# ppwwyyxx/OpenPano

Hardware: NVIDIA H100
Metric: Mpixels/sec SIFT+match+blend (higher is better)
Workload: dtype f32

## Files before the change

openpano_b200/csrc/common.cuh:

```cuda
#pragma once

#include <cuda_runtime.h>
#include <stdint.h>
#include <string>
#include <vector>
#include <map>
#include <memory>
#include <type_traits>
#include <unordered_map>

#include "../../include/pano_b200.h"


int  ctx_alloc(pano_ctx* ctx, void** p, size_t bytes);
void ctx_cache_release(pano_ctx* ctx, size_t keep_bytes);
void ctx_free(pano_ctx* ctx, void* p);
template <class T>
class DevBuf {
 public:
  DevBuf() = default;
  DevBuf(pano_ctx* ctx, T* p) : ctx_(ctx), p_(p) {}
  DevBuf(const DevBuf&) = delete;
  DevBuf& operator=(const DevBuf&) = delete;
  DevBuf(DevBuf&& o) noexcept : ctx_(o.ctx_), p_(o.release()) {}
  DevBuf& operator=(DevBuf&& o) noexcept {
    if (this != &o) { reset(); ctx_ = o.ctx_; p_ = o.release(); }
    return *this;
  }
  ~DevBuf() { reset(); }
  int alloc(pano_ctx* ctx, size_t count) {
    reset();
    ctx_ = ctx;
    void* q = nullptr;
    const int rc = ctx_alloc(ctx, &q, count * sizeof(T));
    p_ = (T*)q;
    return rc;
  }
  void reset() {
    if (p_) ctx_free(ctx_, p_);
    p_ = nullptr;
  }
  T* release() { T* q = p_; p_ = nullptr; return q; }
  T* get() const { return p_; }
  operator T*() const { return p_; }

 private:
  pano_ctx* ctx_ = nullptr;
  T* p_ = nullptr;
};

struct CudaDestroy {
  void operator()(void* host) const { cudaFreeHost(host); }
  void operator()(cudaEvent_t e) const { cudaEventDestroy(e); }
  void operator()(cudaStream_t s) const { cudaStreamDestroy(s); }
  void operator()(cudaMemPool_t p) const { cudaMemPoolDestroy(p); }
};
class PinnedBuf {
 public:
  cudaError_t grow(size_t bytes, size_t alloc, unsigned flags) {
    if (bytes <= cap()) return cudaSuccess;
    p_.reset();
    void* p = nullptr;
    const cudaError_t e = cudaHostAlloc(&p, alloc, flags);
    if (e == cudaSuccess) { p_.reset(p); cap_ = alloc; }
    return e;
  }
  void* get() const { return p_.get(); }
  size_t cap() const { return p_ ? cap_ : 0; }

 private:
  std::unique_ptr<void, CudaDestroy> p_;
  size_t cap_ = 0;
};
using EventPtr = std::unique_ptr<std::remove_pointer_t<cudaEvent_t>, CudaDestroy>;
using StreamPtr = std::unique_ptr<std::remove_pointer_t<cudaStream_t>, CudaDestroy>;
using PoolPtr = std::unique_ptr<std::remove_pointer_t<cudaMemPool_t>, CudaDestroy>;
static inline cudaError_t make_event(EventPtr* ev, unsigned flags) {
  cudaEvent_t e = nullptr;
  const cudaError_t err = cudaEventCreateWithFlags(&e, flags);
  ev->reset(err == cudaSuccess ? e : nullptr);
  return err;
}
static inline cudaError_t make_stream(StreamPtr* s) {
  cudaStream_t h = nullptr;
  const cudaError_t err = cudaStreamCreateWithFlags(&h, cudaStreamNonBlocking);
  s->reset(err == cudaSuccess ? h : nullptr);
  return err;
}


struct ProfEvent {
  const char* name;
  EventPtr start, stop;
};

struct SiftPlan;

struct pano_ctx {
  ~pano_ctx();
  StreamPtr own_stream;
  cudaStream_t stream = nullptr;
  PoolPtr pool;
  int device = 0;
  struct CachedBlock { void* p; unsigned long long stamp; };
  std::multimap<size_t, CachedBlock> cache;
  std::unordered_map<void*, size_t> live;
  size_t cached_bytes = 0, cache_limit = (size_t)16 << 30;
  unsigned long long cache_stamp = 0;
  std::string err;
  bool profiling = false;
  std::vector<ProfEvent> prof_pending;
  std::vector<EventPtr> event_pool;
  std::map<std::string, std::pair<int, double>> prof_acc;
  long long launches = 0;
  int last_match_exact_rows = 0;
  int last_match_nominated_rows = 0;
  int last_match_full_rescans = 0;
  int num_sms = 132;
  bool attr_tc = false, attr_match = false;
  int sift_cap = 0;
  std::unique_ptr<SiftPlan> sift_plan;
  void* tma_encode = nullptr;
  PinnedBuf pinned, pinned2;
  PinnedBuf ring;
  size_t ring_off = 0;
  std::vector<PinnedBuf> small_pinned;
  PinnedBuf flag;
  unsigned flag_seq = 0;
  DevBuf<double2> planet_tab;
};

static inline void ctx_enter(const pano_ctx* ctx) { if (ctx) cudaSetDevice(ctx->device); }

int  ctx_fail(pano_ctx* ctx, int code, const char* fmt, ...);
int  ctx_cuda(pano_ctx* ctx, cudaError_t e, const char* what);
void* ctx_pinned(pano_ctx* ctx, size_t bytes);
void* ctx_pinned2(pano_ctx* ctx, size_t bytes);
extern "C" bool host_is_pinned(const void* p);
cudaError_t ctx_spin_event(cudaEvent_t ev);
cudaError_t ctx_spin_stream(pano_ctx* ctx);
cudaError_t ctx_signal(pano_ctx* ctx, unsigned* token);
cudaError_t ctx_wait_signal(pano_ctx* ctx, unsigned token);
void* ctx_ring(pano_ctx* ctx, size_t bytes);
PinnedBuf ctx_small_pinned_get(pano_ctx* ctx, size_t bytes);
void ctx_small_pinned_put(pano_ctx* ctx, PinnedBuf&& b);
int  ctx_fetch(pano_ctx* ctx, void* d_dst, const void* h_pinned_src, size_t bytes);
int  ctx_store(pano_ctx* ctx, void* h_pinned_dst, const void* d_src, size_t bytes);
int  ctx_put(pano_ctx* ctx, void* d_dst, const void* h_src, size_t bytes);
int  ctx_zero(pano_ctx* ctx, void* d_dst, size_t bytes);
#define CTX_MAX_SEGS 8
int  ctx_put_many(pano_ctx* ctx, int n, void* const* d_dst, const void* const* h_src, const size_t* bytes);
int  ctx_store_many(pano_ctx* ctx, int n, void* const* h_pinned_dst, const void* const* d_src, const size_t* bytes);
int  ctx_copy_blocks(pano_ctx* ctx, int n, void* const* dst, const void* const* src, const size_t* bytes);
void ctx_prof_begin(pano_ctx* ctx, const char* name);
void ctx_prof_end(pano_ctx* ctx);

struct UploadRing {
  ~UploadRing() { if (copy) cudaStreamSynchronize(copy.get()); }
  cudaError_t init();
  int upload(pano_ctx* ctx, int count, const void* const* srcs, const size_t* bytes, const void** d_src, int* slot_out);
  cudaError_t release(pano_ctx* ctx, int slot);

  StreamPtr copy;
  EventPtr ev_copied[2];
  EventPtr ev_done[2];
  DevBuf<unsigned char> slot[2];
  size_t slot_cap[2] = {0, 0};
  PinnedBuf stage[2];
  int windows = 0;
};

double pano_now_ms();
extern double g_trace_slow_ms;
void pano_trace_slow(const char* what, double ms);
struct SlowCall {
  const char* what; double t0;
  explicit SlowCall(const char* w) : what(w), t0(g_trace_slow_ms > 0 ? pano_now_ms() : 0.0) {}
  ~SlowCall() { if (g_trace_slow_ms > 0) { const double d = pano_now_ms() - t0; if (d > g_trace_slow_ms) pano_trace_slow(what, d); } }
};

#define PANO_CUDA(ctx, call)                                          \
  do {                                                                \
    cudaError_t _e;                                                   \
    { SlowCall _sc(#call); _e = (call); }                             \
    if (_e != cudaSuccess) return ctx_cuda((ctx), _e, #call);         \
  } while (0)

#define PANO_LAUNCH(ctx, name, kernel, grid, block, smem, ...)                      \
  do {                                                                              \
    (ctx)->launches++;                                                              \
    if ((ctx)->profiling) ctx_prof_begin((ctx), (name));                            \
    { SlowCall _sc(name); kernel<<<(grid), (block), (smem), (ctx)->stream>>>(__VA_ARGS__); } \
    if ((ctx)->profiling) ctx_prof_end((ctx));                                      \
    cudaError_t _e = cudaGetLastError();                                            \
    if (_e != cudaSuccess) return ctx_cuda((ctx), _e, name);                        \
  } while (0)

struct __align__(64) TmaDesc { unsigned long long opaque[16]; };
int ctx_tma_encode(pano_ctx* ctx, TmaDesc* out, void* base, int rank, const unsigned long long* dims,
                   const unsigned long long* strides_bytes, const unsigned* box);

static inline int pix8_bytes(int fmt) {
  switch (fmt) {
    case PANO_PIX_GREY: return 1;
    case PANO_PIX_RGB: return 3;
    case PANO_PIX_RGBA: return 4;
    case PANO_PIX_RGB_PLANAR: return 3;
    default: return 0;
  }
}
static inline bool pix8_layout(int fmt) { return fmt == PANO_PIX_RGBA || fmt == PANO_PIX_RGB_PLANAR; }
int pix8_check(pano_ctx* ctx, const char* what, int i, int fmt, const void* d_pix);

static inline int ceil_div(int a, int b) { return (a + b - 1) / b; }
static inline unsigned grid_y(long long count) { return (unsigned)(count < 1 ? 1 : count < 65535 ? count : 65535); }
static inline size_t align_up(size_t a, size_t b) { return (a + b - 1) / b * b; }

int host_gauss_kernel(float sigma, int window_factor, float* taps, int cap);

#ifdef __CUDACC__

#define PANO_PI 3.14159265358979323846
#define PANO_PI_2 1.57079632679489661923
#define PANO_SQRT1_2 0.70710678118654752440

#define DBETWEEN(a, b, c) (((a) >= (b)) && ((a) <= (c) - 1))

__constant__ uint64_t c_exp2f_tab[32] = {
    0x3ff0000000000000ull, 0x3fefd9b0d3158574ull, 0x3fefb5586cf9890full, 0x3fef9301d0125b51ull,
    0x3fef72b83c7d517bull, 0x3fef54873168b9aaull, 0x3fef387a6e756238ull, 0x3fef1e9df51fdee1ull,
    0x3fef06fe0a31b715ull, 0x3feef1a7373aa9cbull, 0x3feedea64c123422ull, 0x3feece086061892dull,
    0x3feebfdad5362a27ull, 0x3feeb42b569d4f82ull, 0x3feeab07dd485429ull, 0x3feea47eb03a5585ull,
    0x3feea09e667f3bcdull, 0x3fee9f75e8ec5f74ull, 0x3feea11473eb0187ull, 0x3feea589994cce13ull,
    0x3feeace5422aa0dbull, 0x3feeb737b0cdc5e5ull, 0x3feec49182a3f090ull, 0x3feed503b23e255dull,
    0x3feee89f995ad3adull, 0x3feeff76f2fb5e47ull, 0x3fef199bdd85529cull, 0x3fef3720dcef9069ull,
    0x3fef5818dcfba487ull, 0x3fef7c97337b9b5full, 0x3fefa4afa2a490daull, 0x3fefd0765b6e4540ull};

__device__ __forceinline__ void load_exp2f_tab(uint64_t* s_tab, int tid) {
  if (tid < 32) s_tab[tid] = c_exp2f_tab[tid];
}

__device__ __forceinline__ float glibc_expf(float x, const uint64_t* __restrict__ tab) {
  if (x < -0x1.9fe368p6f) return 0.0f;
  const double InvLn2N = 0x1.71547652b82fep+0 * 32, SHIFT = 0x1.8p+52;
  const double C0 = 0x1.c6af84b912394p-5 / 32 / 32 / 32, C1 = 0x1.ebfce50fac4f3p-3 / 32 / 32,
               C2 = 0x1.62e42ff0c52d6p-1 / 32;
  double xd = (double)x;
  double z = InvLn2N * xd;
  double kd = z + SHIFT;
  uint64_t ki = (uint64_t)__double_as_longlong(kd);
  kd -= SHIFT;
  double r = z - kd;
  uint64_t t = tab[ki & 31];
  t += ki << 47;
  double s = __longlong_as_double((long long)t);
  z = C0 * r + C1;
  double r2 = r * r;
  double y = C2 * r + 1;
  y = z * r2 + y;
  y = y * s;
  return (float)y;
}

__device__ __forceinline__ float glibc_sincos_poly(double x, double x2, bool neg_table, int n) {
  const double sgn = neg_table ? -1.0 : 1.0;
  if ((n & 1) == 0) {
    const double s1c = -0x1.555545995a603p-3, s2c = 0x1.1107605230bc4p-7, s3c = -0x1.994eb3774cf24p-13;
    double x3 = x * x2;
    double s1 = s2c + x2 * s3c;
    double x7 = x3 * x2;
    double s = x + x3 * s1c;
    return (float)(s + x7 * s1);
  } else {
    const double c0 = sgn * 0x1p0, c1c = sgn * -0x1.ffffffd0c621cp-2, c2c = sgn * 0x1.55553e1068f19p-5,
                 c3c = sgn * -0x1.6c087e89a359dp-10, c4c = sgn * 0x1.99343027bf8c3p-16;
    double x4 = x2 * x2;
    double c2 = c3c + x2 * c4c;
    double c1 = c1c + x2 * c2c;
    double x6 = x4 * x2;
    double c = c0 + x2 * c1;
    return (float)(c + x6 * c2);
  }
}

__device__ __forceinline__ uint32_t glibc_abstop12(float x) { return (__float_as_uint(x) >> 20) & 0x7ff; }

__device__ __forceinline__ void glibc_sincosf(float y, float* sn, float* cs) {
  const double hpi_inv = 0x1.45F306DC9C883p+23, hpi = 0x1.921FB54442D18p0;
  double x = (double)y;
  if (glibc_abstop12(y) < glibc_abstop12(0x1.921FB6p-1f)) {
    double x2 = x * x;
    if (glibc_abstop12(y) < glibc_abstop12(0x1p-12f)) { *sn = y; *cs = 1.0f; return; }
    *sn = glibc_sincos_poly(x, x2, false, 0);
    *cs = glibc_sincos_poly(x, x2, false, 1);
    return;
  }
  double r = x * hpi_inv;
  int n = ((int32_t)r + 0x800000) >> 24;
  x = x - n * hpi;
  const double sign = ((n & 3) == 1 || (n & 3) == 2) ? -1.0 : 1.0;
  bool neg = (n & 2) != 0;
  *sn = glibc_sincos_poly(x * sign, x * x, neg, n);
  *cs = glibc_sincos_poly(x * sign, x * x, neg, n ^ 1);
}

__device__ __forceinline__ float glibc_hypotf(float x, float y) {
  double dx = (double)x, dy = (double)y;
  return (float)sqrt(dx * dx + dy * dy);
}

__device__ __forceinline__ float fast_atan(float y, float x) {
  float absx = fabsf(x), absy = fabsf(y);
  float m = absx > absy ? absx : absy;
  if ((double)m < 1e-6) return (float)(-PANO_PI);
  float a = (absy < absx ? absy : absx) / m;
  float s = a * a;
  double sd = (double)s, ad = (double)a;
  float r = (float)(((-0.0464964749 * sd + 0.15931422) * sd - 0.327622764) * sd * ad + ad);
  if (absy > absx) r = (float)(PANO_PI_2 - (double)r);
  if (x < 0) r = (float)(PANO_PI - (double)r);
  if (y < 0) r = -r;
  return r;
}

__device__ __forceinline__ void mag_ort_at(const float* __restrict__ img, int w, int x, int y,
                                           float* mag, float* ort) {
  const float* row = img + (size_t)y * w;
  float dy = row[x + w] - row[x - w];
  float dx = row[x + 1] - row[x - 1];
  *mag = glibc_hypotf(dx, dy);
  *ort = (float)((double)fast_atan(dy, dx) + PANO_PI);
}

struct SrcF32 {
  const float* img;
  static constexpr bool kMayBeNo = true, kLut = false;
  __device__ __forceinline__ void fetch(int w, int fr, int fc, float* q) const {
    const float* p00 = img + ((size_t)fr * w + fc) * 3;
    const float* p10 = p00 + (size_t)w * 3;
#pragma unroll
    for (int k = 0; k < 6; ++k) { q[k] = __ldg(p00 + k); q[6 + k] = __ldg(p10 + k); }
  }
};
struct SrcRgb8 {
  const unsigned char* pix;
  const float* lut;
  int channels;
  static constexpr bool kMayBeNo = false, kLut = true;
  __device__ __forceinline__ void fetch(int w, int fr, int fc, float* q) const {
    if (channels == 1) {
      const unsigned char* p00 = pix + (size_t)fr * w + fc;
      const float a = (float)__ldg(p00), b = (float)__ldg(p00 + 1);
      const float c = (float)__ldg(p00 + w), d = (float)__ldg(p00 + w + 1);
      q[0] = q[1] = q[2] = a; q[3] = q[4] = q[5] = b;
      q[6] = q[7] = q[8] = c; q[9] = q[10] = q[11] = d;
    } else {
      const unsigned char* p00 = pix + ((size_t)fr * w + fc) * 3;
      const unsigned char* p10 = p00 + (size_t)w * 3;
#pragma unroll
      for (int k = 0; k < 6; ++k) { q[k] = lut[__ldg(p00 + k)]; q[6 + k] = lut[__ldg(p10 + k)]; }
    }
  }
};
struct SrcPix8 {
  const unsigned char* pix;
  const float* lut;
  int fmt;
  size_t plane;
  static constexpr bool kMayBeNo = false, kLut = true;
  __device__ __forceinline__ void fetch(int w, int fr, int fc, float* q) const {
    if (fmt == PANO_PIX_RGBA) {
      const unsigned* p00 = reinterpret_cast<const unsigned*>(pix) + (size_t)fr * w + fc;
      const unsigned t[4] = {__ldg(p00), __ldg(p00 + 1), __ldg(p00 + w), __ldg(p00 + w + 1)};
#pragma unroll
      for (int k = 0; k < 4; ++k) {
        q[3 * k] = lut[t[k] & 0xff]; q[3 * k + 1] = lut[(t[k] >> 8) & 0xff]; q[3 * k + 2] = lut[(t[k] >> 16) & 0xff];
      }
    } else if (fmt == PANO_PIX_RGB_PLANAR) {
      const unsigned char* p00 = pix + (size_t)fr * w + fc;
#pragma unroll
      for (int ch = 0; ch < 3; ++ch) {
        const unsigned char* p = p00 + ch * plane;
        q[ch] = lut[__ldg(p)]; q[3 + ch] = lut[__ldg(p + 1)];
        q[6 + ch] = lut[__ldg(p + w)]; q[9 + ch] = lut[__ldg(p + w + 1)];
      }
    } else {
      SrcRgb8{pix, lut, fmt}.fetch(w, fr, fc, q);
    }
  }
};
__device__ __forceinline__ void build_rgb8_lut(float* lut, int tid) {
  if (tid < 256) lut[tid] = (float)((double)tid / 255.0);
}

__device__ __forceinline__ int f2i_x86(float v) {
  return (v >= -2147483648.0f && v < 2147483648.0f) ? (int)v : (int)0x80000000u;
}

template <class Src>
__device__ __forceinline__ bool interpolate_rgb(const Src& src, int w, int h, float r, float c, float* o0, float* o1,
                                                float* o2) {
  int fr = f2i_x86(floorf(r)), fc = f2i_x86(floorf(c));
  if (fr < 0 || fc < 0 || fc + 1 >= w || fr + 1 >= h) return false;
  r -= (float)fr;
  c -= (float)fc;
  float q[12];
  src.fetch(w, fr, fc, q);
  const float q00 = q[0], q01 = q[1], q02 = q[2], q03 = q[3], q04 = q[4], q05 = q[5];
  const float q10 = q[6], q11 = q[7], q12 = q[8], q13 = q[9], q14 = q[10], q15 = q[11];
  if (Src::kMayBeNo && (q00 < 0 || q10 < 0 || q13 < 0 || q03 < 0)) return false;
  float w00 = (1 - r) * (1 - c), w10 = r * (1 - c), w11 = r * c, w01 = (1 - r) * c;
  float a0 = 0.f + q00 * w00, a1 = 0.f + q01 * w00, a2 = 0.f + q02 * w00;
  a0 += q10 * w10; a1 += q11 * w10; a2 += q12 * w10;
  a0 += q13 * w11; a1 += q14 * w11; a2 += q15 * w11;
  a0 += q03 * w01; a1 += q04 * w01; a2 += q05 * w01;
  *o0 = a0; *o1 = a1; *o2 = a2;
  return true;
}
__device__ __forceinline__ bool interpolate_rgb(const float* __restrict__ img, int w, int h, float r, float c,
                                                float* o0, float* o1, float* o2) {
  return interpolate_rgb(SrcF32{img}, w, h, r, c, o0, o1, o2);
}

#endif
```

openpano_b200/csrc/match.cu:

```cuda
#include "sift.cuh"
#include "match_tc.cuh"
#include <float.h>
#include <stdlib.h>
#include <string.h>
#include <algorithm>

__device__ __forceinline__ float exact_dist(const float* __restrict__ a, const float* __restrict__ b) {
  float l0 = 0.f, l1 = 0.f, l2 = 0.f, l3 = 0.f;
  const float4* pa = (const float4*)a;
  const float4* pb = (const float4*)b;
#pragma unroll 8
  for (int k = 0; k < 32; ++k) {
    float4 x = __ldg(pa + k), y = __ldg(pb + k);
    float d0 = x.x - y.x, d1 = x.y - y.y, d2 = x.z - y.z, d3 = x.w - y.w;
    l0 += d0 * d0; l1 += d1 * d1; l2 += d2 * d2; l3 += d3 * d3;
  }
  return (l0 + l1) + (l2 + l3);
}

__device__ __forceinline__ void top2_merge(float& mn, int& idx, float& sec, float m2, int i2, float s2) {
  if (m2 < mn || (m2 == mn && i2 < idx)) { sec = fminf(mn, s2); mn = m2; idx = i2; }
  else sec = fminf(sec, m2);
}

#define MT 64
#define MT_STRIDE 132
#define MT_THREADS 256

struct MatchTask {
  long long q_base, t_base;
  int q_n, t_n;
  int q_row0;
  long long res_off;
};

struct RowInfo { float mn, mn_hi; int idx; float sec_lo, sec_hi; int state; int requested; int pad; };

__global__ void __launch_bounds__(MT_THREADS)
k_match_top2(const float* __restrict__ desc, const MatchTask* __restrict__ tasks, RowInfo* __restrict__ res) {
  extern __shared__ float sm[];
  float* sq = sm;
  float* st = sm + MT * MT_STRIDE;
  const MatchTask tk = tasks[blockIdx.x];
  const int tid = threadIdx.x, tx = tid & 15, ty = tid >> 4;
  const float* Q = desc + tk.q_base * 128;
  const float* T = desc + tk.t_base * 128;

  for (int i = tid; i < MT * 32; i += MT_THREADS) {
    int r = i >> 5, c4 = i & 31;
    int gr = tk.q_row0 + r;
    float4 v = make_float4(0.f, 0.f, 0.f, 0.f);
    if (gr < tk.q_n) v = __ldg((const float4*)(Q + (size_t)gr * 128) + c4);
    *(float4*)(sq + r * MT_STRIDE + c4 * 4) = v;
  }

  float bmn[4], bsec[4];
  int bidx[4];
#pragma unroll
  for (int i = 0; i < 4; ++i) { bmn[i] = FLT_MAX; bsec[i] = FLT_MAX; bidx[i] = 0x7fffffff; }

  for (int t0 = 0; t0 < tk.t_n; t0 += MT) {
    __syncthreads();
    for (int i = tid; i < MT * 32; i += MT_THREADS) {
      int r = i >> 5, c4 = i & 31;
      int gr = t0 + r;
      float4 v = make_float4(0.f, 0.f, 0.f, 0.f);
      if (gr < tk.t_n) v = __ldg((const float4*)(T + (size_t)gr * 128) + c4);
      *(float4*)(st + r * MT_STRIDE + c4 * 4) = v;
    }
    __syncthreads();
    float acc[4][4][4];
#pragma unroll
    for (int i = 0; i < 4; ++i)
#pragma unroll
      for (int j = 0; j < 4; ++j)
#pragma unroll
        for (int l = 0; l < 4; ++l) acc[i][j][l] = 0.f;
#pragma unroll 4
    for (int k = 0; k < 32; ++k) {
      float4 a[4], b[4];
#pragma unroll
      for (int i = 0; i < 4; ++i) a[i] = *(const float4*)(sq + (ty + 16 * i) * MT_STRIDE + k * 4);
#pragma unroll
      for (int j = 0; j < 4; ++j) b[j] = *(const float4*)(st + (tx + 16 * j) * MT_STRIDE + k * 4);
#pragma unroll
      for (int i = 0; i < 4; ++i)
#pragma unroll
        for (int j = 0; j < 4; ++j) {
          float d0 = a[i].x - b[j].x, d1 = a[i].y - b[j].y, d2 = a[i].z - b[j].z, d3 = a[i].w - b[j].w;
          acc[i][j][0] += d0 * d0; acc[i][j][1] += d1 * d1;
          acc[i][j][2] += d2 * d2; acc[i][j][3] += d3 * d3;
        }
    }
#pragma unroll
    for (int i = 0; i < 4; ++i)
#pragma unroll
      for (int j = 0; j < 4; ++j) {
        int col = t0 + tx + 16 * j;
        if (col < tk.t_n) {
          float d = (acc[i][j][0] + acc[i][j][1]) + (acc[i][j][2] + acc[i][j][3]);
          if (d < bmn[i]) { bsec[i] = bmn[i]; bmn[i] = d; bidx[i] = col; }
          else if (d < bsec[i]) bsec[i] = d;
        }
      }
  }
#pragma unroll
  for (int i = 0; i < 4; ++i) {
    float mn = bmn[i], sec = bsec[i];
    int idx = bidx[i];
#pragma unroll
    for (int off = 8; off >= 1; off >>= 1) {
      float m2 = __shfl_xor_sync(0xffffffffu, mn, off);
      float s2 = __shfl_xor_sync(0xffffffffu, sec, off);
      int i2 = __shfl_xor_sync(0xffffffffu, idx, off);
      top2_merge(mn, idx, sec, m2, i2, s2);
    }
    int row = tk.q_row0 + ty + 16 * i;
    if (tx == 0 && row < tk.q_n) {
      RowInfo o; o.mn = mn; o.mn_hi = mn; o.idx = idx; o.sec_lo = sec; o.sec_hi = sec; o.state = 3; o.requested = 0; o.pad = 0;
      res[tk.res_off + row] = o;
    }
  }
}


struct SideMeta {
  long long q_base, t_base;
  int q_n, t_n;
  long long res_off;
  int r0, r1;
  int parts, pad;
};

__device__ __forceinline__ float tc_eps(float nq, float nmax) {
  return 0.00215f * sqrtf(nq * nmax) + 0.0005f * nmax + 1.0f;
}

__device__ __forceinline__ RowInfo refine_row(const float* __restrict__ desc, const SideMeta& sm, int r, const TcTop2 ap,
                                              float eps, float ratio_sqr) {
  RowInfo o;
  o.requested = 0; o.pad = 0;
  const bool idx_ok = ap.idx >= 0 && ap.idx < sm.t_n;
  o.idx = idx_ok ? ap.idx : 0;
  const bool single = ap.m2 == FLT_MAX;
  const bool certain = idx_ok && (single || (ap.m2 - ap.m1 > 2.f * eps));
  if (sm.t_n <= 0) { o.mn = FLT_MAX; o.mn_hi = FLT_MAX; o.sec_lo = FLT_MAX; o.sec_hi = FLT_MAX; o.state = 3; }
  else if (certain && !single && (ap.m1 - eps) > ratio_sqr * (ap.m2 + eps)) {
    o.mn = ap.m1 - eps; o.mn_hi = ap.m1 + eps;
    o.sec_lo = fmaxf(ap.m2 - eps, o.mn); o.sec_hi = ap.m2 + eps;
    o.state = 2;
  }
  else if (certain) {
    o.mn = exact_dist(desc + (size_t)(sm.q_base + r) * 128, desc + (size_t)(sm.t_base + o.idx) * 128);
    o.mn_hi = o.mn;
    if (single) { o.sec_lo = FLT_MAX; o.sec_hi = FLT_MAX; o.state = 3; }
    else { o.sec_lo = fmaxf(ap.m2 - eps, o.mn); o.sec_hi = fmaxf(ap.m2 + eps, o.mn); o.state = 2; }
  } else {
    o.mn = fmaxf(ap.m1 - eps, 0.f); o.mn_hi = ap.m1 + eps;
    o.sec_lo = fmaxf(ap.m2 - eps, 0.f); o.sec_hi = ap.m2 + eps;
    o.state = 0;
  }
  return o;
}

__device__ __forceinline__ void refine_side_row(const float* __restrict__ desc, const float* __restrict__ norms,
                                                const unsigned* __restrict__ maxnorm_bits, const SideMeta* __restrict__ sides,
                                                TcTop2* __restrict__ approx, long long res_total, float ratio_sqr, int lazy,
                                                RowInfo* __restrict__ info, int side, int r) {
  const SideMeta sm = sides[side];
  if (r >= sm.q_n) return;
  if (r < sm.r0 || r >= sm.r1) return;
  if (lazy && (side & 1) && sm.t_n > 0) {
    RowInfo o; o.mn = 0.f; o.mn_hi = FLT_MAX; o.idx = 0; o.sec_lo = 0.f; o.sec_hi = FLT_MAX; o.state = 4; o.requested = 0; o.pad = 0;
    info[sm.res_off + r] = o;
    return;
  }
  const float nmax = __uint_as_float(*maxnorm_bits);
  TcTop2 ap = approx[sm.res_off + r];
  if (sm.parts > 1) {
    for (int p = 1; p < sm.parts; ++p) {
      const TcTop2 q = approx[(long long)p * res_total + sm.res_off + r];
      if (q.m1 < ap.m1) { ap.m2 = fminf(ap.m1, q.m2); ap.m1 = q.m1; ap.idx = q.idx; }
      else ap.m2 = fminf(ap.m2, q.m1);
    }
    approx[sm.res_off + r] = ap;
  }
  info[sm.res_off + r] = refine_row(desc, sm, r, ap, tc_eps(norms[sm.q_base + r], nmax), ratio_sqr);
}

__global__ void k_refine(const float* __restrict__ desc, const float* __restrict__ norms,
                         const unsigned* __restrict__ maxnorm_bits, const SideMeta* __restrict__ sides, int n_sides,
                         TcTop2* __restrict__ approx, long long res_total, float ratio_sqr, int lazy,
                         RowInfo* __restrict__ info) {
  const int r = blockIdx.x * blockDim.x + threadIdx.x;
  for (int side = blockIdx.y; side < n_sides; side += gridDim.y)
    refine_side_row(desc, norms, maxnorm_bits, sides, approx, res_total, ratio_sqr, lazy, info, side, r);
}

__global__ void k_refine_gathered(const float* __restrict__ desc, const float* __restrict__ norms,
                                  const unsigned* __restrict__ maxnorm_bits, const SideMeta* __restrict__ sides,
                                  const int2* __restrict__ g_meta, const TcTop2* __restrict__ g_approx,
                                  const int* __restrict__ n_blocks, float ratio_sqr, TcTop2* __restrict__ approx,
                                  RowInfo* __restrict__ info) {
  const int g = blockIdx.x * blockDim.x + threadIdx.x;
  if (g >= *n_blocks * 128) return;
  const int2 me = g_meta[g];
  if (me.x < 0) return;
  const SideMeta sm = sides[me.x];
  const TcTop2 ap = g_approx[g];
  const float nmax = __uint_as_float(*maxnorm_bits);
  approx[sm.res_off + me.y] = ap;
  info[sm.res_off + me.y] = refine_row(desc, sm, me.y, ap, tc_eps(norms[sm.q_base + me.y], nmax), ratio_sqr);
}

__global__ void __launch_bounds__(256)
k_exact_rows(const float* __restrict__ desc, const SideMeta* __restrict__ sides, const int2* __restrict__ list,
             const int* __restrict__ list_count, RowInfo* __restrict__ info) {
  __shared__ __align__(16) float sq[128];
  __shared__ float s_mn[8], s_sec[8];
  __shared__ int s_idx[8];
  const int tid = threadIdx.x, lane = tid & 31, wid = tid >> 5;
  const int n = *list_count;
  for (int e = blockIdx.x; e < n; e += gridDim.x) {
    const int2 it = list[e];
    const SideMeta sm = sides[it.x];
    const float* q = desc + (size_t)(sm.q_base + it.y) * 128;
    __syncthreads();
    if (tid < 32) *(float4*)(&sq[tid * 4]) = __ldg((const float4*)q + tid);
    __syncthreads();
    float mn = FLT_MAX, sec = FLT_MAX;
    int idx = 0x7fffffff;
    for (int c = tid; c < sm.t_n; c += 256) {
      const float4* pb = (const float4*)(desc + (size_t)(sm.t_base + c) * 128);
      float4 yv[32];
#pragma unroll
      for (int k = 0; k < 32; ++k) yv[k] = __ldg(pb + k);
      float l0 = 0.f, l1 = 0.f, l2 = 0.f, l3 = 0.f;
#pragma unroll
      for (int k = 0; k < 32; ++k) {
        const float4 x = *(const float4*)(&sq[k * 4]), y = yv[k];
        float d0 = x.x - y.x, d1 = x.y - y.y, d2 = x.z - y.z, d3 = x.w - y.w;
        l0 += d0 * d0; l1 += d1 * d1; l2 += d2 * d2; l3 += d3 * d3;
      }
      float d = (l0 + l1) + (l2 + l3);
      if (d < mn) { sec = mn; mn = d; idx = c; }
      else if (d < sec) sec = d;
    }
#pragma unroll
    for (int off = 16; off >= 1; off >>= 1) {
      float m2 = __shfl_xor_sync(0xffffffffu, mn, off);
      float s2 = __shfl_xor_sync(0xffffffffu, sec, off);
      int i2 = __shfl_xor_sync(0xffffffffu, idx, off);
      top2_merge(mn, idx, sec, m2, i2, s2);
    }
    if (lane == 0) { s_mn[wid] = mn; s_sec[wid] = sec; s_idx[wid] = idx; }
    __syncthreads();
    if (tid == 0) {
      for (int wdx = 1; wdx < 8; ++wdx) top2_merge(mn, idx, sec, s_mn[wdx], s_idx[wdx], s_sec[wdx]);
      RowInfo o; o.mn = mn; o.mn_hi = mn; o.idx = idx; o.sec_lo = sec; o.sec_hi = sec; o.state = 3; o.requested = 1; o.pad = 0;
      info[sm.res_off + it.y] = o;
    }
  }
}

struct PairMeta {
  int side_small, side_large;
  int n_small, n_large;
  long long out_off;
  int rev, pad;
  int k0, k1;
};

#define OUT_PENDING (-2)

__device__ __forceinline__ void request_row(const SideMeta* __restrict__ sides, RowInfo* __restrict__ info, int side,
                                            int row, int* list_rows, int* list_unknown,
                                            int* __restrict__ side_cnt, int n_sides) {
  const long long off = sides[side].res_off;
  RowInfo* ri = &info[off + row];
  if (atomicExch(&ri->requested, 1) == 0) {
    if (ri->state & 4) list_unknown[off + atomicAdd(&side_cnt[n_sides + side], 1)] = row;
    else list_rows[off + atomicAdd(&side_cnt[side], 1)] = row;
  }
}

__device__ __forceinline__ void match_decide_row(const PairMeta* __restrict__ pairs, const SideMeta* __restrict__ sides,
                                                 RowInfo* __restrict__ info, float ratio_sqr, int first_round,
                                                 int* __restrict__ out, int* __restrict__ total,
                                                 int* list_rows, int* list_unknown, int* __restrict__ side_cnt,
                                                 int n_sides, int pair, int row) {
  const PairMeta pm = pairs[pair];
  const int k = pm.k0 + row;
  if (k >= pm.k1) return;
  const size_t oslot = pm.out_off + k;
  if (!first_round && out[oslot] != OUT_PENDING) return;
  int result = -1;
  if (pm.n_large > 0) {
    const SideMeta ss = sides[pm.side_small], sl = sides[pm.side_large];
    const RowInfo r = info[ss.res_off + k];
    if (!(r.state & 2)) {
      if (r.mn > ratio_sqr * r.sec_hi) result = -1;
      else {
        result = OUT_PENDING;
        request_row(sides, info, pm.side_small, k, list_rows, list_unknown, side_cnt, n_sides);
        if (info[sl.res_off + r.idx].state & 4)
          request_row(sides, info, pm.side_large, r.idx, list_rows, list_unknown, side_cnt, n_sides);
      }
    } else {
      const RowInfo c = info[sl.res_off + r.idx];
      if (c.state & 4) {
        if (r.mn > ratio_sqr * r.sec_hi) result = -1;
        else if (!(r.mn > 0.f)) result = r.idx;
        else {
          result = OUT_PENDING;
          request_row(sides, info, pm.side_large, r.idx, list_rows, list_unknown, side_cnt, n_sides);
        }
      } else {
        float c_lo, c_hi;
        bool need_c = false;
        if (c.state & 2) {
          const bool mine = c.idx == k;
          c_lo = mine ? c.sec_lo : c.mn; c_hi = mine ? c.sec_hi : c.mn_hi;
          need_c = mine && !(c.state & 1);
        } else {
          c_lo = c.mn; c_hi = c.sec_hi;
          need_c = true;
        }
        const float nlo = fminf(r.sec_lo, c_lo), nhi = fminf(r.sec_hi, c_hi);
        if (r.mn > ratio_sqr * nhi) result = -1;
        else if (!(r.mn > ratio_sqr * nlo)) result = r.idx;
        else {
          result = OUT_PENDING;
          if (!(r.state & 1)) request_row(sides, info, pm.side_small, k, list_rows, list_unknown, side_cnt, n_sides);
          if (need_c) request_row(sides, info, pm.side_large, r.idx, list_rows, list_unknown, side_cnt, n_sides);
        }
      }
    }
  }
  out[oslot] = result;
  if (result >= 0) atomicAdd(total, 1);
}

__global__ void k_match_decide(const PairMeta* __restrict__ pairs, int n_pairs, const SideMeta* __restrict__ sides,
                               RowInfo* __restrict__ info, float ratio_sqr, int first_round,
                               int* __restrict__ out, int* __restrict__ total,
                               int* list_rows, int* list_unknown, int* __restrict__ side_cnt,
                               int n_sides) {
  const int row = blockIdx.x * blockDim.x + threadIdx.x;
  for (int pair = blockIdx.y; pair < n_pairs; pair += gridDim.y)
    match_decide_row(pairs, sides, info, ratio_sqr, first_round, out, total, list_rows, list_unknown, side_cnt, n_sides,
                     pair, row);
}

__global__ void k_gather_plan(const TcGatherSide* __restrict__ gsides, int n_sides, const int* __restrict__ side_cnt,
                              const int* __restrict__ list_rows, int block_cap, TcTask* __restrict__ tasks,
                              int* __restrict__ n_blocks, int2* __restrict__ fb_list, int* __restrict__ fb_cnt) {
  const int side = blockIdx.x * blockDim.x + threadIdx.x;
  if (side >= n_sides) return;
  const int cnt = side_cnt[side];
  if (cnt == 0) return;
  const TcGatherSide gs = gsides[side];
  const int nb = (cnt + 127) / 128;
  const int b0 = atomicAdd(n_blocks, nb);
  if (b0 + nb > block_cap) {
    atomicSub(n_blocks, nb);
    const int f0 = atomicAdd(fb_cnt, cnt);
    for (int i = 0; i < cnt; ++i) fb_list[f0 + i] = make_int2(side, list_rows[gs.list_off + i]);
    return;
  }
  for (int i = 0; i < nb; ++i) {
    TcTask t;
    t.q_blk = b0 + i; t.q_row0 = (b0 + i) * 128; t.q_n = min(128, cnt - i * 128);
    t.t_blk0 = gs.t_blk0; t.t_blocks = gs.t_blocks; t.t_n = gs.t_n; t.t_pad = i * 128;
    t.res_off = side;
    tasks[b0 + i] = t;
  }
}

__global__ void __launch_bounds__(256)
k_exact_cands(const float* __restrict__ desc, const SideMeta* __restrict__ sides, const int* __restrict__ n_blocks,
              const int2* __restrict__ g_meta, const int* __restrict__ cand_cnt, const int* __restrict__ cand,
              RowInfo* __restrict__ info, int2* __restrict__ fb_list, int* __restrict__ fb_cnt) {
  const int lane = threadIdx.x & 31;
  const int nrow = *n_blocks * 128;
  for (int g = blockIdx.x * 8 + (threadIdx.x >> 5); g < nrow; g += gridDim.x * 8) {
    const int2 me = g_meta[g];
    if (me.x < 0) continue;
    const SideMeta sm = sides[me.x];
    const int cnt = cand_cnt[g];
    if (cnt > TC_CAND_CAP || cnt < 1 || (cnt < 2 && sm.t_n >= 2)) {
      if (lane == 0) fb_list[atomicAdd(fb_cnt, 1)] = me;
      continue;
    }
    float mn = FLT_MAX, sec = FLT_MAX;
    int idx = 0x7fffffff;
    if (lane < cnt) {
      idx = cand[(size_t)g * TC_CAND_CAP + lane];
      mn = exact_dist(desc + (size_t)(sm.q_base + me.y) * 128, desc + (size_t)(sm.t_base + idx) * 128);
    }
#pragma unroll
    for (int off = 16; off >= 1; off >>= 1) {
      float m2 = __shfl_xor_sync(0xffffffffu, mn, off);
      float s2 = __shfl_xor_sync(0xffffffffu, sec, off);
      int i2 = __shfl_xor_sync(0xffffffffu, idx, off);
      top2_merge(mn, idx, sec, m2, i2, s2);
    }
    if (lane == 0) {
      RowInfo o; o.mn = mn; o.mn_hi = mn; o.idx = idx; o.sec_lo = sec; o.sec_hi = sec; o.state = 3; o.requested = 1; o.pad = 0;
      info[sm.res_off + me.y] = o;
    }
  }
}

__global__ void __launch_bounds__(256)
k_match_count(const PairMeta* __restrict__ pairs, const int* __restrict__ out, int n_pairs, int* __restrict__ hdr) {
  __shared__ int s_c[8], s_p[8];
  const PairMeta pm = pairs[blockIdx.x];
  int c = 0, pend = 0;
  for (int r = pm.k0 + threadIdx.x; r < pm.k1; r += 256) {
    const int v = out[pm.out_off + r];
    c += v >= 0; pend += v == OUT_PENDING;
  }
  for (int off = 16; off; off >>= 1) { c += __shfl_xor_sync(0xffffffffu, c, off); pend += __shfl_xor_sync(0xffffffffu, pend, off); }
  if ((threadIdx.x & 31) == 0) { s_c[threadIdx.x >> 5] = c; s_p[threadIdx.x >> 5] = pend; }
  __syncthreads();
  if (threadIdx.x == 0) {
    for (int q = 1; q < 8; ++q) { c += s_c[q]; pend += s_p[q]; }
    hdr[2 + blockIdx.x] = c;
    if (pend) atomicAdd(&hdr[1], pend);
  }
}

__global__ void __launch_bounds__(1024)
k_match_offsets(int n_pairs, int* __restrict__ hdr) {
  __shared__ int s_w[32];
  __shared__ int s_carry;
  const int* cnt = hdr + 2;
  int* off = hdr + 2 + n_pairs;
  const int tid = threadIdx.x, lane = tid & 31, wid = tid >> 5;
  if (tid == 0) s_carry = 0;
  __syncthreads();
  for (int base = 0; base < n_pairs; base += 1024) {
    const int k = base + tid;
    const int v = k < n_pairs ? cnt[k] : 0;
    int incl = v;
    for (int d = 1; d < 32; d <<= 1) { const int t = __shfl_up_sync(0xffffffffu, incl, d); if (lane >= d) incl += t; }
    if (lane == 31) s_w[wid] = incl;
    __syncthreads();
    if (wid == 0) {
      int w = s_w[lane], a = w;
      for (int d = 1; d < 32; d <<= 1) { const int t = __shfl_up_sync(0xffffffffu, a, d); if (lane >= d) a += t; }
      s_w[lane] = a - w;
    }
    __syncthreads();
    const int carry = s_carry;
    if (k < n_pairs) off[k] = carry + s_w[wid] + incl - v;
    __syncthreads();
    if (tid == 1023) s_carry = carry + s_w[31] + incl;
    __syncthreads();
  }
  if (tid == 0) { off[n_pairs] = s_carry; hdr[0] = s_carry; }
}

__global__ void __launch_bounds__(256)
k_match_write(const PairMeta* __restrict__ pairs, const int* __restrict__ out, int n_pairs, const int* __restrict__ hdr,
              int* __restrict__ dense) {
  __shared__ int s_w[8];
  __shared__ int s_base;
  const PairMeta pm = pairs[blockIdx.x];
  int* dst = dense + 2 * (size_t)hdr[2 + n_pairs + blockIdx.x];
  const int tid = threadIdx.x, lane = tid & 31, wid = tid >> 5;
  if (tid == 0) s_base = 0;
  __syncthreads();
  for (int r0 = pm.k0; r0 < pm.k1; r0 += 256) {
    const int r = r0 + tid;
    const int j = r < pm.k1 ? out[pm.out_off + r] : -1;
    const unsigned bal = __ballot_sync(0xffffffffu, j >= 0);
    if (lane == 0) s_w[wid] = __popc(bal);
    __syncthreads();
    int before = s_base;
    for (int q = 0; q < wid; ++q) before += s_w[q];
    if (j >= 0) {
      int* d = dst + 2 * (before + __popc(bal & ((1u << lane) - 1)));
      if (pm.rev) { d[0] = j; d[1] = r; } else { d[0] = r; d[1] = j; }
    }
    __syncthreads();
    if (tid == 0) { int t = 0; for (int q = 0; q < 8; ++q) t += s_w[q]; s_base += t; }
    __syncthreads();
  }
}

__global__ void k_match_download(int* __restrict__ h_dst, const int* __restrict__ dense, const int* __restrict__ hdr) {
  const size_t n = (size_t)hdr[0] * 2;
  for (size_t i = (size_t)blockIdx.x * blockDim.x + threadIdx.x; i < n; i += (size_t)gridDim.x * blockDim.x) h_dst[i] = dense[i];
}


struct MatchPlan {
  std::vector<SideMeta> sides;
  std::vector<PairMeta> pairs;
  std::vector<MatchTask> exact_tasks;
  std::vector<TcTask> tc_tasks;
  std::vector<int> task_part;
  std::vector<TcGatherSide> gsides;
  std::vector<char> rev;
  long long res_total = 0, out_total = 0;
  int max_side_n = 0, max_small = 0;
  int parts = 1;
  int shard = 0, n_shards = 1;
  bool lazy = false;
  long long large_blocks = 0;
  long long block_pairs = 0;
};

#define MC_FB(r) (1 + (r))
#define MC_BLK_FILTER(r) (5 + (r))
#define MC_BLK_NOMINATE(r) (9 + (r))
#define MC_HEAD 16
#define MC_ROUNDS 4

static bool use_exact_path() {
  const char* e = getenv("PANO_MATCH_PATH");
  return e && strcmp(e, "exact") == 0;
}

static int build_plan(pano_ctx* ctx, pano_featureset* fs, int n_pairs, const int* ij, MatchPlan& pl,
                      const std::vector<TcImage>* tcimgs) {
  for (int k = 0; k < n_pairs; ++k) {
    int i = ij[2 * k], j = ij[2 * k + 1];
    if (i < 0 || j < 0 || i >= fs->n_images || j >= fs->n_images)
      return ctx_fail(ctx, PANO_ERR_INVALID, "pair %d: image index out of range", k);
    if (fs->h_count[i] > 0 && fs->h_count[j] > 0) {
      const long long bl = (std::max(fs->h_count[i], fs->h_count[j]) + 127) / 128, bs = (std::min(fs->h_count[i], fs->h_count[j]) + 127) / 128;
      pl.large_blocks += bl;
      pl.block_pairs += bl * bs;
    }
  }
  if (tcimgs) {
    pl.lazy = pl.block_pairs >= 32768;
    if (const char* e = getenv("PANO_MATCH_LAZY")) pl.lazy = atoi(e) != 0;
    if (pl.n_shards > 1) pl.lazy = true;
    long long n1 = 0, tile_sum = 0;
    for (int k = 0; k < n_pairs; ++k) {
      const int ci = fs->h_count[ij[2 * k]], cj = fs->h_count[ij[2 * k + 1]];
      if (ci <= 0 || cj <= 0) continue;
      const long long bs = (std::min(ci, cj) + 127) / 128, bl = (std::max(ci, cj) + 127) / 128;
      const long long ts = (std::min(ci, cj) + 255) / 256, tl = (std::max(ci, cj) + 255) / 256;
      const long long mine = pl.lazy ? (bs + pl.n_shards - 1) / pl.n_shards : bs;
      n1 += mine; tile_sum += mine * tl;
      if (!pl.lazy) { n1 += bl; tile_sum += bl * ts; }
    }
    const long long W = std::max(1, ctx->num_sms);
    if (n1 > 0 && n1 < 12 * W) {
      const double T = (double)tile_sum / (double)n1;
      auto cost = [&](int P) { return (double)((n1 * P + W - 1) / W) * (T / P + 0.7); };
      double best = cost(1) * 0.96;
      for (int P = 2; P <= 8; ++P)
        if (T / P >= 4.0 && cost(P) < best * 0.99) { best = cost(P); pl.parts = P; }
    }
    if (const char* e = getenv("PANO_MATCH_PARTS")) pl.parts = std::max(1, std::min(8, atoi(e)));
  }
  for (int k = 0; k < n_pairs; ++k) {
    int i = ij[2 * k], j = ij[2 * k + 1];
    const bool rev = fs->h_count[i] > fs->h_count[j];
    const int is = rev ? j : i, il = rev ? i : j;
    const int ns = fs->h_count[is], nl = fs->h_count[il];
    const int k0 = (int)((long long)ns * pl.shard / pl.n_shards), k1 = (int)((long long)ns * (pl.shard + 1) / pl.n_shards);
    const int tiles_l = tcimgs ? (*tcimgs)[il].n_pad / 256 : 0, tiles_s = tcimgs ? (*tcimgs)[is].n_pad / 256 : 0;
    const int parts_a = std::max(1, std::min(pl.parts, tiles_l / 4)), parts_b = pl.lazy ? 1 : std::max(1, std::min(pl.parts, tiles_s / 4));
    SideMeta a{fs->base[is], fs->base[il], ns, nl, pl.res_total, k0, k1, parts_a, 0}; pl.res_total += ns;
    SideMeta b{fs->base[il], fs->base[is], nl, ns, pl.res_total, 0, nl, parts_b, 0}; pl.res_total += nl;
    PairMeta pm{(int)pl.sides.size(), (int)pl.sides.size() + 1, ns, nl, pl.out_total, rev ? 1 : 0, 0, k0, k1};
    pl.out_total += ns;
    pl.sides.push_back(a); pl.sides.push_back(b);
    pl.pairs.push_back(pm);
    pl.rev.push_back(rev ? 1 : 0);
    pl.max_side_n = std::max(pl.max_side_n, std::max(ns, nl));
    pl.max_small = std::max(pl.max_small, k1 - k0);
    if (tcimgs) {
      const TcImage &ts = (*tcimgs)[is], &tl = (*tcimgs)[il];
      auto add_tasks = [&](const TcImage& tq, const TcImage& tt, int row_lo, int row_hi, int q_n, int t_n, long long res_off, int parts) {
        const int tiles = tt.n_pad / 256;
        for (int r0 = row_lo / 128 * 128; r0 < row_hi; r0 += 128)
          for (int pp = 0; pp < parts; ++pp) {
            const int t0 = (int)((long long)tiles * pp / parts), t1 = (int)((long long)tiles * (pp + 1) / parts);
            pl.tc_tasks.push_back(TcTask{tq.blk0 + r0 / 128, r0, q_n, tt.blk0 + 2 * t0, 2 * (t1 - t0), t_n, t0 * 256, res_off});
            pl.task_part.push_back(pp);
          }
      };
      if (nl > 0) add_tasks(ts, tl, k0, k1, ns, nl, a.res_off, parts_a);
      if (ns > 0 && !pl.lazy) add_tasks(tl, ts, 0, nl, nl, ns, b.res_off, parts_b);
      pl.gsides.push_back(TcGatherSide{a.q_base, a.res_off, a.res_off, ts.blk0, tl.blk0, tl.n_pad / 128, nl});
      pl.gsides.push_back(TcGatherSide{b.q_base, b.res_off, b.res_off, tl.blk0, ts.blk0, ts.n_pad / 128, ns});
    } else {
      for (int r0 = k0 / MT * MT; r0 < k1; r0 += MT) pl.exact_tasks.push_back(MatchTask{a.q_base, a.t_base, ns, nl, r0, a.res_off});
      for (int r0 = 0; r0 < nl; r0 += MT) pl.exact_tasks.push_back(MatchTask{b.q_base, b.t_base, nl, ns, r0, b.res_off});
    }
  }
  for (size_t t = 0; t < pl.tc_tasks.size(); ++t) pl.tc_tasks[t].res_off += (long long)pl.task_part[t] * pl.res_total;
  return PANO_OK;
}

struct MatchBuffers {
  DevBuf<unsigned char> tasks; DevBuf<PairMeta> pairs; DevBuf<SideMeta> sides;
  DevBuf<RowInfo> info; DevBuf<TcTop2> approx;
  DevBuf<int2> list;
  DevBuf<int> counters;
  int n_counters = 0;
  DevBuf<int> out;
  DevBuf<TcGatherSide> gsides; DevBuf<int> list_rows; DevBuf<TcTask> gtasks; DevBuf<unsigned char> gq;
  DevBuf<int2> g_meta; DevBuf<int> g_thr; DevBuf<int> cand_cnt; DevBuf<int> cand;
  DevBuf<int> list_unknown; DevBuf<TcTask> ntasks; DevBuf<unsigned char> nq; DevBuf<int2> n_meta;
  DevBuf<TcTop2> n_approx;
  int rounds = 2;
};

static int run_plan(pano_ctx* ctx, pano_featureset* fs, const MatchPlan& pl, float ratio, bool tensor,
                    const TcOperands* ops, MatchBuffers& b) {
  int rc = 0;
  const size_t bt = tensor ? pl.tc_tasks.size() * sizeof(TcTask) : pl.exact_tasks.size() * sizeof(MatchTask);
  const size_t bp = pl.pairs.size() * sizeof(PairMeta), bs = pl.sides.size() * sizeof(SideMeta);
  const long long nres = std::max<long long>(pl.res_total, 1);
  if ((rc = b.tasks.alloc(ctx, bt)) || (rc = b.pairs.alloc(ctx, pl.pairs.size())) ||
      (rc = b.sides.alloc(ctx, pl.sides.size())) || (rc = b.info.alloc(ctx, nres)) ||
      (rc = b.approx.alloc(ctx, nres * std::max(pl.parts, 1))) || (rc = b.list.alloc(ctx, nres)) ||
      (rc = b.out.alloc(ctx, std::max<long long>(pl.out_total, 1))))
    return rc;
  const int n_sides = (int)pl.sides.size();
  b.n_counters = MC_HEAD + MC_ROUNDS * 2 * n_sides;
  if ((rc = b.counters.alloc(ctx, b.n_counters))) return rc;
  const void* tsrc = tensor ? (const void*)pl.tc_tasks.data() : (const void*)pl.exact_tasks.data();
  const size_t bg = tensor ? pl.gsides.size() * sizeof(TcGatherSide) : 0;
  if (bg && (rc = b.gsides.alloc(ctx, pl.gsides.size()))) return rc;
  {
    void* dsts[5] = {b.tasks, b.pairs, b.sides, b.counters, b.gsides};
    const void* srcs[5] = {tsrc, pl.pairs.data(), pl.sides.data(), nullptr, pl.gsides.data()};
    size_t sizes[5] = {bt, bp, bs, b.n_counters * sizeof(int), bg};
    if ((rc = ctx_put_many(ctx, 5, dsts, srcs, sizes))) return rc;
  }
  if (pl.pairs.empty()) return PANO_OK;
  const float rs = ratio * ratio;
  const int n_pairs = (int)pl.pairs.size();
  dim3 gd(std::max(1, ceil_div(pl.max_small, 256)), grid_y(n_pairs));
  if (!tensor) {
    const size_t smem = (size_t)2 * MT * MT_STRIDE * sizeof(float);
    if (!ctx->attr_match) {
      PANO_CUDA(ctx, cudaFuncSetAttribute(k_match_top2, cudaFuncAttributeMaxDynamicSharedMemorySize, (int)smem));
      ctx->attr_match = true;
    }
    if (!pl.exact_tasks.empty())
      PANO_LAUNCH(ctx, "k_match_top2", k_match_top2, (unsigned)pl.exact_tasks.size(), MT_THREADS, smem, fs->d_desc,
                  (const MatchTask*)b.tasks.get(), b.info);
    if (pl.max_small > 0) {
      if ((rc = b.list_rows.alloc(ctx, nres))) return rc;
      PANO_LAUNCH(ctx, "k_match_decide", k_match_decide, gd, 256, 0, b.pairs, n_pairs, b.sides, b.info, rs, 1, b.out,
                  b.counters, b.list_rows, b.list_rows, b.counters + MC_HEAD, n_sides);
    }
    return PANO_OK;
  }
  rc = tc_run_top2(ctx, ops, (const TcTask*)b.tasks.get(), (int)pl.tc_tasks.size(), b.approx);
  if (rc) return rc;
  if (pl.max_side_n > 0) {
    dim3 gr(ceil_div(pl.max_side_n, 128), grid_y(n_sides));
    PANO_LAUNCH(ctx, "k_refine", k_refine, gr, 128, 0, fs->d_desc, ops->d_norms, ops->d_maxnorm, b.sides, n_sides, b.approx,
                (long long)pl.res_total, rs, pl.lazy ? 1 : 0, b.info);
  }
  if (pl.max_small > 0) {
    int block_cap = (int)std::min<size_t>(std::max<size_t>(pl.tc_tasks.size(), 1), 4096);
    if (const char* e = getenv("PANO_MATCH_BLOCK_CAP")) block_cap = std::max(1, std::min(block_cap, atoi(e)));
    const size_t grow = (size_t)block_cap * 128;
    TcFilter f;
    if ((rc = b.list_rows.alloc(ctx, nres)) || (rc = b.gtasks.alloc(ctx, block_cap)) ||
        (rc = b.gq.alloc(ctx, (size_t)block_cap * tc_block_bytes())) || (rc = b.g_meta.alloc(ctx, grow)) ||
        (rc = b.g_thr.alloc(ctx, grow)) || (rc = b.cand_cnt.alloc(ctx, grow)) ||
        (rc = b.cand.alloc(ctx, grow * TC_CAND_CAP)))
      return rc;
    f.gq = b.gq; f.tasks = b.gtasks; f.gsides = b.gsides; f.list_rows = b.list_rows; f.approx = b.approx;
    f.g_meta = b.g_meta; f.g_thr = b.g_thr; f.cand_cnt = b.cand_cnt; f.cand = b.cand;
    TcFilter nf;
    int nom_cap = 0;
    if (pl.lazy) {
      nom_cap = (int)std::min<long long>(std::max<long long>(pl.large_blocks, 1), 8192);
      const size_t nrow = (size_t)nom_cap * 128;
      if ((rc = b.list_unknown.alloc(ctx, nres)) || (rc = b.ntasks.alloc(ctx, nom_cap)) ||
          (rc = b.nq.alloc(ctx, (size_t)nom_cap * tc_block_bytes())) || (rc = b.n_meta.alloc(ctx, nrow)) ||
          (rc = b.n_approx.alloc(ctx, nrow)))
        return rc;
      nf.gq = b.nq; nf.tasks = b.ntasks; nf.gsides = b.gsides; nf.list_rows = b.list_unknown; nf.approx = nullptr;
      nf.g_meta = b.n_meta; nf.g_thr = nullptr; nf.cand_cnt = nullptr; nf.cand = nullptr;
    }
    int* list_unknown = pl.lazy ? b.list_unknown : b.list_rows;
    const int eg = ctx->num_sms * 4;
    b.rounds = pl.lazy ? 3 : 2;
    for (int round = 0; round <= b.rounds; ++round) {
      int* side_cnt = b.counters + MC_HEAD + round * 2 * n_sides;
      int* fb_cnt = b.counters + MC_FB(round);
      int* n_blocks = b.counters + MC_BLK_FILTER(round);
      PANO_LAUNCH(ctx, "k_match_decide", k_match_decide, gd, 256, 0, b.pairs, n_pairs, b.sides, b.info, rs, round == 0 ? 1 : 0,
                  b.out, b.counters, b.list_rows, list_unknown, side_cnt, n_sides);
      if (round == b.rounds) break;
      if (pl.lazy) {
        int* nom_blocks = b.counters + MC_BLK_NOMINATE(round);
        PANO_LAUNCH(ctx, "k_gather_plan", k_gather_plan, ceil_div(n_sides, 128), 128, 0, b.gsides, n_sides,
                    side_cnt + n_sides, b.list_unknown, nom_cap, b.ntasks, nom_blocks, b.list, fb_cnt);
        nf.n_tasks = nom_blocks;
        if ((rc = tc_run_nominate(ctx, ops, &nf, nom_cap, b.n_approx))) return rc;
        PANO_LAUNCH(ctx, "k_refine_gathered", k_refine_gathered, nom_cap, 128, 0, fs->d_desc, ops->d_norms, ops->d_maxnorm,
                    b.sides, b.n_meta, b.n_approx, nom_blocks, rs, b.approx, b.info);
      }
      PANO_LAUNCH(ctx, "k_gather_plan", k_gather_plan, ceil_div(n_sides, 128), 128, 0, b.gsides, n_sides, side_cnt,
                  b.list_rows, block_cap, b.gtasks, n_blocks, b.list, fb_cnt);
      f.n_tasks = n_blocks;
      if ((rc = tc_run_filter(ctx, ops, &f, block_cap))) return rc;
      PANO_LAUNCH(ctx, "k_exact_cands", k_exact_cands, eg, 256, 0, fs->d_desc, b.sides, n_blocks, b.g_meta, b.cand_cnt,
                  b.cand, b.info, b.list, fb_cnt);
      PANO_LAUNCH(ctx, "k_exact_rows", k_exact_rows, eg, 256, 0, fs->d_desc, b.sides, b.list, fb_cnt, b.info);
    }
  }
  return PANO_OK;
}

static int ensure_tc_operands(pano_ctx* ctx, pano_featureset* fs, std::vector<TcImage>& imgs) {
  imgs.resize(fs->n_images);
  int blk = 0;
  for (int i = 0; i < fs->n_images; ++i) {
    TcImage& im = imgs[i];
    im.row0 = fs->base[i]; im.n = fs->h_count[i];
    im.n_pad = (im.n + 255) / 256 * 256;
    im.blk0 = blk;
    blk += im.n_pad / 128;
  }
  if (fs->tc_ready) return PANO_OK;
  int rc = tc_prepare(ctx, fs->d_desc, imgs, &fs->tc);
  if (rc) return rc;
  fs->tc_ready = true;
  return PANO_OK;
}

static int match_common(pano_ctx* ctx, pano_featureset* fs, int n_pairs, const int* ij, const pano_params* p,
                        int shard, int n_shards, MatchPlan& pl, MatchBuffers& b) {
  if (n_shards < 1 || shard < 0 || shard >= n_shards) return ctx_fail(ctx, PANO_ERR_INVALID, "shard %d of %d", shard, n_shards);
  pl.shard = shard; pl.n_shards = n_shards;
  int rc = featureset_sync_counts(fs);
  if (rc) return rc;
  const bool tensor = !use_exact_path();
  std::vector<TcImage> tcimgs;
  if (tensor && (rc = ensure_tc_operands(ctx, fs, tcimgs))) return rc;
  rc = build_plan(ctx, fs, n_pairs, ij, pl, tensor ? &tcimgs : nullptr);
  if (rc) return rc;
  return run_plan(ctx, fs, pl, p->match_reject_next_ratio, tensor, &fs->tc, b);
}

extern "C" {

int pano_match_pairs(pano_ctx* ctx, pano_featureset* fs, int n_pairs, const int* ij, const pano_params* p,
                     pano_matches* out) {
  return pano_match_pairs_shard(ctx, fs, n_pairs, ij, p, 0, 1, out);
}

int pano_match_pairs_shard(pano_ctx* ctx, pano_featureset* fs, int n_pairs, const int* ij, const pano_params* p,
                           int shard, int n_shards, pano_matches* out) {
  ctx_enter(ctx);
  if (!ctx || !fs || !out || n_pairs < 0 || (n_pairs && !ij) || !p) return PANO_ERR_INVALID;
  memset(out, 0, sizeof(*out));
  MatchPlan pl;
  MatchBuffers b;
  int rc = match_common(ctx, fs, n_pairs, ij, p, shard, n_shards, pl, b);
  if (rc) return rc;
  const size_t n_hdr = 3 + 2 * (size_t)n_pairs;
  const size_t cap = (size_t)std::max<long long>(pl.out_total, 1) * 2;
  DevBuf<int> d_hdr, d_dense;
  if ((rc = d_hdr.alloc(ctx, n_hdr)) || (rc = d_dense.alloc(ctx, cap))) return rc;
  int* h_stage = (int*)ctx_ring(ctx, (n_hdr + cap) * sizeof(int));
  if (!h_stage) return ctx_fail(ctx, PANO_ERR_CUDA, "pinned ring allocation failed");
  if ((rc = ctx_zero(ctx, d_hdr, 2 * sizeof(int)))) return rc;
  if (n_pairs > 0) {
    PANO_LAUNCH(ctx, "k_match_count", k_match_count, n_pairs, 256, 0, b.pairs, b.out, n_pairs, d_hdr);
    PANO_LAUNCH(ctx, "k_match_offsets", k_match_offsets, 1, 1024, 0, n_pairs, d_hdr);
    PANO_LAUNCH(ctx, "k_match_write", k_match_write, n_pairs, 256, 0, b.pairs, b.out, n_pairs, d_hdr, d_dense);
    PANO_LAUNCH(ctx, "k_match_download", k_match_download, std::max(1, std::min(ctx->num_sms, (int)(cap / 4096) + 1)), 256, 0,
                h_stage + n_hdr, d_dense, d_hdr);
  }
  rc = ctx_store(ctx, h_stage, d_hdr, n_hdr * sizeof(int));
  cudaError_t e = ctx_spin_stream(ctx);
  if (rc) return rc;
  if (e != cudaSuccess) return ctx_cuda(ctx, e, "match download");
  if (n_pairs > 0 && h_stage[1] != 0) return ctx_fail(ctx, PANO_ERR_CUDA, "match: %d undecided rows (internal error)", h_stage[1]);
  const int total = n_pairs > 0 ? h_stage[0] : 0;
  out->n_pairs = n_pairs;
  out->count = (int*)calloc(std::max(n_pairs, 1), sizeof(int));
  out->offset = (int*)calloc(n_pairs + 1, sizeof(int));
  out->idx = (int*)calloc((size_t)std::max(total, 1) * 2, sizeof(int));
  if (n_pairs > 0) {
    memcpy(out->count, h_stage + 2, (size_t)n_pairs * sizeof(int));
    memcpy(out->offset, h_stage + 2 + n_pairs, (size_t)(n_pairs + 1) * sizeof(int));
    memcpy(out->idx, h_stage + n_hdr, (size_t)total * 2 * sizeof(int));
  }
  return PANO_OK;
}

void pano_matches_free(pano_matches* m) {
  if (!m) return;
  free(m->count); free(m->offset); free(m->idx);
  memset(m, 0, sizeof(*m));
}

int pano_match_pairs_dev(pano_ctx* ctx, pano_featureset* fs, int n_pairs, const int* ij, const pano_params* p,
                         int* total_matches) {
  return pano_match_pairs_dev_shard(ctx, fs, n_pairs, ij, p, 0, 1, total_matches);
}

int pano_match_pairs_dev_shard(pano_ctx* ctx, pano_featureset* fs, int n_pairs, const int* ij, const pano_params* p,
                               int shard, int n_shards, int* total_matches) {
  ctx_enter(ctx);
  if (!ctx || !fs || n_pairs < 0 || (n_pairs && !ij) || !p || !total_matches) return PANO_ERR_INVALID;
  MatchPlan pl;
  MatchBuffers b;
  int rc = match_common(ctx, fs, n_pairs, ij, p, shard, n_shards, pl, b);
  if (rc) return rc;
  int* h = (int*)ctx_ring(ctx, (size_t)std::max(b.n_counters, MC_HEAD) * sizeof(int));
  if (!h) return ctx_fail(ctx, PANO_ERR_CUDA, "pinned ring allocation failed");
  const int n_counters = b.n_counters, n_sides = (int)pl.sides.size(), rounds = b.rounds;
  rc = b.counters ? ctx_store(ctx, h, b.counters, (size_t)n_counters * sizeof(int)) : 0;
  cudaError_t e = ctx_spin_stream(ctx);
  if (rc) return rc;
  if (e != cudaSuccess) return ctx_cuda(ctx, e, "match total download");
  if (n_counters < MC_HEAD) { *total_matches = 0; return PANO_OK; }
  long long requested = 0, nominated = 0, undecided = 0, rescans = 0;
  for (int round = 0; round <= rounds; ++round)
    for (int q = 0; q < 2 * n_sides; ++q) {
      const int v = h[MC_HEAD + round * 2 * n_sides + q];
      if (round == rounds) undecided += v;
      else if (q < n_sides) requested += v;
      else nominated += v;
    }
  for (int round = 0; round < rounds; ++round) rescans += h[MC_FB(round)];
  ctx->last_match_nominated_rows = (int)nominated;
  ctx->last_match_exact_rows = (int)requested;
  ctx->last_match_full_rescans = (int)rescans;
  if (undecided != 0) return ctx_fail(ctx, PANO_ERR_CUDA, "match: %lld rows undecided after the exact passes", undecided);
  *total_matches = h[0];
  return PANO_OK;
}

int pano_match_bruteforce(pano_ctx* ctx, const float* a, int n, const float* b, int m, const pano_params* p,
                          int* pairs_out, int* n_pairs_out) {
  ctx_enter(ctx);
  if (!ctx || n < 0 || m < 0 || !p || !pairs_out || !n_pairs_out) return PANO_ERR_INVALID;
  *n_pairs_out = 0;
  if (n == 0 || m == 0) return PANO_OK;
  int cnt[2] = {n, m};
  const float* ds[2] = {a, b};
  pano_featureset* fs = nullptr;
  int rc = pano_featureset_upload(ctx, 2, cnt, ds, nullptr, &fs);
  if (rc) return rc;
  int ij[2] = {0, 1};
  pano_matches mt;
  rc = pano_match_pairs(ctx, fs, 1, ij, p, &mt);
  pano_featureset_free(fs);
  if (rc) return rc;
  *n_pairs_out = mt.count[0];
  memcpy(pairs_out, mt.idx, sizeof(int) * 2 * mt.count[0]);
  pano_matches_free(&mt);
  return PANO_OK;
}

}
```

openpano_b200/csrc/match_tc.cu:

```cuda
#include "sift.cuh"
#include "match_tc.cuh"
#include <cuda_fp16.h>
#include <float.h>
#include <algorithm>

#define TC_KC 18
#define TC_BLOCK_BYTES (TC_KC * 2048)
#define TC_LBO 2048u
#define TC_TLBO 4096u
#define TC_SBO 128u
#define TC_TILE_BLOCKS 2
#define TC_STAGES 2
#define TC_THREADS 384
#define TC_CONSUMER_WARPS 8


__global__ void k_tc_maxnorm(const float* __restrict__ desc, const TcImage* __restrict__ imgs, int n_img,
                             float* __restrict__ norms, unsigned* __restrict__ maxnorm_bits) {
  const int img = blockIdx.y;
  const TcImage im = imgs[img];
  const int r = blockIdx.x * blockDim.x + threadIdx.x;
  float n = 0.f;
  if (r < im.n) {
    const float4* p = (const float4*)(desc + (size_t)(im.row0 + r) * 128);
    float acc = 0.f;
#pragma unroll 8
    for (int k = 0; k < 32; ++k) { float4 v = __ldg(p + k); acc += v.x * v.x; acc += v.y * v.y; acc += v.z * v.z; acc += v.w * v.w; }
    n = acc;
    norms[im.row0 + r] = n;
  }
  for (int off = 16; off; off >>= 1) n = fmaxf(n, __shfl_xor_sync(0xffffffffu, n, off));
  if ((threadIdx.x & 31) == 0 && n > 0.f) atomicMax(maxnorm_bits, __float_as_uint(n));
}

__device__ __forceinline__ float tc_scale_from_maxnorm(float maxn2) {
  if (!(maxn2 > 0.f)) return 1.f;
  int e = (int)ceilf(0.5f * log2f(maxn2 / 1024.f));
  return exp2f((float)-e);
}

__global__ void k_tc_prep(const float* __restrict__ desc, const float* __restrict__ norms,
                          const unsigned* __restrict__ maxnorm_bits, const TcImage* __restrict__ imgs,
                          unsigned char* __restrict__ qbuf, unsigned char* __restrict__ tbuf) {
  const TcImage im = imgs[blockIdx.y];
  const int r = blockIdx.x * blockDim.x + threadIdx.x;
  if (r >= im.n_pad) return;
  const float s = tc_scale_from_maxnorm(__uint_as_float(*maxnorm_bits));
  const size_t blk = (size_t)(im.blk0 + r / 128);
  const int rr = r % 128;
  unsigned char* qd = qbuf + blk * TC_BLOCK_BYTES + (rr / 8) * TC_SBO + (rr % 8) * 16;
  const int tr = r % 256;
  unsigned char* td = tbuf + (size_t)(im.blk0 + (r / 256) * 2) * TC_BLOCK_BYTES + (tr / 8) * TC_SBO + (tr % 8) * 16;
  const bool real = r < im.n;
  const float4* p = (const float4*)(desc + (size_t)(im.row0 + (real ? r : 0)) * 128);
#pragma unroll 4
  for (int kc = 0; kc < 16; ++kc) {
    float4 a = real ? __ldg(p + 2 * kc) : make_float4(0.f, 0.f, 0.f, 0.f);
    float4 b = real ? __ldg(p + 2 * kc + 1) : make_float4(0.f, 0.f, 0.f, 0.f);
    __half2 q0 = __floats2half2_rn(a.x * s, a.y * s), q1 = __floats2half2_rn(a.z * s, a.w * s);
    __half2 q2 = __floats2half2_rn(b.x * s, b.y * s), q3 = __floats2half2_rn(b.z * s, b.w * s);
    const float m = -2.f * s;
    __half2 t0 = __floats2half2_rn(a.x * m, a.y * m), t1 = __floats2half2_rn(a.z * m, a.w * m);
    __half2 t2 = __floats2half2_rn(b.x * m, b.y * m), t3 = __floats2half2_rn(b.z * m, b.w * m);
    uint4 qv, tv;
    qv.x = *(unsigned*)&q0; qv.y = *(unsigned*)&q1; qv.z = *(unsigned*)&q2; qv.w = *(unsigned*)&q3;
    tv.x = *(unsigned*)&t0; tv.y = *(unsigned*)&t1; tv.z = *(unsigned*)&t2; tv.w = *(unsigned*)&t3;
    *(uint4*)(qd + (size_t)kc * TC_LBO) = qv;
    *(uint4*)(td + (size_t)kc * TC_TLBO) = tv;
  }
  float n = real ? norms[im.row0 + r] * s * s : 0.f;
  __half nh = __float2half_rn(n);
  __half nl = __float2half_rn(n - __half2float(nh));
  const __half one = __float2half_rn(1.f), zero = __float2half_rn(0.f);
  __half qx[8] = {one, one, nh, nl, one, zero, zero, zero};
  __half tx[8] = {nh, nl, one, one, one, zero, zero, zero};
  if (!real) {
    tx[0] = __float2half_rn(30000.f); tx[1] = zero; tx[2] = zero; tx[3] = zero; tx[4] = zero;
    qx[2] = zero; qx[3] = zero;
  }
  *(uint4*)(qd + (size_t)16 * TC_LBO) = *(uint4*)qx;
  *(uint4*)(td + (size_t)16 * TC_TLBO) = *(uint4*)tx;
  *(uint4*)(qd + (size_t)17 * TC_LBO) = make_uint4(0, 0, 0, 0);
  *(uint4*)(td + (size_t)17 * TC_TLBO) = make_uint4(0, 0, 0, 0);
}


__device__ __forceinline__ uint32_t smem_u32(const void* p) { return (uint32_t)__cvta_generic_to_shared(p); }

__device__ __forceinline__ void mbar_init(uint32_t bar, uint32_t count) {
  asm volatile("mbarrier.init.shared::cta.b64 [%0], %1;" ::"r"(bar), "r"(count));
}
__device__ __forceinline__ void mbar_arrive(uint32_t bar) {
  asm volatile("mbarrier.arrive.shared::cta.b64 _, [%0];" ::"r"(bar) : "memory");
}
__device__ __forceinline__ void mbar_expect_tx(uint32_t bar, uint32_t bytes) {
  asm volatile("mbarrier.arrive.expect_tx.shared::cta.b64 _, [%0], %1;" ::"r"(bar), "r"(bytes) : "memory");
}
__device__ __forceinline__ void mbar_wait(uint32_t bar, uint32_t parity) {
  uint32_t done = 0;
  for (uint32_t spin = 0; spin < (1u << 28); ++spin) {
    asm volatile(
        "{\n\t.reg .pred P1;\n\t"
        "mbarrier.try_wait.parity.shared::cta.b64 P1, [%1], %2;\n\t"
        "selp.b32 %0, 1, 0, P1;\n\t}"
        : "=r"(done)
        : "r"(bar), "r"(parity)
        : "memory");
    if (done) return;
  }
  __trap();
}
__device__ __forceinline__ void bulk_g2s(uint32_t dst, const void* src, uint32_t bytes, uint32_t bar) {
  asm volatile("cp.async.bulk.shared::cluster.global.mbarrier::complete_tx::bytes [%0], [%1], %2, [%3];"
               ::"r"(dst), "l"(src), "r"(bytes), "r"(bar) : "memory");
}
__device__ __forceinline__ uint64_t make_smem_desc(uint32_t saddr, uint32_t lbo) {
  return (uint64_t)((saddr & 0x3FFFFu) >> 4) | ((uint64_t)(lbo >> 4) << 16) | ((uint64_t)(TC_SBO >> 4) << 32);
}
__device__ __forceinline__ void wgmma_m64n128k16(float (&d)[64], uint64_t adesc, uint64_t bdesc, int accum) {
  asm volatile(
      "{\n\t.reg .pred p;\n\t"
      "setp.ne.b32 p, %66, 0;\n\t"
      "wgmma.mma_async.sync.aligned.m64n128k16.f32.f16.f16 "
      "{%0, %1, %2, %3, %4, %5, %6, %7, %8, %9, %10, %11, %12, %13, %14, %15, %16, %17, %18, %19, %20, %21, %22, %23, %24, %25, %26, %27, %28, %29, %30, %31, %32, %33, %34, %35, %36, %37, %38, %39, %40, %41, %42, %43, %44, %45, %46, %47, %48, %49, %50, %51, %52, %53, %54, %55, %56, %57, %58, %59, %60, %61, %62, %63}, "
      "%64, %65, p, 1, 1, 0, 0;\n\t}"
      : "+f"(d[0]), "+f"(d[1]), "+f"(d[2]), "+f"(d[3]), "+f"(d[4]), "+f"(d[5]), "+f"(d[6]), "+f"(d[7]),
        "+f"(d[8]), "+f"(d[9]), "+f"(d[10]), "+f"(d[11]), "+f"(d[12]), "+f"(d[13]), "+f"(d[14]), "+f"(d[15]),
        "+f"(d[16]), "+f"(d[17]), "+f"(d[18]), "+f"(d[19]), "+f"(d[20]), "+f"(d[21]), "+f"(d[22]), "+f"(d[23]),
        "+f"(d[24]), "+f"(d[25]), "+f"(d[26]), "+f"(d[27]), "+f"(d[28]), "+f"(d[29]), "+f"(d[30]), "+f"(d[31]),
        "+f"(d[32]), "+f"(d[33]), "+f"(d[34]), "+f"(d[35]), "+f"(d[36]), "+f"(d[37]), "+f"(d[38]), "+f"(d[39]),
        "+f"(d[40]), "+f"(d[41]), "+f"(d[42]), "+f"(d[43]), "+f"(d[44]), "+f"(d[45]), "+f"(d[46]), "+f"(d[47]),
        "+f"(d[48]), "+f"(d[49]), "+f"(d[50]), "+f"(d[51]), "+f"(d[52]), "+f"(d[53]), "+f"(d[54]), "+f"(d[55]),
        "+f"(d[56]), "+f"(d[57]), "+f"(d[58]), "+f"(d[59]), "+f"(d[60]), "+f"(d[61]), "+f"(d[62]), "+f"(d[63])
      : "l"(adesc), "l"(bdesc), "r"(accum));
}
__device__ __forceinline__ void wgmma_fence() { asm volatile("wgmma.fence.sync.aligned;" ::: "memory"); }
__device__ __forceinline__ void wgmma_commit() { asm volatile("wgmma.commit_group.sync.aligned;" ::: "memory"); }
template <int N>
__device__ __forceinline__ void wgmma_wait() { asm volatile("wgmma.wait_group.sync.aligned %0;" ::"n"(N) : "memory"); }
__device__ __forceinline__ void acc_fence(float (&d)[64]) {
#pragma unroll
  for (int i = 0; i < 64; ++i) asm volatile("" : "+f"(d[i])::"memory");
}


struct __align__(8) TcBarriers {
  uint64_t full[TC_STAGES], empty[TC_STAGES], a_full[2], a_empty[2];
};

template <bool FILTER, int H>
__device__ __forceinline__ void tc_reduce_half(const float (&d)[64], uint32_t keymask, bool prefilter, const int* g2,
                                               int* k1, int* k2, const int* thr, int col_base, int t_n, const int* grow,
                                               int* __restrict__ cand_cnt, int* __restrict__ cand) {
  if (FILTER) {
#pragma unroll
    for (int r = 0; r < 2; ++r) {
      unsigned hit = 0;
#pragma unroll
      for (int j = 0; j < 32; ++j)
        hit |= ((int)(__float_as_uint(d[4 * (j >> 1) + 2 * r + (j & 1)]) & 0xffffff00u) <= thr[r]) ? (1u << j) : 0u;
      while (hit) {
        const int j = __ffs(hit) - 1;
        hit &= hit - 1;
        const int col = col_base + H * 128 + 8 * (j >> 1) + (j & 1);
        if (col < t_n) {
          const int slot = atomicAdd(&cand_cnt[grow[r]], 1);
          if (slot < TC_CAND_CAP) cand[(size_t)grow[r] * TC_CAND_CAP + slot] = col;
        }
      }
    }
  } else {
    if (prefilter) {
      int m0 = (int)__float_as_uint(d[0]), m1 = (int)__float_as_uint(d[2]);
#pragma unroll
      for (int i = 0; i < 16; ++i) {
        m0 = min(m0, min((int)__float_as_uint(d[4 * i]), (int)__float_as_uint(d[4 * i + 1])));
        m1 = min(m1, min((int)__float_as_uint(d[4 * i + 2]), (int)__float_as_uint(d[4 * i + 3])));
      }
      if (!__any_sync(0xffffffffu, m0 < g2[0] || m1 < g2[1])) return;
    }
#pragma unroll
    for (int i = 0; i < 16; ++i)
#pragma unroll
      for (int e = 0; e < 4; ++e) {
        uint32_t ukey;
        asm("lop3.b32 %0, %1, %2, %3, 0xEA;" : "=r"(ukey) : "r"(__float_as_uint(d[4 * i + e])), "r"(keymask), "r"((uint32_t)(H * 128 + 8 * i + (e & 1))));
        const int key = (int)ukey, r = e >> 1;
        k2[r] = min(k2[r], max(k1[r], key));
        k1[r] = min(k1[r], key);
      }
  }
}

template <bool FILTER>
__global__ void __launch_bounds__(TC_THREADS, 1)
k_tc_pass(const unsigned char* __restrict__ qbuf, const unsigned char* __restrict__ tbuf,
          const TcTask* __restrict__ tasks, const int* __restrict__ n_tasks_dev, int n_tasks_host,
          const unsigned* __restrict__ maxnorm_bits, TcTop2* __restrict__ res,
          const int* __restrict__ g_thr, int* __restrict__ cand_cnt, int* __restrict__ cand) {
  extern __shared__ __align__(1024) unsigned char tc_smem[];
  const int task_end = n_tasks_dev ? *n_tasks_dev : n_tasks_host;
  if ((int)blockIdx.x >= task_end) return;
  unsigned char* sA = tc_smem;
  unsigned char* sB = tc_smem + 2 * TC_BLOCK_BYTES;
  TcBarriers* bars = (TcBarriers*)(sB + (size_t)TC_STAGES * TC_TILE_BLOCKS * TC_BLOCK_BYTES);
  const int warp = threadIdx.x >> 5, lane = threadIdx.x & 31;
  if (threadIdx.x == 0) {
    for (int s = 0; s < TC_STAGES; ++s) { mbar_init(smem_u32(&bars->full[s]), 1); mbar_init(smem_u32(&bars->empty[s]), TC_CONSUMER_WARPS); }
    for (int s = 0; s < 2; ++s) { mbar_init(smem_u32(&bars->a_full[s]), 1); mbar_init(smem_u32(&bars->a_empty[s]), TC_CONSUMER_WARPS); }
    asm volatile("fence.mbarrier_init.release.cluster;" ::: "memory");
  }
  __syncthreads();

  if (warp == 0) {
    if (lane == 0) {
      uint32_t gt = 0;
      uint32_t ti = 0;
      for (int task = blockIdx.x; task < task_end; task += gridDim.x, ++ti) {
        const TcTask tk = tasks[task];
        const int ntile = tk.t_blocks / TC_TILE_BLOCKS;
        const uint32_t as = ti & 1u;
        mbar_wait(smem_u32(&bars->a_empty[as]), ((ti >> 1) & 1u) ^ 1u);
        mbar_expect_tx(smem_u32(&bars->a_full[as]), TC_BLOCK_BYTES);
        bulk_g2s(smem_u32(sA + (size_t)as * TC_BLOCK_BYTES), qbuf + (size_t)tk.q_blk * TC_BLOCK_BYTES, TC_BLOCK_BYTES,
                 smem_u32(&bars->a_full[as]));
        for (int t = 0; t < ntile; ++t, ++gt) {
          const uint32_t s = gt % TC_STAGES, ph = (gt / TC_STAGES) & 1u;
          mbar_wait(smem_u32(&bars->empty[s]), ph ^ 1u);
          const uint32_t bytes = TC_TILE_BLOCKS * TC_BLOCK_BYTES;
          mbar_expect_tx(smem_u32(&bars->full[s]), bytes);
          bulk_g2s(smem_u32(sB + (size_t)s * bytes), tbuf + (size_t)(tk.t_blk0 + t * TC_TILE_BLOCKS) * TC_BLOCK_BYTES, bytes,
                   smem_u32(&bars->full[s]));
        }
      }
    }
  } else if (warp >= 4) {
    const int wg = (warp - 4) >> 2, quad = lane & 3;
    const int r0 = wg * 64 + (warp & 3) * 16 + (lane >> 2);
    const int rows[2] = {r0, r0 + 8};
    uint32_t keymask;
    asm volatile("mov.b32 %0, 0xffffff00;" : "=r"(keymask));
    float acc0[64], acc1[64];
    uint32_t gt = 0, ti = 0;
    for (int task = blockIdx.x; task < task_end; task += gridDim.x, ++ti) {
      const TcTask tk = tasks[task];
      const int ntile = tk.t_blocks / TC_TILE_BLOCKS;
      int g1[2] = {0x7f7fff00, 0x7f7fff00}, g2[2] = {0x7f7fff00, 0x7f7fff00};
      int gi[2] = {0x7fffffff, 0x7fffffff};
      const int col0 = (FILTER || n_tasks_dev) ? 0 : tk.t_pad;
      int grow[2], thr[2];
#pragma unroll
      for (int r = 0; r < 2; ++r) { grow[r] = tk.q_row0 + rows[r]; thr[r] = FILTER ? g_thr[grow[r]] : 0; }
      const bool prefilter = !FILTER && tk.t_blocks >= 128;
      const uint32_t asl = ti & 1u;
      mbar_wait(smem_u32(&bars->a_full[asl]), (ti >> 1) & 1u);
      const uint32_t a0 = smem_u32(sA + (size_t)asl * TC_BLOCK_BYTES) + (uint32_t)(wg * 8) * TC_SBO;
      for (int t = 0; t < ntile; ++t, ++gt) {
        const uint32_t s = gt % TC_STAGES;
        mbar_wait(smem_u32(&bars->full[s]), (gt / TC_STAGES) & 1u);
        const uint32_t b0 = smem_u32(sB + (size_t)s * TC_TILE_BLOCKS * TC_BLOCK_BYTES);
        acc_fence(acc0); acc_fence(acc1);
        wgmma_fence();
#pragma unroll
        for (int k = 0; k < TC_KC / 2; ++k)
          wgmma_m64n128k16(acc0, make_smem_desc(a0 + k * 2 * TC_LBO, TC_LBO), make_smem_desc(b0 + k * 2 * TC_TLBO, TC_TLBO), k);
        wgmma_commit();
#pragma unroll
        for (int k = 0; k < TC_KC / 2; ++k)
          wgmma_m64n128k16(acc1, make_smem_desc(a0 + k * 2 * TC_LBO, TC_LBO),
                           make_smem_desc(b0 + 16 * TC_SBO + k * 2 * TC_TLBO, TC_TLBO), k);
        wgmma_commit();
        int k1[2] = {0x7fffffff, 0x7fffffff}, k2[2] = {0x7fffffff, 0x7fffffff};
        const int col_base = t * 256 + 2 * quad;
        wgmma_wait<1>();
        acc_fence(acc0);
        tc_reduce_half<FILTER, 0>(acc0, keymask, prefilter, g2, k1, k2, thr, col_base, tk.t_n, grow, cand_cnt, cand);
        wgmma_wait<0>();
        acc_fence(acc1);
        __syncwarp();
        if (lane == 0) mbar_arrive(smem_u32(&bars->empty[s]));
        tc_reduce_half<FILTER, 1>(acc1, keymask, prefilter, g2, k1, k2, thr, col_base, tk.t_n, grow, cand_cnt, cand);
        if (!FILTER) {
#pragma unroll
          for (int r = 0; r < 2; ++r) {
            const int v1 = k1[r] & (int)0xffffff00, v2 = k2[r] & (int)0xffffff00;
            if (v1 < g1[r]) { g2[r] = min(g1[r], v2); g1[r] = v1; gi[r] = col0 + col_base + (k1[r] & 0xff); }
            else g2[r] = min(g2[r], v1);
          }
        }
      }
      __syncwarp();
      if (lane == 0) mbar_arrive(smem_u32(&bars->a_empty[asl]));
#pragma unroll
      for (int r = 0; r < 2 && !FILTER; ++r) {
#pragma unroll
        for (int off = 1; off < 4; off <<= 1) {
          const int o1 = __shfl_xor_sync(0xffffffffu, g1[r], off), o2 = __shfl_xor_sync(0xffffffffu, g2[r], off);
          const int oi = __shfl_xor_sync(0xffffffffu, gi[r], off);
          if (o1 < g1[r] || (o1 == g1[r] && oi < gi[r])) { g2[r] = min(g1[r], o2); g1[r] = o1; gi[r] = oi; }
          else g2[r] = min(g2[r], o1);
        }
        const int qrow = tk.q_row0 + rows[r];
        if (quad == 0 && (n_tasks_dev ? rows[r] < tk.q_n : qrow < tk.q_n)) {
          const float s = tc_scale_from_maxnorm(__uint_as_float(*maxnorm_bits));
          const float inv = 1.f / (s * s);
          TcTop2 o;
          o.m1 = (__int_as_float(g1[r]) - 1.f) * inv;
          o.m2 = g2[r] == 0x7f7fff00 ? FLT_MAX : (__int_as_float(g2[r]) - 1.f) * inv;
          o.idx = gi[r];
          o.pad = 0;
          res[(n_tasks_dev ? 0 : tk.res_off) + qrow] = o;
        }
      }
    }
  }
}


size_t tc_block_bytes() { return TC_BLOCK_BYTES; }

size_t tc_smem_bytes() {
  return (size_t)TC_BLOCK_BYTES * (2 + TC_STAGES * TC_TILE_BLOCKS) + sizeof(TcBarriers) + 1024;
}

int tc_prepare(pano_ctx* ctx, const float* d_desc, const std::vector<TcImage>& imgs, TcOperands* ops) {
  const int n = (int)imgs.size();
  long long rows = 0, blocks = 0;
  int max_pad = 0;
  for (auto& im : imgs) { rows = std::max<long long>(rows, im.row0 + im.n); blocks = std::max<long long>(blocks, im.blk0 + im.n_pad / 128); max_pad = std::max(max_pad, im.n_pad); }
  int rc = 0;
  if ((rc = ops->d_imgs.alloc(ctx, n)) || (rc = ops->d_norms.alloc(ctx, std::max<long long>(rows, 1))) ||
      (rc = ops->d_maxnorm.alloc(ctx, 1)) ||
      (rc = ops->qbuf.alloc(ctx, (size_t)std::max<long long>(blocks, 1) * TC_BLOCK_BYTES)) ||
      (rc = ops->tbuf.alloc(ctx, (size_t)std::max<long long>(blocks, 1) * TC_BLOCK_BYTES)))
    return rc;
  if ((rc = ctx_put(ctx, ops->d_imgs, imgs.data(), n * sizeof(TcImage)))) return rc;
  if ((rc = ctx_zero(ctx, ops->d_maxnorm, sizeof(unsigned)))) return rc;
  if (max_pad == 0) return PANO_OK;
  dim3 g1(ceil_div(max_pad, 128), n);
  PANO_LAUNCH(ctx, "k_tc_maxnorm", k_tc_maxnorm, g1, 128, 0, d_desc, ops->d_imgs, n, ops->d_norms, ops->d_maxnorm);
  PANO_LAUNCH(ctx, "k_tc_prep", k_tc_prep, g1, 128, 0, d_desc, ops->d_norms, ops->d_maxnorm, ops->d_imgs, ops->qbuf, ops->tbuf);
  return PANO_OK;
}

static int tc_set_attrs(pano_ctx* ctx) {
  if (ctx->attr_tc) return PANO_OK;
  const size_t smem = tc_smem_bytes();
  PANO_CUDA(ctx, cudaFuncSetAttribute(k_tc_pass<false>, cudaFuncAttributeMaxDynamicSharedMemorySize, (int)smem));
  PANO_CUDA(ctx, cudaFuncSetAttribute(k_tc_pass<true>, cudaFuncAttributeMaxDynamicSharedMemorySize, (int)smem));
  ctx->attr_tc = true;
  return PANO_OK;
}

int tc_run_top2(pano_ctx* ctx, const TcOperands* ops, const TcTask* d_tasks, int n_tasks, TcTop2* d_res) {
  if (n_tasks == 0) return PANO_OK;
  const size_t smem = tc_smem_bytes();
  if (int rc = tc_set_attrs(ctx)) return rc;
  PANO_LAUNCH(ctx, "k_tc_top2", k_tc_pass<false>, std::min(n_tasks, ctx->num_sms), TC_THREADS, smem, ops->qbuf, ops->tbuf, d_tasks,
              (const int*)nullptr, n_tasks, ops->d_maxnorm, d_res, (const int*)nullptr, (int*)nullptr, (int*)nullptr);
  return PANO_OK;
}


__global__ void __launch_bounds__(128)
k_tc_gather_rows(const unsigned char* __restrict__ qbuf, unsigned char* __restrict__ gq,
                 const TcTask* __restrict__ tasks, const int* __restrict__ n_tasks_dev,
                 const TcGatherSide* __restrict__ gsides, const int* __restrict__ list_rows,
                 const TcTop2* __restrict__ approx, const float* __restrict__ norms,
                 const unsigned* __restrict__ maxnorm_bits, int2* __restrict__ g_meta, int* __restrict__ g_thr,
                 int* __restrict__ cand_cnt) {
  if ((int)blockIdx.x >= *n_tasks_dev) return;
  const TcTask tk = tasks[blockIdx.x];
  const int side = (int)tk.res_off;
  const TcGatherSide gs = gsides[side];
  const int r = threadIdx.x, g = tk.q_row0 + r;
  unsigned char* dst = gq + (size_t)tk.q_blk * TC_BLOCK_BYTES + (r / 8) * TC_SBO + (r % 8) * 16;
  if (r < tk.q_n) {
    const int row = list_rows[gs.list_off + tk.t_pad + r];
    const unsigned char* src = qbuf + (size_t)(gs.q_blk0 + row / 128) * TC_BLOCK_BYTES + ((row % 128) / 8) * TC_SBO + (row % 8) * 16;
#pragma unroll
    for (int kc = 0; kc < TC_KC; ++kc) *(uint4*)(dst + (size_t)kc * TC_LBO) = *(const uint4*)(src + (size_t)kc * TC_LBO);
    if (approx) {
      const float nmax = __uint_as_float(*maxnorm_bits);
      const float s = tc_scale_from_maxnorm(nmax);
      const float nq = norms[gs.q_base + row];
      const float eps = 0.00215f * sqrtf(nq * nmax) + 0.0005f * nmax + 1.0f;
      const TcTop2 ap = approx[gs.res_off + row];
      float thr_v = ap.m2 == FLT_MAX ? FLT_MAX : (ap.m2 + 2.5f * eps) * (s * s) + 1.f;
      g_thr[g] = (int)(__float_as_uint(thr_v) | 0xffu);
      cand_cnt[g] = 0;
    }
    g_meta[g] = make_int2(side, row);
  } else {
#pragma unroll
    for (int kc = 0; kc < TC_KC; ++kc) *(uint4*)(dst + (size_t)kc * TC_LBO) = make_uint4(0, 0, 0, 0);
    if (approx) { g_thr[g] = -1; cand_cnt[g] = 0; }
    g_meta[g] = make_int2(-1, -1);
  }
}

int tc_run_filter(pano_ctx* ctx, const TcOperands* ops, const TcFilter* f, int max_blocks) {
  if (max_blocks <= 0) return PANO_OK;
  const size_t smem = tc_smem_bytes();
  if (int rc = tc_set_attrs(ctx)) return rc;
  PANO_LAUNCH(ctx, "k_tc_gather_rows", k_tc_gather_rows, max_blocks, 128, 0, ops->qbuf, f->gq, f->tasks, f->n_tasks,
              f->gsides, f->list_rows, f->approx, ops->d_norms, ops->d_maxnorm, f->g_meta, f->g_thr, f->cand_cnt);
  PANO_LAUNCH(ctx, "k_tc_filter", k_tc_pass<true>, std::min(max_blocks, ctx->num_sms), TC_THREADS, smem, f->gq, ops->tbuf, f->tasks, f->n_tasks,
              0, ops->d_maxnorm, (TcTop2*)nullptr, f->g_thr, f->cand_cnt, f->cand);
  return PANO_OK;
}

int tc_run_nominate(pano_ctx* ctx, const TcOperands* ops, const TcFilter* f, int max_blocks, TcTop2* d_res) {
  if (max_blocks <= 0) return PANO_OK;
  const size_t smem = tc_smem_bytes();
  if (int rc = tc_set_attrs(ctx)) return rc;
  PANO_LAUNCH(ctx, "k_tc_gather_rows", k_tc_gather_rows, max_blocks, 128, 0, ops->qbuf, f->gq, f->tasks, f->n_tasks,
              f->gsides, f->list_rows, (const TcTop2*)nullptr, ops->d_norms, ops->d_maxnorm, f->g_meta, (int*)nullptr,
              (int*)nullptr);
  PANO_LAUNCH(ctx, "k_tc_nominate", k_tc_pass<false>, std::min(max_blocks, ctx->num_sms), TC_THREADS, smem, f->gq, ops->tbuf, f->tasks,
              f->n_tasks, 0, ops->d_maxnorm, d_res, (const int*)nullptr, (int*)nullptr, (int*)nullptr);
  return PANO_OK;
}
```

openpano_b200/csrc/match_tc.cuh:

```cuda
#pragma once
#include "common.cuh"
#include <vector>

struct TcImage {
  long long row0;
  int n;
  int n_pad;
  int blk0;
};

struct TcTop2 { float m1, m2; int idx; int pad; };

#define TC_CAND_CAP 16

struct TcTask {
  int q_blk;
  int q_row0, q_n;
  int t_blk0, t_blocks;
  int t_n, t_pad;
  long long res_off;
};

struct TcGatherSide {
  long long q_base;
  long long res_off;
  long long list_off;
  int q_blk0;
  int t_blk0, t_blocks, t_n;
};

struct TcFilter {
  unsigned char* gq;
  TcTask* tasks;
  int* n_tasks;
  const TcGatherSide* gsides;
  const int* list_rows;
  const TcTop2* approx;
  int2* g_meta;
  int* g_thr;
  int* cand_cnt;
  int* cand;
};

struct TcOperands {
  DevBuf<TcImage> d_imgs;
  DevBuf<float> d_norms;
  DevBuf<unsigned> d_maxnorm;
  DevBuf<unsigned char> qbuf;
  DevBuf<unsigned char> tbuf;
};

int  tc_prepare(pano_ctx* ctx, const float* d_desc, const std::vector<TcImage>& imgs, TcOperands* ops);
int  tc_run_top2(pano_ctx* ctx, const TcOperands* ops, const TcTask* d_tasks, int n_tasks, TcTop2* d_res);
int  tc_run_filter(pano_ctx* ctx, const TcOperands* ops, const TcFilter* f, int max_blocks);
int  tc_run_nominate(pano_ctx* ctx, const TcOperands* ops, const TcFilter* f, int max_blocks, TcTop2* d_res);
size_t tc_block_bytes();
```

openpano_b200/csrc/sift.cu:

```cuda
#include "sift.cuh"
#include "desc_interval.h"
#include <math.h>
#include <string.h>
#include <algorithm>
#include <map>
#include <mutex>
#include <cuda.h>

__device__ __forceinline__ void bilinear_coef(int d, float inv, int src_n, int* s, float* frac) {
  float r = ((float)d + 0.5f) * inv - 0.5f;
  int si = (int)floorf(r);
  r -= (float)si;
  if (si < 0) { si = 0; r = 0.f; }
  else if (si + 1 >= src_n) { si = src_n - 2; r = 1.f; }
  *s = si; *frac = r;
}

__device__ __forceinline__ int first_tap_at_least(int t, float inv, int src_n, int dst_n) {
  auto tap = [&](int d) { int s; float f; bilinear_coef(d, inv, src_n, &s, &f); return s; };
  int d = (int)fminf(fmaxf(((float)t + 0.5f) / inv - 0.5f, 0.f), (float)dst_n);
  while (d > 0 && tap(d - 1) >= t) --d;
  while (d < dst_n && tap(d) < t) ++d;
  return d;
}

#define PG_TW 64
#define PG_TH 32
#define PG_THREADS 256

template <class Src>
__global__ void __launch_bounds__(PG_THREADS) k_pyramid_grey(const ImgMeta* __restrict__ imgs,
                                                             const OctMeta* __restrict__ octs, int n_oct,
                                                             float* __restrict__ arena, float* work) {
  constexpr int SW = PG_TW + 1, SP = SW * (PG_TH + 1);
  __shared__ float tile[3 * SP];
  __shared__ float lut[Src::kLut ? 256 : 1];
  const ImgMeta im = imgs[blockIdx.z];
  const int C0 = blockIdx.x * PG_TW, R0 = blockIdx.y * PG_TH;
  if (C0 >= im.w0 || R0 >= im.h0) return;
  const int own_w = min(PG_TW, im.w0 - C0), own_h = min(PG_TH, im.h0 - R0);
  const int last_c = min(PG_TW, im.w0 - 1 - C0), last_r = min(PG_TH, im.h0 - 1 - R0);
  Src src;
  if constexpr (Src::kLut) {
    build_rgb8_lut(lut, threadIdx.x);
    __syncthreads();
    if constexpr (std::is_same<Src, SrcPix8>::value) src = Src{im.pix, lut, im.channels, (size_t)im.in_w * im.in_h};
    else src = Src{im.pix, lut, im.channels};
  } else {
    src = Src{im.src};
  }
  const OctMeta& o0 = octs[blockIdx.z * n_oct];
  float* g0 = arena + o0.gauss_off;
  auto stage = [&](int lr, int lc, int sy, float ry) {
    const int r = R0 + lr, c = C0 + lc;
    int sx; float rx;
    bilinear_coef(r, im.ifx, im.in_h, &sx, &rx);
    const float irx = 1.0f - rx, iry = 1.0f - ry;
    float q[12];
    src.fetch(im.in_w, sx, sy, q);
    float v[3];
#pragma unroll
    for (int ch = 0; ch < 3; ++ch) {
      v[ch] = rx * (q[9 + ch] * ry + q[6 + ch] * iry) + irx * (q[3 + ch] * ry + q[ch] * iry);
      tile[ch * SP + lr * SW + lc] = v[ch];
    }
    if (lr < own_h && lc < own_w) {
      g0[(size_t)r * o0.pitch + c] = (v[0] + v[1] + v[2]) / 3.f;
      if (work) {
        float* dst = work + im.work_off + ((size_t)r * im.w0 + c) * 3;
        dst[0] = v[0]; dst[1] = v[1]; dst[2] = v[2];
      }
    }
  };
  constexpr int PG_ROWS_PER_PASS = PG_THREADS / PG_TW;
  static_assert(PG_THREADS % PG_TW == 0 && PG_TW >= PG_TH + 1, "whole row groups; the last one holds the halo column");
  {
    const int lc = threadIdx.x % PG_TW;
    if (lc <= last_c) {
      int sy; float ry;
      bilinear_coef(C0 + lc, im.ify, im.in_w, &sy, &ry);
      for (int lr = threadIdx.x / PG_TW; lr <= last_r; lr += PG_ROWS_PER_PASS) stage(lr, lc, sy, ry);
    }
    const int hr = (int)threadIdx.x - (PG_THREADS - PG_TW);
    if (hr >= 0 && hr <= last_r && PG_TW <= last_c) {
      int sy; float ry;
      bilinear_coef(C0 + PG_TW, im.ify, im.in_w, &sy, &ry);
      stage(hr, PG_TW, sy, ry);
    }
  }
  if (n_oct == 1) return;
  __syncthreads();
  for (int o = 1; o < n_oct; ++o) {
    const OctMeta& om = octs[blockIdx.z * n_oct + o];
    const float ifx = om.ifx, ify = om.ify;
    const int d_r0 = first_tap_at_least(R0, ifx, im.h0, om.h), d_r1 = first_tap_at_least(R0 + PG_TH, ifx, im.h0, om.h);
    const int d_c0 = first_tap_at_least(C0, ify, im.w0, om.w), d_c1 = first_tap_at_least(C0 + PG_TW, ify, im.w0, om.w);
    const int nc = d_c1 - d_c0;
    if (nc == 0) continue;
    float* g = arena + om.gauss_off;
    const int pitch = om.pitch;
    const int step_r = PG_THREADS / nc, step_c = PG_THREADS - step_r * nc;
    int dr = d_r0 + (int)threadIdx.x / nc, dc = d_c0 + (int)threadIdx.x % nc;
    for (; dr < d_r1; dr += step_r, dc += step_c) {
      if (dc >= d_c1) { dc -= nc; ++dr; if (dr >= d_r1) break; }
      int sx, sy; float rx, ry;
      bilinear_coef(dr, ifx, im.h0, &sx, &rx);
      bilinear_coef(dc, ify, im.w0, &sy, &ry);
      const float irx = 1.0f - rx, iry = 1.0f - ry;
      const float* p0 = tile + (sx - R0) * SW + (sy - C0);
      const float* p1 = p0 + SW;
      float v[3];
#pragma unroll
      for (int ch = 0; ch < 3; ++ch)
        v[ch] = rx * (p1[ch * SP + 1] * ry + p1[ch * SP] * iry) + irx * (p0[ch * SP + 1] * ry + p0[ch * SP] * iry);
      g[(size_t)dr * pitch + dc] = (v[0] + v[1] + v[2]) / 3.f;
    }
  }
}

struct ExtremaParams {
  int nscale;
  float pre_color_thres, diff_thres;
  int cap;
  int* cand_count;
  uint32_t* cand_keys;
  int seam_cap;
  int* seam_count;
  uint32_t* seam_keys;
};

__device__ __forceinline__ uint32_t make_key(int oct, int scale, int y, int x) {
  return ((uint32_t)oct << 29) | ((uint32_t)scale << 26) | ((uint32_t)y << 13) | (uint32_t)x;
}

template <class DoG>
__device__ __forceinline__ bool is_extremum(float center, float pre_color_thres, float diff_thres, const DoG& dog) {
  if (center < pre_color_thres) return false;
  const float cmp1 = center - diff_thres, cmp2 = center + diff_thres;
  bool mx = true, mn = true;
#pragma unroll
  for (int ds = -1; ds <= 1; ++ds) {
#pragma unroll
    for (int di = -1; di <= 1; ++di)
#pragma unroll
      for (int dj = -1; dj <= 1; ++dj) {
        if (ds == 0 && di == 0 && dj == 0) continue;
        const float v = dog(ds, di, dj);
        if (v >= cmp1) mx = false;
        if (v <= cmp2) mn = false;
      }
    if (!mx && !mn) return false;
  }
  return true;
}

__device__ __forceinline__ void append_candidate(const ExtremaParams& ep, int img, uint32_t key) {
  const int slot = atomicAdd(&ep.cand_count[img], 1);
  if (slot < ep.cap) ep.cand_keys[(size_t)img * ep.cap + slot] = key;
}

#include "blur_tile.cuh"

__global__ void __launch_bounds__(BT_THREADS)
k_blur_dog(const OctMeta* __restrict__ octs, const int2* __restrict__ span, int n_om,
           float* __restrict__ arena, const __grid_constant__ GaussTable gt) {
  extern __shared__ float smem[];
  const BlurTile tl = find_blur_tile(span, n_om, blockIdx.x);
  const OctMeta om = octs[tl.om];
  const int R = gt.rmax;
  const int GW = BT_W + 2 * R;
  const int GH = BT_H + 2 * R;
  float* grey = smem;
  float* colbuf = smem + GH * GW;
  const int x0 = tl.tx * BT_W, y0 = tl.ty * BT_H;
  const float* g0 = arena + om.gauss_off;
  const int tid = threadIdx.x;

  for (int i = tid; i < GH * GW; i += BT_THREADS) {
    int yy = i / GW, xx = i - yy * GW;
    int gy = min(max(y0 + yy - R, 0), om.h - 1);
    int gx = min(max(x0 + xx - R, 0), om.w - 1);
    grey[i] = __ldg(g0 + (size_t)gy * om.pitch + gx);
  }
  __syncthreads();

  const int tx = tid & (BT_W - 1), ty = tid / BT_W;
  for (int s = 0; s < gt.nlev; ++s) {
    const int c = gt.center[s];
    const float* taps = gt.taps[s];
    const int cw = BT_W + 2 * c;
    for (int i = tid; i < BT_H * cw; i += BT_THREADS) {
      int y = i / cw, xx = i - y * cw;
      const float* col = grey + (y + R - c) * GW + (xx + R - c);
      float tmp = 0.f;
      for (int k = 0; k <= 2 * c; ++k) tmp += col[k * GW] * taps[k];
      colbuf[y * GW + xx] = tmp;
    }
    __syncthreads();
    float* lvl = arena + om.gauss_off + (size_t)(s + 1) * om.plane;
#pragma unroll
    for (int i = 0; i < BT_H / 4; ++i) {
      int y = ty + 4 * i;
      const float* row = colbuf + y * GW + tx;
      float tmp = 0.f;
      for (int k = 0; k <= 2 * c; ++k) tmp += row[k] * taps[k];
      int gx = x0 + tx, gy = y0 + y;
      if (gx < om.w && gy < om.h) lvl[(size_t)gy * om.pitch + gx] = tmp;
    }
    __syncthreads();
  }
}

#define EX_RING_FLOATS (3 * BT_H * BT_W)
__global__ void __launch_bounds__(BT_THREADS, 3)
k_blur_extrema(const OctMeta* __restrict__ octs, const int2* __restrict__ span, int n_om, int n_tiles,
               const TmaDesc* __restrict__ maps, float* __restrict__ arena, const __grid_constant__ GaussTable gt,
               const ExtremaParams ep) {
  extern __shared__ __align__(128) float smem[];
  __shared__ __align__(8) uint64_t s_bar[2];
  __shared__ BlurTile s_tile[2];
  const int R = gt.rmax;
  const int RX = (R + 3) & ~3;
  const int GW = BT_W + 2 * RX, GH = BT_H + 2 * R;
  const int GSZ = (GH * GW + 31) & ~31;
  float* grey0 = smem;
  float* colbuf = smem + 2 * GSZ;
  float* outT = colbuf + BLUR_COLBUF_FLOATS(6);
  float* ring = outT + BT_H * (BT_W + 1);
  const int tid = threadIdx.x;
  const uint32_t tile_bytes = (uint32_t)(GH * GW * sizeof(float));
  int t = blockIdx.x;
  if (tid == 0) {
    sbar_init(sm_u32(&s_bar[0]), 1);
    sbar_init(sm_u32(&s_bar[1]), 1);
    asm volatile("fence.mbarrier_init.release.cluster;" ::: "memory");
    if (t < n_tiles) {
      const BlurTile tl = find_blur_tile(span, n_om, t);
      s_tile[0] = tl;
      sbar_expect_tx(sm_u32(&s_bar[0]), tile_bytes);
      tma_load_2d(sm_u32(grey0), maps + tl.om, tl.tx * BT_W - RX, tl.ty * BT_H - R, sm_u32(&s_bar[0]));
    }
  }
  __syncthreads();
  for (int it = 0; t < n_tiles; t += gridDim.x, ++it) {
    const int b = it & 1;
    float* grey = grey0 + b * GSZ;
    const BlurTile tl = s_tile[b];
    const OctMeta om = octs[tl.om];
    const int x0 = tl.tx * BT_W, y0 = tl.ty * BT_H;
    if (tid == 0 && t + (int)gridDim.x < n_tiles) {
      const BlurTile nx = find_blur_tile(span, n_om, t + gridDim.x);
      s_tile[b ^ 1] = nx;
      asm volatile("fence.proxy.async.shared::cta;" ::: "memory");
      sbar_expect_tx(sm_u32(&s_bar[b ^ 1]), tile_bytes);
      tma_load_2d(sm_u32(grey0 + (b ^ 1) * GSZ), maps + nx.om, nx.tx * BT_W - RX, nx.ty * BT_H - R, sm_u32(&s_bar[b ^ 1]));
    }
    sbar_wait(sm_u32(&s_bar[b]), (uint32_t)(it >> 1) & 1u);
    if (x0 - RX < 0 || y0 - R < 0 || x0 + BT_W + RX > om.w || y0 + BT_H + R > om.h) {
      for (int i = tid; i < GH * GW; i += BT_THREADS) {
        const int yy = i / GW, xx = i - yy * GW;
        const int gy = y0 + yy - R, gx = x0 + xx - RX;
        const int cy = min(max(gy, 0), om.h - 1), cx = min(max(gx, 0), om.w - 1);
        if (cy != gy || cx != gx) grey[i] = grey[(cy - y0 + R) * GW + (cx - x0 + RX)];
      }
      __syncthreads();
    }
    const int tx = tid & (BT_W - 1), ty = tid / BT_W;
    const int gx = x0 + tx;
    const bool col_in = gx >= 1 && gx <= om.w - 2;
    const bool col_seam = tx == 0 || tx == BT_W - 1;
    float prev[BT_H / 4];
#pragma unroll
    for (int i = 0; i < BT_H / 4; ++i) prev[i] = grey[(ty + 4 * i + R) * GW + tx + RX];
    for (int s = 0; s < gt.nlev; ++s) {
      if (gt.center[s] == 3) blur_level<3>(grey, colbuf, outT, gt.taps[s], R, RX, GW, tid);
      else blur_level<6>(grey, colbuf, outT, gt.taps[s], R, RX, GW, tid);
      float* lvl = arena + om.gauss_off + (size_t)(s + 1) * om.plane;
      float* dog = ring + (s % 3) * (BT_H * BT_W);
#pragma unroll
      for (int i = 0; i < BT_H / 4; ++i) {
        const int y = ty + 4 * i, gy = y0 + y;
        const float v = outT[y * (BT_W + 1) + tx];
        if (gx < om.w && gy < om.h) lvl[(size_t)gy * om.pitch + gx] = v;
        dog[y * BT_W + tx] = fabsf(prev[i] - v);
        prev[i] = v;
      }
      if (s >= 2) {
        __syncthreads();
        const int j = s - 1;
        const float* d0 = ring + ((s - 2) % 3) * (BT_H * BT_W);
        const float* d1 = ring + ((s - 1) % 3) * (BT_H * BT_W);
        const float* d2 = dog;
#pragma unroll 1
        for (int i = 0; i < BT_H / 4; ++i) {
          const int y = ty + 4 * i, gy = y0 + y;
          if (!col_in || gy < 1 || gy > om.h - 2) continue;
          const int o = y * BT_W + tx;
          const float center = d1[o];
          if (center < ep.pre_color_thres) continue;
          if (col_seam || y == 0 || y == BT_H - 1) {
            const int slot = atomicAdd(&ep.seam_count[om.img], 1);
            if (slot < ep.seam_cap) ep.seam_keys[(size_t)om.img * ep.seam_cap + slot] = make_key(om.oct, j, gy, gx);
            continue;
          }
          auto at = [&](int ds, int di, int dj) {
            const float* d = ds < 0 ? d0 : ds == 0 ? d1 : d2;
            return d[o + di * BT_W + dj];
          };
          if (is_extremum(center, ep.pre_color_thres, ep.diff_thres, at))
            append_candidate(ep, om.img, make_key(om.oct, j, gy, gx));
        }
      }
    }
    __syncthreads();
  }
}

__device__ __forceinline__ void test_from_levels(const ExtremaParams& ep, const OctMeta& om, const float* arena,
                                                 int j, int gy, int gx, float center) {
  const float* c = arena + om.gauss_off + (size_t)gy * om.pitch + gx;
  auto at = [&](int ds, int di, int dj) {
    const float* q = c + (ptrdiff_t)(j + ds) * om.plane + (ptrdiff_t)di * om.pitch + dj;
    return fabsf(__ldg(q) - __ldg(q + om.plane));
  };
  if (is_extremum(center, ep.pre_color_thres, ep.diff_thres, at))
    append_candidate(ep, om.img, make_key(om.oct, j, gy, gx));
}

__global__ void __launch_bounds__(256)
k_extrema_seams(const OctMeta* __restrict__ octs, int n_oct, const float* __restrict__ arena, const ExtremaParams ep) {
  const int img = blockIdx.y;
  const int n = min(ep.seam_count[img], ep.seam_cap);
  for (int i = blockIdx.x * blockDim.x + threadIdx.x; i < n; i += gridDim.x * blockDim.x) {
    const uint32_t key = ep.seam_keys[(size_t)img * ep.seam_cap + i];
    const int oct = key >> 29, j = (key >> 26) & 7, gy = (key >> 13) & 8191, gx = key & 8191;
    const OctMeta om = octs[img * n_oct + oct];
    const float* c = arena + om.gauss_off + (size_t)gy * om.pitch + gx;
    test_from_levels(ep, om, arena, j, gy, gx, fabsf(__ldg(c + (size_t)j * om.plane) - __ldg(c + (size_t)(j + 1) * om.plane)));
  }
}

#define EXS_THREADS 192

__global__ void __launch_bounds__(EXS_THREADS, 6)
k_extrema_scan(const OctMeta* __restrict__ octs, const int2* __restrict__ span, int n_om,
               const float* __restrict__ arena, const ExtremaParams ep) {
  const BlurTile tl = find_blur_tile(span, n_om, blockIdx.x);
  const OctMeta om = octs[tl.om];
  const int x0 = tl.tx * BT_W, y0 = tl.ty * BT_H;
  for (int p = threadIdx.x; p < BT_W * BT_H; p += EXS_THREADS) {
    const int gx = x0 + (p & (BT_W - 1)), gy = y0 + p / BT_W;
    if (gx < 1 || gx > om.w - 2 || gy < 1 || gy > om.h - 2) continue;
    const float* c = arena + om.gauss_off + (size_t)gy * om.pitch + gx;
    float lv[SIFT_MAX_LEVELS];
#pragma unroll
    for (int l = 1; l < SIFT_MAX_LEVELS; ++l) lv[l] = l <= ep.nscale - 2 ? __ldg(c + (size_t)l * om.plane) : 0.f;
#pragma unroll
    for (int j = 1; j < SIFT_MAX_LEVELS - 1; ++j) {
      if (j >= ep.nscale - 2) break;
      test_from_levels(ep, om, arena, j, gy, gx, fabsf(lv[j] - lv[j + 1]));
    }
  }
}

__global__ void __launch_bounds__(256)
k_rank_sort(const int* __restrict__ cand_count, const uint32_t* __restrict__ keys,
            uint32_t* __restrict__ sorted, int cap) {
  __shared__ uint32_t sk[1024];
  const int img = blockIdx.y;
  const int n = min(cand_count[img], cap);
  const uint32_t* k = keys + (size_t)img * cap;
  for (int c0 = blockIdx.x * 256; c0 < n; c0 += gridDim.x * 256) {
    const int i = c0 + threadIdx.x;
    uint32_t mine = i < n ? k[i] : 0xffffffffu;
    int rank = 0;
    for (int base = 0; base < n; base += 1024) {
      int m = min(1024, n - base);
      __syncthreads();
      for (int t = threadIdx.x; t < m; t += blockDim.x) sk[t] = k[base + t];
      __syncthreads();
      for (int t = 0; t < m; ++t) rank += sk[t] < mine;
    }
    if (i < n) sorted[(size_t)img * cap + rank] = mine;
  }
}

__device__ bool lu3_inverse(const double* a_in, double* inv) {
  double a[9];
  int rowperm[3] = {0, 1, 2}, colperm[3] = {0, 1, 2};
  int nonzero = 3, rank = 0;
  double maxpivot = 0.0;
  for (int i = 0; i < 9; ++i) a[i] = a_in[i];
  for (int k = 0; k < 3; ++k) {
    int br = k, bc = k;
    double big = -1.0;
    for (int i = k; i < 3; ++i)
      for (int j = k; j < 3; ++j) {
        double v = fabs(a[i * 3 + j]);
        if (v > big) { big = v; br = i; bc = j; }
      }
    if (big == 0.0) { nonzero = k; break; }
    if (big > maxpivot) maxpivot = big;
    if (br != k) {
      for (int j = 0; j < 3; ++j) { double w = a[k * 3 + j]; a[k * 3 + j] = a[br * 3 + j]; a[br * 3 + j] = w; }
      int t = rowperm[k]; rowperm[k] = rowperm[br]; rowperm[br] = t;
    }
    if (bc != k) {
      for (int i = 0; i < 3; ++i) { double w = a[i * 3 + k]; a[i * 3 + k] = a[i * 3 + bc]; a[i * 3 + bc] = w; }
      int t = colperm[k]; colperm[k] = colperm[bc]; colperm[bc] = t;
    }
    for (int i = k + 1; i < 3; ++i) a[i * 3 + k] /= a[k * 3 + k];
    for (int i = k + 1; i < 3; ++i)
      for (int j = k + 1; j < 3; ++j) a[i * 3 + j] -= a[i * 3 + k] * a[k * 3 + j];
  }
  double thr = 2.2204460492503131e-16 * 3.0 * maxpivot;
  for (int k = 0; k < nonzero; ++k) if (fabs(a[k * 3 + k]) > thr) ++rank;
  if (rank < 3) return false;
  for (int col = 0; col < 3; ++col) {
    double c[3];
    for (int i = 0; i < 3; ++i) c[i] = rowperm[i] == col ? 1.0 : 0.0;
    c[1] -= a[3] * c[0];
    c[2] -= a[6] * c[0];
    c[2] -= a[7] * c[1];
    c[2] /= a[8];
    c[1] -= a[5] * c[2];
    c[0] -= a[2] * c[2];
    c[1] /= a[4];
    c[0] -= a[1] * c[1];
    c[0] /= a[0];
    for (int i = 0; i < 3; ++i) inv[colperm[i] * 3 + col] = c[i];
  }
  return true;
}

__device__ void sym3_pinv(const double* a_in, double* out) {
  double a[9], v[9] = {1, 0, 0, 0, 1, 0, 0, 0, 1};
  for (int i = 0; i < 9; ++i) a[i] = a_in[i];
  for (int sweep = 0; sweep < 32; ++sweep) {
    double off = fabs(a[1]) + fabs(a[2]) + fabs(a[5]);
    if (off < 1e-300) break;
    for (int p = 0; p < 2; ++p)
      for (int q = p + 1; q < 3; ++q) {
        double apq = a[p * 3 + q];
        if (apq == 0.0) continue;
        double theta = (a[q * 3 + q] - a[p * 3 + p]) / (2.0 * apq);
        double t = (theta >= 0 ? 1.0 : -1.0) / (fabs(theta) + sqrt(theta * theta + 1.0));
        double c = 1.0 / sqrt(t * t + 1.0);
        double s = t * c;
        for (int k = 0; k < 3; ++k) {
          double akp = a[k * 3 + p], akq = a[k * 3 + q];
          a[k * 3 + p] = c * akp - s * akq;
          a[k * 3 + q] = s * akp + c * akq;
        }
        for (int k = 0; k < 3; ++k) {
          double apk = a[p * 3 + k], aqk = a[q * 3 + k];
          a[p * 3 + k] = c * apk - s * aqk;
          a[q * 3 + k] = s * apk + c * aqk;
        }
        for (int k = 0; k < 3; ++k) {
          double vkp = v[k * 3 + p], vkq = v[k * 3 + q];
          v[k * 3 + p] = c * vkp - s * vkq;
          v[k * 3 + q] = s * vkp + c * vkq;
        }
      }
  }
  for (int i = 0; i < 3; ++i)
    for (int j = 0; j < 3; ++j) {
      double acc = 0.0;
      for (int k = 0; k < 3; ++k) {
        double l = a[k * 3 + k];
        if (fabs(l) > 1e-6) acc += v[i * 3 + k] * (1.0 / l) * v[j * 3 + k];
      }
      out[i * 3 + j] = acc;
    }
}

struct RefineParams {
  int nscale, depth;
  float offset_thres, contrast_thres, edge_ratio, gauss_sigma, scale_factor;
};

__global__ void k_refine(const OctMeta* __restrict__ octs, const float* __restrict__ arena, int n_oct,
                         const int* __restrict__ cand_count, const uint32_t* __restrict__ sorted,
                         RefineParams rp, int cap, pano_sspoint* __restrict__ out, unsigned char* __restrict__ valid) {
  const int img = blockIdx.y;
  const int n = min(cand_count[img], cap);
  for (int i = blockIdx.x * blockDim.x + threadIdx.x; i < n; i += gridDim.x * blockDim.x) {
  const size_t slot = (size_t)img * cap + i;
  uint32_t key = sorted[slot];
  int oct = key >> 29, s0 = (key >> 26) & 7, y0 = (key >> 13) & 8191, x0 = key & 8191;
  const OctMeta om = octs[img * n_oct + oct];
  const float* gauss = arena + om.gauss_off;
  const int w = om.w, h = om.h;
  auto dog_at = [&](int xx, int yy, int ss) {
    const float* q = gauss + (size_t)ss * om.plane + (size_t)yy * om.pitch + xx;
    return fabsf(__ldg(q) - __ldg(q + om.plane));
  };
#define DG(xx, yy, ss) dog_at(xx, yy, ss)
  pano_sspoint sp;
  sp.x = x0; sp.y = y0; sp.pyr_id = oct; sp.scale_id = s0;
  sp.real_x = 0; sp.real_y = 0; sp.dir = 0; sp.scale_factor = 0;
  bool ok = true;
  int nowx = x0, nowy = y0, nows = s0, niter = 0;
  double offset[3] = {0, 0, 0}, delta[3] = {0, 0, 0};
  for (; niter < rp.depth; ++niter) {
    if (!DBETWEEN(nowx, 1, w - 1) || !DBETWEEN(nowy, 1, h - 1) || !DBETWEEN(nows, 1, rp.nscale - 2)) {
      ok = false; break;
    }
    const int x = nowx, y = nowy, s = nows;
    float val = DG(x, y, s);
    delta[0] = (double)((DG(x + 1, y, s) - DG(x - 1, y, s)) / 2);
    delta[1] = (double)((DG(x, y + 1, s) - DG(x, y - 1, s)) / 2);
    delta[2] = (double)((DG(x, y, s + 1) - DG(x, y, s - 1)) / 2);
    double dxx = (double)(DG(x + 1, y, s) + DG(x - 1, y, s) - val - val);
    double dyy = (double)(DG(x, y + 1, s) + DG(x, y - 1, s) - val - val);
    double dss = (double)(DG(x, y, s + 1) + DG(x, y, s - 1) - val - val);
    double dxy = (double)((DG(x + 1, y + 1, s) - DG(x + 1, y - 1, s) - DG(x - 1, y + 1, s) + DG(x - 1, y - 1, s)) / 4);
    double dys = (double)((DG(x, y + 1, s + 1) - DG(x, y - 1, s + 1) - DG(x, y + 1, s - 1) + DG(x, y - 1, s - 1)) / 4);
    double dsx = (double)((DG(x + 1, y, s + 1) - DG(x - 1, y, s + 1) - DG(x + 1, y, s - 1) + DG(x - 1, y, s - 1)) / 4);
    double m[9] = {dxx, dxy, dsx, dxy, dyy, dys, dsx, dys, dss}, inv[9];
    if (!lu3_inverse(m, inv)) sym3_pinv(m, inv);
    for (int q = 0; q < 3; ++q) {
      double acc = inv[q * 3] * delta[0];
      acc += inv[q * 3 + 1] * delta[1];
      acc += inv[q * 3 + 2] * delta[2];
      offset[q] = acc;
    }
    double am = fmax(fabs(offset[0]), fmax(fabs(offset[1]), fabs(offset[2])));
    if (am < (double)rp.offset_thres) break;
    nowx = (int)((double)nowx + round(offset[0]));
    nowy = (int)((double)nowy + round(offset[1]));
    nows = (int)((double)nows + round(offset[2]));
  }
  if (ok && niter == rp.depth) ok = false;
  if (ok) {
    double dextr = offset[0] * delta[0] + offset[1] * delta[1] + offset[2] * delta[2];
    dextr = (double)DG(nowx, nowy, nows) + dextr / 2;
    if (dextr < (double)rp.contrast_thres) ok = false;
  }
  if (ok) {
    sp.x = nowx; sp.y = nowy; sp.scale_id = nows;
    sp.scale_factor = (float)((double)rp.gauss_sigma *
                              pow((double)rp.scale_factor, ((double)nows + offset[2]) / rp.nscale));
    sp.real_x = ((double)nowx + offset[0]) / w;
    sp.real_y = ((double)nowy + offset[1]) / h;
    const int x = nowx, y = nowy, s = nows;
    float val = DG(x, y, s);
    float dxx = DG(x + 1, y, s) + DG(x - 1, y, s) - val - val;
    float dyy = DG(x, y + 1, s) + DG(x, y - 1, s) - val - val;
    float dxy = (DG(x + 1, y + 1, s) + DG(x - 1, y - 1, s) - DG(x - 1, y + 1, s) - DG(x + 1, y - 1, s)) / 4;
    float det = dxx * dyy - dxy * dxy;
    if (det <= 0) ok = false;
    else {
      float tr2 = (dxx + dyy) * (dxx + dyy);
      float lim = ((rp.edge_ratio + 1) * (rp.edge_ratio + 1)) / rp.edge_ratio;
      if (!(tr2 / det < lim)) ok = false;
    }
  }
#undef DG
  out[slot] = sp;
  valid[slot] = ok ? 1 : 0;
  }
}

#define ORI_BINS 36
#define ORI_WARPS 4

#define SIFT_MAX_IMG PANO_MAX_SIFT_BATCH

#define ORI_QUADS 8
__global__ void __launch_bounds__(ORI_WARPS * 32)
k_orientation(const OctMeta* __restrict__ octs, const float* __restrict__ arena, int n_oct, int n_img, int cap,
              const int* __restrict__ cand_count, const pano_sspoint* __restrict__ pts,
              const unsigned char* __restrict__ valid, float ori_radius, int smooth_count,
              int* __restrict__ npeaks, float* __restrict__ dirs, int* __restrict__ work_counter) {
  __shared__ float s_hist[ORI_WARPS][ORI_BINS][ORI_QUADS];
  __shared__ uint64_t s_exptab[32];
  __shared__ int s_pref[SIFT_MAX_IMG + 1];
  load_exp2f_tab(s_exptab, threadIdx.x);
  if (threadIdx.x == 0) {
    int acc = 0;
    for (int i = 0; i < n_img; ++i) { s_pref[i] = acc; acc += min(cand_count[i], cap); }
    s_pref[n_img] = acc;
  }
  __syncthreads();
  const unsigned FULL = 0xffffffffu;
  const int wid = threadIdx.x >> 5, lane = threadIdx.x & 31;
  const int g = lane >> 2, l = lane & 3;
  const int total_work = s_pref[n_img];
  float* hist = &s_hist[wid][0][g];
  const float halfipi = (float)(0.5 / PANO_PI);
  int img = 0;
  while (true) {
    int flat = 0;
    if (lane == 0) flat = atomicAdd(work_counter, ORI_QUADS);
    flat = __shfl_sync(FULL, flat, 0);
    if (flat >= total_work) break;
    flat += g;
    bool live = flat < total_work;
    size_t slot = 0;
    int px = 0, py = 0, w = 0, h = 0, pitch = 0, rad = 0;
    float exp_denom = 1.f;
    const float* lvl = arena;
    if (live) {
      while (flat >= s_pref[img + 1]) ++img;
      slot = (size_t)img * cap + (flat - s_pref[img]);
      if (!valid[slot]) {
        if (l == 0) npeaks[slot] = 0;
        live = false;
      } else {
        const pano_sspoint p = pts[slot];
        const OctMeta om = octs[img * n_oct + p.pyr_id];
        lvl = arena + om.gauss_off + (size_t)p.scale_id * om.plane;
        px = p.x; py = p.y; w = om.w; h = om.h; pitch = om.pitch;
        const float gws = p.scale_factor * 1.5f;
        rad = (int)roundf(p.scale_factor * ori_radius);
        exp_denom = 2 * (gws * gws);
      }
    }
    const float fr2 = (float)rad * (float)rad;
    const int side = 2 * rad, total = side * side;
    for (int b = l; b < ORI_BINS; b += 4) hist[b * ORI_QUADS] = 0.f;
    __syncwarp();
    const int total_mx = __reduce_max_sync(FULL, total);
    int xx = -rad, yy = -rad + l;
    if (side > 0) while (yy >= rad) { yy -= side; ++xx; }
    for (int base = 0; base < total_mx; base += 4) {
      int bin = -1;
      float val = 0.f;
      if (base + l < total) {
        const int newx = px + xx, newy = py + yy;
        if (DBETWEEN(newx, 1, w - 1) && DBETWEEN(newy, 1, h - 1)) {
          const float fx = (float)xx, fy = (float)yy;
          const float d2 = fx * fx + fy * fy;
          if (!(d2 > fr2)) {
            float mag, ort;
            mag_ort_at(lvl, pitch, newx, newy, &mag, &ort);
            int b = (int)roundf((float)ORI_BINS * halfipi * ort);
            if (b == ORI_BINS) b = 0;
            const float weight = glibc_expf(-d2 / exp_denom, s_exptab);
            bin = b;
            val = weight * mag;
          }
        }
        yy += 4;
        while (yy >= rad) { yy -= side; ++xx; }
      }
#pragma unroll
      for (int j = 0; j < 4; ++j) {
        if (l == j && bin >= 0) hist[bin * ORI_QUADS] = hist[bin * ORI_QUADS] + val;
        __syncwarp();
      }
    }
    if (l == 0 && live) {
      for (int K = smooth_count; K--;)
        for (int b = 0; b < ORI_BINS; ++b) {
          float prev = hist[(b == 0 ? ORI_BINS - 1 : b - 1) * ORI_QUADS];
          float next = hist[(b == ORI_BINS - 1 ? 0 : b + 1) * ORI_QUADS];
          hist[b * ORI_QUADS] = (float)((double)hist[b * ORI_QUADS] * 0.5 + (double)(prev + next) * 0.25);
        }
    }
    __syncwarp();
    if (live) {
      float mx = 0.f;
      for (int b = 0; b < ORI_BINS; ++b) if (mx < hist[b * ORI_QUADS]) mx = hist[b * ORI_QUADS];
      const float thres = mx * 0.8f;
      float my_dir[5];
      int mine = 0;
      for (int b = l * 9; b < l * 9 + 9; ++b) {
        const float hb = hist[b * ORI_QUADS];
        const float prev = hist[(b == 0 ? ORI_BINS - 1 : b - 1) * ORI_QUADS];
        const float next = hist[(b == ORI_BINS - 1 ? 0 : b + 1) * ORI_QUADS];
        if (hb > thres && hb > (prev < next ? next : prev)) {
          double newbin = (double)(float)b - 0.5 + (double)((hb - prev) / (prev + next - 2 * hb));
          if (newbin < 0) newbin += ORI_BINS;
          else if (newbin >= ORI_BINS) newbin -= ORI_BINS;
          const float dir = (float)(newbin / ORI_BINS * 2 * PANO_PI);
          if (mine < 5) my_dir[mine] = dir;
          ++mine;
        }
      }
      const unsigned qmask = 0xfu << (g * 4);
      int before = 0;
      const int m0 = __shfl_sync(qmask, mine, g * 4 + 0), m1 = __shfl_sync(qmask, mine, g * 4 + 1),
                m2 = __shfl_sync(qmask, mine, g * 4 + 2), m3 = __shfl_sync(qmask, mine, g * 4 + 3);
      if (l > 0) before += m0;
      if (l > 1) before += m1;
      if (l > 2) before += m2;
      for (int k = 0; k < mine && k < 5; ++k)
        if (before + k < SIFT_MAX_PEAKS) dirs[slot * SIFT_MAX_PEAKS + before + k] = my_dir[k];
      if (l == 0) npeaks[slot] = min(m0 + m1 + m2 + m3, SIFT_MAX_PEAKS);
    }
    __syncwarp();
  }
}

#define SCAN_THREADS 1024
__global__ void __launch_bounds__(SCAN_THREADS)
k_expand_scan(const int* __restrict__ cand_count, const unsigned char* __restrict__ valid,
              const int* __restrict__ npeaks, const float* __restrict__ dirs, int cap,
              int* __restrict__ n_desc, int* __restrict__ n_refined,
              int* __restrict__ desc_cand, float* __restrict__ desc_dir) {
  __shared__ int s_warp[32];
  __shared__ int s_warp2[32];
  const int img = blockIdx.x;
  const int n = min(cand_count[img], cap);
  const int per = (n + SCAN_THREADS - 1) / SCAN_THREADS;
  const int tid = threadIdx.x, lane = tid & 31, wid = tid >> 5;
  const size_t base = (size_t)img * cap;
  int local = 0, nval = 0;
  for (int k = 0; k < per; ++k) {
    int i = tid * per + k;
    if (i < n && valid[base + i]) { local += npeaks[base + i]; nval++; }
  }
  int incl = local, incl2 = nval;
  for (int d = 1; d < 32; d <<= 1) {
    int t = __shfl_up_sync(0xffffffffu, incl, d);
    int t2 = __shfl_up_sync(0xffffffffu, incl2, d);
    if (lane >= d) { incl += t; incl2 += t2; }
  }
  if (lane == 31) { s_warp[wid] = incl; s_warp2[wid] = incl2; }
  __syncthreads();
  if (wid == 0) {
    int v = s_warp[lane], v2 = s_warp2[lane];
    int a = v, a2 = v2;
    for (int d = 1; d < 32; d <<= 1) {
      int t = __shfl_up_sync(0xffffffffu, a, d);
      int t2 = __shfl_up_sync(0xffffffffu, a2, d);
      if (lane >= d) { a += t; a2 += t2; }
    }
    s_warp[lane] = a - v;
    s_warp2[lane] = a2;
  }
  __syncthreads();
  int off = s_warp[wid] + incl - local;
  for (int k = 0; k < per; ++k) {
    int i = tid * per + k;
    if (i < n && valid[base + i]) {
      int np = npeaks[base + i];
      for (int q = 0; q < np; ++q) {
        int d = off + q;
        if (d < cap) {
          desc_cand[(size_t)img * cap + d] = i;
          desc_dir[(size_t)img * cap + d] = dirs[(base + i) * SIFT_MAX_PEAKS + q];
        }
      }
      off += np;
    }
  }
  if (tid == SCAN_THREADS - 1) { n_desc[img] = off; n_refined[img] = s_warp2[31]; }
}

#define DESC_WARPS 4
#define DESC_THREADS (DESC_WARPS * 32)

struct DescParams { int hist_scale_factor; int int_factor; };

#define DQ_COLS 96

struct __align__(16) DescQuadSmem {
  float acc[32 * 32];
  float r_q[4][32];
  float2 r_h[4][8];
  unsigned char col_len[8][DQ_COLS];
  signed char col_y0[8][DQ_COLS];
};

#ifndef DESC_MIN_CTAS
#define DESC_MIN_CTAS 6
#endif
__global__ void __launch_bounds__(DESC_THREADS, DESC_MIN_CTAS)
k_descriptor(const OctMeta* __restrict__ octs, const ImgMeta* __restrict__ imgs,
             const float* __restrict__ arena, int n_oct, int n_img, int cap,
             const pano_sspoint* __restrict__ pts, const int* __restrict__ n_desc,
             const int* __restrict__ desc_cand, const float* __restrict__ desc_dir,
             DescParams dp, float* __restrict__ out_desc, double* __restrict__ out_coor,
             int* __restrict__ work_counter) {
  extern __shared__ __align__(16) unsigned char desc_smem_raw[];
  __shared__ uint64_t s_exptab[32];
  __shared__ int s_pref[SIFT_MAX_IMG + 1];
  load_exp2f_tab(s_exptab, threadIdx.x);
  if (threadIdx.x == 0) {
    int acc = 0;
    for (int i = 0; i < n_img; ++i) { s_pref[i] = acc; acc += min(n_desc[i], cap); }
    s_pref[n_img] = acc;
  }
  __syncthreads();
  const unsigned FULL = 0xffffffffu;
  const int lane = threadIdx.x & 31, wid = threadIdx.x >> 5;
  const int g = lane >> 2, l = lane & 3;
  DescQuadSmem& S = reinterpret_cast<DescQuadSmem*>(desc_smem_raw)[wid];
  float* const acc = S.acc + lane;
  const float pi2 = (float)(2 * PANO_PI);
  const float nbin_per_rad = 8 / pi2;
  const float exp_denom = 2 * (4.f * 4.f);
  const int hi_shift = 4 + 2 * l;
  const int total = s_pref[n_img];
  int img = 0;
  while (true) {
    int flat = 0;
    if (lane == 0) flat = atomicAdd(work_counter, 8);
    flat = __shfl_sync(FULL, flat, 0);
    if (flat >= total) break;
    flat += g;
    const bool live = flat < total;

    int px = 0, py = 0, w = 0, h = 0, pitch = 0, radius = 0, side = 0;
    float ort = 0.f, hist_w = 1.f, sinort = 0.f, cosort = 1.f;
    const float* lvl = arena;
    size_t dslot = 0, pslot = 0;
    if (live) {
      while (flat >= s_pref[img + 1]) ++img;
      dslot = (size_t)img * cap + (flat - s_pref[img]);
      pslot = (size_t)img * cap + desc_cand[dslot];
      const pano_sspoint p = pts[pslot];
      ort = desc_dir[dslot];
      const OctMeta om = octs[img * n_oct + p.pyr_id];
      lvl = arena + om.gauss_off + (size_t)p.scale_id * om.plane;
      px = p.x; py = p.y; w = om.w; h = om.h; pitch = om.pitch;
      hist_w = p.scale_factor * (float)dp.hist_scale_factor;
      radius = (int)round(PANO_SQRT1_2 * (double)hist_w * (4 + 1));
      glibc_sincosf(ort, &sinort, &cosort);
      side = 2 * radius + 1;
    }
    const float fr2 = (float)radius * (float)radius;
    const float lo = -2.5f * hist_w - 0.02f * hist_w - 1e-3f, hi = 1.5f * hist_w + 0.02f * hist_w + 1e-3f;
#pragma unroll
    for (int k = 0; k < 32; ++k) acc[32 * k] = 0.f;

    const int side_mx = __reduce_max_sync(FULL, side);
    for (int cb = 0; cb < side_mx; cb += DQ_COLS) {
      int nblk = 0;
      const int ncol_mx = min(DQ_COLS, side_mx - cb);
      for (int c0 = 0; c0 < ncol_mx; c0 += 4) {
        const int c = c0 + l;
        int len = 0;
        if (c < DQ_COLS && cb + c < side) {
          int y0, y1;
          desc_col_interval(cb + c - radius, radius, px, py, w, h, sinort, cosort, lo, hi, &y0, &y1);
          len = max(0, y1 - y0 + 1);
          S.col_len[g][c] = (unsigned char)len;
          S.col_y0[g][c] = (signed char)y0;
        }
        len += __shfl_xor_sync(FULL, len, 1);
        len += __shfl_xor_sync(FULL, len, 2);
        nblk += len;
      }
      __syncwarp();
      const int nblk_mx = __reduce_max_sync(FULL, nblk);
      int col = 0, cstart = 0, clen = nblk > 0 ? (int)S.col_len[g][0] : 0;

      for (int base = 0; base < nblk_mx; base += 4) {
        const int s = base + l;
        float q0 = 0.f, q1 = 0.f, q2 = 0.f, q3 = 0.f, hd = 0.f;
        uint32_t pk = 0;
        if (s < nblk) {
          while (s >= cstart + clen) { cstart += clen; ++col; clen = (int)S.col_len[g][col]; }
          const int xx = cb + col - radius, yy = (int)S.col_y0[g][col] + (s - cstart);
          const int nowx = px + xx, nowy = py + yy;
          const float fx = (float)xx, fy = (float)yy;
          if (DBETWEEN(nowx, 1, w - 1) && DBETWEEN(nowy, 1, h - 1) && !(fx * fx + fy * fy > fr2)) {
            const float y_rot = ((float)(-xx) * sinort + fy * cosort) / hist_w;
            const float x_rot = (fx * cosort + fy * sinort) / hist_w;
            const float ybin = (float)((double)(y_rot + 2.f) - 0.5);
            const float xbin = (float)((double)(x_rot + 2.f) - 0.5);
            if (ybin >= -1.f && ybin <= 3.f && xbin >= -1.f && xbin <= 3.f) {
              float now_mag, now_ort;
              mag_ort_at(lvl, pitch, nowx, nowy, &now_mag, &now_ort);
              float weight = glibc_expf(-(x_rot * x_rot + y_rot * y_rot) / exp_denom, s_exptab);
              weight = weight * now_mag;
              now_ort -= ort;
              if (now_ort < 0) now_ort += pi2;
              if (now_ort > pi2) now_ort -= pi2;
              const float hbin = now_ort * nbin_per_rad;
              const int ybinf = (int)floorf(ybin), xbinf = (int)floorf(xbin), hbinf = (int)floorf(hbin);
              const float yd = ybin - (float)ybinf, xd = xbin - (float)xbinf;
              hd = hbin - (float)hbinf;
              const float wy_lo = weight * (1 - yd), wy_hi = weight * yd;
              const float fx_lo = 1 - xd, fx_hi = xd;
              const int yodd = ybinf & 1, xodd = xbinf & 1;
              const int cy0 = ybinf + yodd, cy1 = ybinf + 1 - yodd;
              const int cx0 = xbinf + xodd, cx1 = xbinf + 1 - xodd;
              const bool vy0 = (unsigned)cy0 <= 3u, vy1 = (unsigned)cy1 <= 3u;
              const bool vx0 = (unsigned)cx0 <= 3u, vx1 = (unsigned)cx1 <= 3u;
              const float wy0 = yodd ? wy_hi : wy_lo, wy1 = yodd ? wy_lo : wy_hi;
              const float fx0 = xodd ? fx_hi : fx_lo, fx1 = xodd ? fx_lo : fx_hi;
              q0 = (vy0 && vx0) ? wy0 * fx0 : 0.f;
              q1 = (vy0 && vx1) ? wy0 * fx1 : 0.f;
              q2 = (vy1 && vx0) ? wy1 * fx0 : 0.f;
              q3 = (vy1 && vx1) ? wy1 * fx1 : 0.f;
              const uint32_t hy0 = vy0 ? (uint32_t)(cy0 >> 1) : 0u, hy1 = vy1 ? (uint32_t)(cy1 >> 1) : 0u;
              const uint32_t hx0 = vx0 ? (uint32_t)(cx0 >> 1) : 0u, hx1 = vx1 ? (uint32_t)(cx1 >> 1) : 0u;
              pk = (uint32_t)hbinf | ((hy0 * 2 + hx0) << 4) | ((hy0 * 2 + hx1) << 6) | ((hy1 * 2 + hx0) << 8) | ((hy1 * 2 + hx1) << 10);
            }
          }
        }
        *reinterpret_cast<float4*>(&S.r_q[l][g * 4]) = make_float4(q0, q1, q2, q3);
        S.r_h[l][g] = make_float2(hd, __uint_as_float(pk));
        __syncwarp();
#pragma unroll
        for (int j = 0; j < 4; ++j) {
          const float q = S.r_q[j][lane];
          const float2 hh = S.r_h[j][g];
          const uint32_t word = __float_as_uint(hh.y);
          const float v0 = q * (1 - hh.x), v1 = q * hh.x;
          const uint32_t cell_hi = (word >> hi_shift) & 3u;
          float* a0 = acc + 32 * ((word & 7u) * 4 + cell_hi);
          float* a1 = acc + 32 * (((word + 1u) & 7u) * 4 + cell_hi);
          *a0 = *a0 + v0;
          *a1 = *a1 + v1;
        }
        __syncwarp();
      }
    }

    __syncwarp();
    const float* qacc = S.acc + g * 4;
    float sum = 0.f;
    if (l == 0) {
      for (int c = 0; c < 16; ++c) {
        const int cy = c >> 2, cx = c & 3;
        const float* a = qacc + ((cy & 1) * 2 + (cx & 1)) + 32 * ((cy >> 1) * 2 + (cx >> 1));
#pragma unroll
        for (int b = 0; b < 8; ++b) sum += a[32 * 4 * b];
      }
    }
    sum = __shfl_sync(FULL, sum, g * 4);
    if (live) {
      const float fac = (float)dp.int_factor;
#pragma unroll
      for (int k = 0; k < 8; ++k) {
        const int e = l * 4 + 16 * k;
        const int c = e >> 3, b = e & 7, cy = c >> 2, cx = c & 3;
        const float* a = qacc + ((cy & 1) * 2 + (cx & 1)) + 32 * ((cy >> 1) * 2 + (cx >> 1));
        float4 o;
        o.x = sqrtf(a[32 * 4 * (b + 0)] / sum) * fac;
        o.y = sqrtf(a[32 * 4 * (b + 1)] / sum) * fac;
        o.z = sqrtf(a[32 * 4 * (b + 2)] / sum) * fac;
        o.w = sqrtf(a[32 * 4 * (b + 3)] / sum) * fac;
        *reinterpret_cast<float4*>(out_desc + dslot * 128 + e) = o;
      }
      if (l == 0) {
        const pano_sspoint p = pts[pslot];
        const ImgMeta im = imgs[img];
        out_coor[dslot * 2] = (p.real_x - 0.5) * im.in_w;
        out_coor[dslot * 2 + 1] = (p.real_y - 0.5) * im.in_h;
        double* out_real = out_coor + (size_t)n_img * cap * 2;
        out_real[dslot * 2] = p.real_x;
        out_real[dslot * 2 + 1] = p.real_y;
      }
    }
    __syncwarp();
  }
}

#define PANO_SQRT1_2_HOST 0.70710678118654752440

int host_gauss_kernel(float sigma, int window_factor, float* taps, int cap) {
  int kw = (int)(ceil(0.3 * (sigma / 2 - 1) + 0.8) * window_factor);
  if (kw % 2 == 0) kw++;
  if (kw > cap) return -kw;
  const int center = kw / 2;
  float* k = taps + center;
  k[0] = 1;
  float exp_coeff = (float)(-1.0 / (sigma * sigma * 2)), wsum = 1;
  for (int i = 1; i <= center; i++) {
    k[i] = expf((float)(i * i) * exp_coeff);
    wsum += k[i] * 2;
  }
  float fac = (float)(1.0 / wsum);
  k[0] = fac;
  for (int i = 1; i <= center; i++) { k[i] *= fac; k[-i] = k[i]; }
  return kw;
}

typedef CUresult (*tma_encode_fn)(CUtensorMap*, CUtensorMapDataType, cuuint32_t, void*, const cuuint64_t*,
                                  const cuuint64_t*, const cuuint32_t*, const cuuint32_t*, CUtensorMapInterleave,
                                  CUtensorMapSwizzle, CUtensorMapL2promotion, CUtensorMapFloatOOBfill);

int ctx_tma_encode(pano_ctx* ctx, TmaDesc* out, void* base, int rank, const unsigned long long* dims,
                   const unsigned long long* strides_bytes, const unsigned* box) {
  SlowCall sc("ctx_tma_encode");
  if (!ctx->tma_encode) {
    void* fn = nullptr;
    cudaDriverEntryPointQueryResult q;
    cudaError_t e = cudaGetDriverEntryPoint("cuTensorMapEncodeTiled", &fn, cudaEnableDefault, &q);
    if (e != cudaSuccess || q != cudaDriverEntryPointSuccess || !fn)
      return ctx_fail(ctx, PANO_ERR_CUDA, "cuTensorMapEncodeTiled is not available from this driver");
    ctx->tma_encode = fn;
  }
  cuuint64_t gd[5], gs[5];
  cuuint32_t bx[5], es[5];
  for (int i = 0; i < rank; ++i) { gd[i] = dims[i]; bx[i] = box[i]; es[i] = 1; }
  for (int i = 0; i + 1 < rank; ++i) gs[i] = strides_bytes[i];
  static_assert(sizeof(TmaDesc) == sizeof(CUtensorMap), "CUtensorMap is 128 bytes");
  CUresult r = ((tma_encode_fn)ctx->tma_encode)((CUtensorMap*)out, CU_TENSOR_MAP_DATA_TYPE_FLOAT32, (cuuint32_t)rank, base, gd,
                                                gs, bx, es, CU_TENSOR_MAP_INTERLEAVE_NONE, CU_TENSOR_MAP_SWIZZLE_NONE,
                                                CU_TENSOR_MAP_L2_PROMOTION_L2_128B, CU_TENSOR_MAP_FLOAT_OOB_FILL_NONE);
  if (r != CUDA_SUCCESS) return ctx_fail(ctx, PANO_ERR_CUDA, "cuTensorMapEncodeTiled failed (%d)", (int)r);
  return PANO_OK;
}

static std::vector<int> sift_plan_key(int n, const int* channels, const int* w, const int* h, const pano_params* p,
                                      int cap) {
  static_assert(sizeof(pano_params) % sizeof(int) == 0, "pano_params holds 4-byte fields only");
  std::vector<int> key;
  key.reserve(2 + 3 * (size_t)n + sizeof(pano_params) / sizeof(int));
  key.push_back(n);
  key.push_back(cap);
  for (int i = 0; i < n; ++i) {
    key.push_back(w[i]);
    key.push_back(h[i]);
    key.push_back(channels ? channels[i] : 0);
  }
  const size_t at = key.size();
  key.resize(at + sizeof(pano_params) / sizeof(int));
  memcpy(key.data() + at, p, sizeof(pano_params));
  return key;
}

template <class T>
static int plan_alloc(pano_ctx* ctx, SiftPlan* plan, DevBuf<T>& buf, size_t count) {
  const int rc = buf.alloc(ctx, count);
  if (rc == PANO_OK) {
    auto f = ctx->live.find(buf.get());
    plan->bytes += f != ctx->live.end() ? f->second : count * sizeof(T);
  }
  return rc;
}

static cudaError_t sift_smem_limit(pano_ctx* ctx, const void* fn, size_t bytes) {
  static std::mutex mu;
  static std::map<std::pair<int, const void*>, size_t> set;
  std::lock_guard<std::mutex> lock(mu);
  size_t& cur = set[std::make_pair(ctx->device, fn)];
  if (bytes <= cur) return cudaSuccess;
  const cudaError_t e = cudaFuncSetAttribute(fn, cudaFuncAttributeMaxDynamicSharedMemorySize, (int)bytes);
  if (e == cudaSuccess) cur = bytes;
  return e;
}

int sift_run_batch(pano_ctx* ctx, int n, const void* const* d_src, const int* channels, const int* w, const int* h,
                   const pano_params* p, pano_featureset* fs, std::unique_ptr<SiftWork>* keep, int cap) {
  if (n <= 0 || !d_src || !w || !h || !p || !fs) return ctx_fail(ctx, PANO_ERR_INVALID, "sift: bad argument");
  if (n > SIFT_MAX_IMG) return ctx_fail(ctx, PANO_ERR_INVALID, "sift: %d images in one batch (limit %d): split the batch", n, SIFT_MAX_IMG);
  const int n_oct = p->num_octave, n_scale = p->num_scale;
  if (n_oct < 1 || n_oct > SIFT_MAX_OCT || n_scale < 4 || n_scale - 1 > SIFT_MAX_LEVELS || n_scale - 2 > 7)
    return ctx_fail(ctx, PANO_ERR_INVALID, "sift: NUM_OCTAVE/NUM_SCALE out of supported range");
  if (cap < 256 || cap > SIFT_CAP_MAX) return ctx_fail(ctx, PANO_ERR_INVALID, "sift: list capacity %d out of range", cap);
  {
    const double e_lo = (1.0 - (double)p->offset_thres) / n_scale;
    const double e_hi = (n_scale - 3.0 + (double)p->offset_thres) / n_scale;
    const double sf_max = (double)p->gauss_sigma * std::max(pow((double)p->scale_factor, e_lo), pow((double)p->scale_factor, e_hi));
    const double rad_max = PANO_SQRT1_2_HOST * sf_max * (double)p->desc_hist_scale_factor * 5.0;
    if (!(rad_max <= 127.0))
      return ctx_fail(ctx, PANO_ERR_INVALID, "sift: descriptor windows of up to %.0f pixels radius (limit 127): lower DESC_HIST_SCALE_FACTOR / GAUSS_SIGMA", rad_max);
  }

  std::vector<int> key = sift_plan_key(n, channels, w, h, p, cap);
  std::unique_ptr<SiftPlan> plan;
  if (!keep) {
    plan = std::move(ctx->sift_plan);
    if (plan && plan->key != key) plan.reset();
  }
  const bool fresh = plan == nullptr;

  std::vector<int2> tilespan;
  if (fresh) {
    plan.reset(new SiftPlan);
    plan->key = std::move(key);
    plan->wk.reset(new SiftWork);
    SiftWork* wk = plan->wk.get();
    wk->n_img = n; wk->n_oct = n_oct; wk->n_scale = n_scale; wk->cap = cap;
    wk->h_img.resize(n);
    wk->h_oct.resize((size_t)n * n_oct);
    size_t off = 0;
    int max_w0 = 0, max_h0 = 0;
    int n_tiles = 0;
    size_t seam_cap = 0;
    tilespan.resize((size_t)n * n_oct);
    for (int i = 0; i < n; ++i) {
      if (w[i] < 2 || h[i] < 2) return ctx_fail(ctx, PANO_ERR_INVALID, "sift: image too small");
      if (channels)
        if (int rc = pix8_check(ctx, "sift", i, channels[i], nullptr)) return rc;
      ImgMeta& im = wk->h_img[i];
      im.channels = channels ? channels[i] : 3;
      im.in_w = w[i]; im.in_h = h[i];
      float ratio = p->sift_working_size * 2.0f / (w[i] + h[i]);
      im.h0 = (int)(h[i] * ratio); im.w0 = (int)(w[i] * ratio);
      if (im.w0 < 8 || im.h0 < 8 || im.w0 > 8191 || im.h0 > 8191) return ctx_fail(ctx, PANO_ERR_INVALID, "sift: working size out of range");
      float fx = (float)im.h0 / h[i], fy = (float)im.w0 / w[i];
      im.ifx = 1.f / fx; im.ify = 1.f / fy;
      im.work_off = (long long)off;
      if (keep) off += align_up((size_t)im.w0 * im.h0 * 3, 32);
      max_w0 = std::max(max_w0, im.w0); max_h0 = std::max(max_h0, im.h0);
      size_t img_tiles = 0;
      for (int o = 0; o < n_oct; ++o) {
        OctMeta& om = wk->h_oct[(size_t)i * n_oct + o];
        om.img = i; om.oct = o;
        if (o == 0) { om.w = im.w0; om.h = im.h0; om.ifx = om.ify = 1.f; }
        else {
          float factor = (float)pow((double)p->scale_factor, (double)-o);
          om.w = (int)ceilf(im.w0 * factor); om.h = (int)ceilf(im.h0 * factor);
          if (om.w <= 5 || om.h <= 5) return ctx_fail(ctx, PANO_ERR_INVALID, "sift: octave too small");
          float ofx = (float)om.h / im.h0, ofy = (float)om.w / im.w0;
          om.ifx = 1.f / ofx; om.ify = 1.f / ofy;
        }
        om.pitch = (int)align_up((size_t)om.w, 32);
        om.plane = (long long)om.pitch * om.h;
        om.gauss_off = (long long)off; off += (size_t)om.plane * n_scale;
        tilespan[(size_t)i * n_oct + o] = make_int2(n_tiles, ceil_div(om.w, BT_W));
        n_tiles += ceil_div(om.w, BT_W) * ceil_div(om.h, BT_H);
        img_tiles += (size_t)ceil_div(om.w, BT_W) * ceil_div(om.h, BT_H);
      }
      seam_cap = std::max(seam_cap, img_tiles * (2 * BT_W + 2 * (BT_H - 2)) * (size_t)(n_scale - 3));
    }
    wk->arena_floats = off;
    wk->n_tiles = n_tiles;
    plan->seam_cap = seam_cap;
    plan->max_w0 = max_w0; plan->max_h0 = max_h0;

    GaussTable& gt = plan->gt;
    memset(&gt, 0, sizeof(gt));
    gt.nlev = n_scale - 1;
    {
      float sigma = p->gauss_sigma;
      for (int s = 0; s < gt.nlev; ++s) {
        int kw = host_gauss_kernel(sigma, p->gauss_window_factor, gt.taps[s], SIFT_MAX_TAPS);
        if (kw < 0) return ctx_fail(ctx, PANO_ERR_INVALID, "sift: gaussian window %d too wide", -kw);
        gt.center[s] = kw / 2;
        gt.rmax = std::max(gt.rmax, kw / 2);
        sigma *= p->scale_factor;
      }
    }
    plan->fast = true;
    for (int s = 0; s < gt.nlev; ++s) plan->fast = plan->fast && (gt.center[s] == 3 || gt.center[s] == 6);
    const int R = gt.rmax;
    if (((size_t)(BT_H + 2 * R) * (BT_W + 2 * R) + (size_t)BT_H * (BT_W + 2 * R)) * sizeof(float) > 200 * 1024)
      return ctx_fail(ctx, PANO_ERR_INVALID, "sift: blur halo too large");

    const size_t nlist = (size_t)n * cap;
    if (int rc = plan_alloc(ctx, plan.get(), wk->arena, off)) return rc;
    if (int rc = plan_alloc(ctx, plan.get(), wk->d_img, n)) return rc;
    if (int rc = plan_alloc(ctx, plan.get(), wk->d_oct, wk->h_oct.size())) return rc;
    if (int rc = plan_alloc(ctx, plan.get(), wk->d_maps, (size_t)n * n_oct)) return rc;
    if (int rc = plan_alloc(ctx, plan.get(), wk->d_tilespan, tilespan.size())) return rc;
    if (int rc = plan_alloc(ctx, plan.get(), wk->cand_count, 2 * n + 2)) return rc;
    if (int rc = plan_alloc(ctx, plan.get(), wk->seam_keys, (size_t)n * seam_cap)) return rc;
    if (int rc = plan_alloc(ctx, plan.get(), wk->cand_keys, nlist)) return rc;
    if (int rc = plan_alloc(ctx, plan.get(), wk->sorted_keys, nlist)) return rc;
    if (int rc = plan_alloc(ctx, plan.get(), wk->refined, nlist)) return rc;
    if (int rc = plan_alloc(ctx, plan.get(), wk->kp_valid, nlist)) return rc;
    if (int rc = plan_alloc(ctx, plan.get(), wk->npeaks, nlist)) return rc;
    if (int rc = plan_alloc(ctx, plan.get(), wk->dirs, nlist * SIFT_MAX_PEAKS)) return rc;
    if (int rc = plan_alloc(ctx, plan.get(), wk->n_refined, n)) return rc;
    if (int rc = plan_alloc(ctx, plan.get(), wk->desc_cand, nlist)) return rc;
    if (int rc = plan_alloc(ctx, plan.get(), wk->desc_dir, nlist)) return rc;
  }
  SiftWork* wk = plan->wk.get();
  const GaussTable& gt = plan->gt;
  const bool fast = plan->fast;
  const size_t seam_cap = plan->seam_cap;
  for (int i = 0; i < n; ++i) {
    if (channels) wk->h_img[i].pix = (const unsigned char*)d_src[i];
    else wk->h_img[i].src = (const float*)d_src[i];
  }

  const size_t nlist = (size_t)n * cap;
  const int n_om = n * n_oct;
  fs->ctx = ctx; fs->n_images = n; fs->cap = cap;
  if (int rc = fs->d_desc.alloc(ctx, nlist * 128)) return rc;
  if (int rc = fs->d_coor.alloc(ctx, nlist * 4)) return rc;
  fs->d_real = fs->d_coor + nlist * 2;
  if (int rc = fs->d_count.alloc(ctx, n)) return rc;
  fs->base.resize(n);
  for (int i = 0; i < n; ++i) fs->base[i] = (long long)i * cap;

  {
    void* dsts[4] = {wk->d_img, wk->cand_count, wk->d_oct, wk->d_tilespan};
    const void* srcs[4] = {wk->h_img.data(), nullptr, wk->h_oct.data(), tilespan.data()};
    size_t sizes[4] = {n * sizeof(ImgMeta), (2 * n + 2) * sizeof(int), wk->h_oct.size() * sizeof(OctMeta),
                       tilespan.size() * sizeof(int2)};
    if (int rc = ctx_put_many(ctx, fresh ? 4 : 2, dsts, srcs, sizes)) return rc;
  }
  if (fresh && fast) {
    std::vector<TmaDesc> maps(n_om);
    const int R = gt.rmax;
    for (int k = 0; k < n_om; ++k) {
      const OctMeta& om = wk->h_oct[k];
      unsigned long long dims[2] = {(unsigned long long)om.w, (unsigned long long)om.h};
      unsigned long long strides[1] = {(unsigned long long)om.pitch * sizeof(float)};
      unsigned box[2] = {(unsigned)(BT_W + 2 * ((R + 3) & ~3)), (unsigned)(BT_H + 2 * R)};
      if (int rc = ctx_tma_encode(ctx, &maps[k], wk->arena + om.gauss_off, 2, dims, strides, box)) return rc;
    }
    if (int rc = ctx_put(ctx, wk->d_maps, maps.data(), maps.size() * sizeof(TmaDesc))) return rc;
  }

  {
    dim3 g(ceil_div(plan->max_w0, PG_TW), ceil_div(plan->max_h0, PG_TH), n);
    float* work = keep ? wk->arena.get() : nullptr;
    if (channels && std::any_of(channels, channels + n, pix8_layout))
      PANO_LAUNCH(ctx, "k_pyramid_grey_pix8", k_pyramid_grey<SrcPix8>, g, PG_THREADS, 0, wk->d_img, wk->d_oct, n_oct, wk->arena, work);
    else if (channels)
      PANO_LAUNCH(ctx, "k_pyramid_grey_rgb8", k_pyramid_grey<SrcRgb8>, g, PG_THREADS, 0, wk->d_img, wk->d_oct, n_oct, wk->arena, work);
    else
      PANO_LAUNCH(ctx, "k_pyramid_grey", k_pyramid_grey<SrcF32>, g, PG_THREADS, 0, wk->d_img, wk->d_oct, n_oct, wk->arena, work);
  }
  {
    const ExtremaParams ep{n_scale, p->pre_color_thres, p->judge_extrema_diff_thres, cap, wk->cand_count, wk->cand_keys,
                           (int)seam_cap, wk->cand_count + n + 2, wk->seam_keys};
    const int R = gt.rmax;
    size_t smem = ((size_t)(BT_H + 2 * R) * (BT_W + 2 * R) + (size_t)BT_H * (BT_W + 2 * R)) * sizeof(float);
    if (fast) {
      const int GW = BT_W + 2 * ((R + 3) & ~3), GH = BT_H + 2 * R;
      const size_t gsz = ((size_t)GH * GW + 31) & ~(size_t)31;
      size_t smf = (2 * gsz + (size_t)BLUR_COLBUF_FLOATS(6) + (size_t)BT_H * (BT_W + 1) + EX_RING_FLOATS) * sizeof(float);
      PANO_CUDA(ctx, sift_smem_limit(ctx, (const void*)k_blur_extrema, smf));
      const int grid = std::min(wk->n_tiles, ctx->num_sms * 3);
      PANO_LAUNCH(ctx, "k_blur_extrema", k_blur_extrema, grid, BT_THREADS, smf, wk->d_oct, wk->d_tilespan, n_om, wk->n_tiles,
                  wk->d_maps, wk->arena, gt, ep);
      PANO_LAUNCH(ctx, "k_extrema_seams", k_extrema_seams, dim3(8, n), 256, 0, wk->d_oct, n_oct, wk->arena, ep);
    } else {
      if (smem > 48 * 1024)
        PANO_CUDA(ctx, sift_smem_limit(ctx, (const void*)k_blur_dog, smem));
      PANO_LAUNCH(ctx, "k_blur_dog_generic", k_blur_dog, wk->n_tiles, BT_THREADS, smem, wk->d_oct, wk->d_tilespan, n_om, wk->arena, gt);
      PANO_LAUNCH(ctx, "k_extrema_scan", k_extrema_scan, wk->n_tiles, EXS_THREADS, 0, wk->d_oct, wk->d_tilespan, n_om,
                  wk->arena, ep);
    }
  }
  {
    dim3 g(8, n);
    PANO_LAUNCH(ctx, "k_rank_sort", k_rank_sort, g, 256, 0, wk->cand_count, wk->cand_keys, wk->sorted_keys, cap);
    RefineParams rp{n_scale, p->calc_offset_depth, p->offset_thres, p->contrast_thres, p->edge_ratio,
                    p->gauss_sigma, p->scale_factor};
    dim3 g4(16, n);
    PANO_LAUNCH(ctx, "k_refine", k_refine, g4, 128, 0, wk->d_oct, wk->arena, n_oct, wk->cand_count, wk->sorted_keys, rp, cap,
                wk->refined, wk->kp_valid);
    PANO_LAUNCH(ctx, "k_orientation", k_orientation, ctx->num_sms * 8, ORI_WARPS * 32, 0, wk->d_oct, wk->arena, n_oct, n, cap,
                wk->cand_count, wk->refined, wk->kp_valid, p->ori_radius, p->ori_hist_smooth_count, wk->npeaks, wk->dirs,
                wk->cand_count + n + 1);
    PANO_LAUNCH(ctx, "k_expand_scan", k_expand_scan, n, SCAN_THREADS, 0, wk->cand_count, wk->kp_valid, wk->npeaks,
                wk->dirs, cap, fs->d_count, wk->n_refined, wk->desc_cand, wk->desc_dir);
    DescParams dp{p->desc_hist_scale_factor, p->desc_int_factor};
    const size_t dsm = sizeof(DescQuadSmem) * DESC_WARPS;
    PANO_CUDA(ctx, sift_smem_limit(ctx, (const void*)k_descriptor, dsm));
    const int grid = ctx->num_sms * DESC_MIN_CTAS;
    PANO_LAUNCH(ctx, "k_descriptor", k_descriptor, grid, DESC_THREADS, dsm, wk->d_oct, wk->d_img, wk->arena, n_oct, n, cap,
                wk->refined, fs->d_count, wk->desc_cand, wk->desc_dir, dp, fs->d_desc, fs->d_coor, wk->cand_count + n);
  }
  wk->n_desc = fs->d_count;

  if (!fs->h_count_pinned.get()) {
    fs->h_count_pinned = ctx_small_pinned_get(ctx, (size_t)2 * n * sizeof(int) + 16);
    if (!fs->h_count_pinned.get()) return ctx_fail(ctx, PANO_ERR_CUDA, "pinned allocation failed");
  }
  {
    int* h_counts = (int*)fs->h_count_pinned.get();
    void* dsts[2] = {h_counts, h_counts + n};
    const void* srcs[2] = {fs->d_count, wk->cand_count};
    size_t sizes[2] = {n * sizeof(int), n * sizeof(int)};
    if (int rc = ctx_store_many(ctx, 2, dsts, srcs, sizes)) return rc;
  }
  PANO_CUDA(ctx, ctx_signal(ctx, &fs->counts_token));
  fs->counts_pending = true;
  fs->counts_on_host = false;

  if (keep) {
    *keep = std::move(plan->wk);
  } else if (ctx->cache_limit && plan->bytes <= ctx->cache_limit) {
    ctx->sift_plan = std::move(plan);
    if (ctx->cached_bytes + ctx->sift_plan->bytes > ctx->cache_limit) ctx_cache_release(ctx, ctx->cache_limit - ctx->sift_plan->bytes);
  }
  return PANO_OK;
}


int featureset_sync_counts(pano_featureset* fs) {
  SlowCall sc("featureset_sync_counts");
  if (fs->error) return fs->error;
  if (fs->counts_on_host) return PANO_OK;
  pano_ctx* ctx = fs->ctx;
  while (fs->counts_pending) {
    cudaError_t e = ctx_wait_signal(ctx, fs->counts_token);
    if (e != cudaSuccess) return fs->error = ctx_cuda(ctx, e, "feature count read-back");
    fs->counts_pending = false;
    const int n = fs->n_images;
    const int* h_counts = (const int*)fs->h_count_pinned.get();
    int worst = 0;
    for (int i = 0; i < n; ++i) worst = std::max(worst, std::max(h_counts[i], h_counts[n + i]));
    if (worst <= fs->cap) {
      fs->h_count.assign(h_counts, h_counts + n);
      break;
    }
    int cap = fs->cap;
    while (cap < worst && cap < SIFT_CAP_MAX) cap *= 2;
    if (cap < worst || fs->src.empty())
      return fs->error = ctx_fail(ctx, PANO_ERR_CAPACITY, "sift: %d list entries in one image exceed the capacity %d", worst, fs->cap);
    fs->d_desc.reset(); fs->d_coor.reset(); fs->d_count.reset();
    fs->d_real = nullptr;
    ctx->sift_cap = cap;
    const std::vector<const void*> src = fs->src;
    const std::vector<int> channels = fs->src_channels;
    int rc = sift_run_batch(ctx, n, src.data(), channels.empty() ? nullptr : channels.data(), fs->src_w.data(),
                            fs->src_h.data(), &fs->src_params, fs, nullptr, cap);
    if (rc) return fs->error = rc;
  }
  fs->owned_block.reset();
  fs->counts_on_host = true;
  return PANO_OK;
}
```

Baseline: 11210.

## Add programmatic dependent launch and fuse match planning, fallback, and filter splitting

Adds a launch macro that sets programmatic stream serialization, and has many SIFT and matching kernels call griddepcontrol.wait. This lets each kernel's launch and prologue overlap the tail of the kernel before it. It also folds the gather planning into k_match_decide through a last-block ticket, and folds the exact-rescan fallback into k_exact_cands, which removes separate launches. It splits filter tasks across column partitions to raise parallelism. The cost is extra complexity, last-block atomics, and possible ordering hazards if any kernel reads predecessor output before its wait.

Measured after the change: 11540 (median of 6 runs). +2.9%, better.

```diff
diff --git a/openpano_b200/csrc/common.cuh b/openpano_b200/csrc/common.cuh
--- a/openpano_b200/csrc/common.cuh
+++ b/openpano_b200/csrc/common.cuh
@@ -196,6 +196,31 @@
     if (_e != cudaSuccess) return ctx_cuda((ctx), _e, name);                        \
   } while (0)
 
+#define PANO_LAUNCH_PDL(ctx, name, kernel, grid, block, smem, ...)                  \
+  do {                                                                              \
+    (ctx)->launches++;                                                              \
+    if ((ctx)->profiling) ctx_prof_begin((ctx), (name));                            \
+    cudaError_t _e;                                                                 \
+    {                                                                               \
+      SlowCall _sc(name);                                                           \
+      cudaLaunchAttribute _at[1];                                                   \
+      _at[0].id = cudaLaunchAttributeProgrammaticStreamSerialization;               \
+      _at[0].val.programmaticStreamSerializationAllowed = 1;                        \
+      cudaLaunchConfig_t _cfg = {};                                                 \
+      _cfg.gridDim = dim3(grid); _cfg.blockDim = dim3(block);                       \
+      _cfg.dynamicSmemBytes = (smem); _cfg.stream = (ctx)->stream;                  \
+      _cfg.attrs = _at; _cfg.numAttrs = 1;                                          \
+      _e = cudaLaunchKernelEx(&_cfg, kernel, __VA_ARGS__);                          \
+    }                                                                               \
+    if ((ctx)->profiling) ctx_prof_end((ctx));                                      \
+    if (_e == cudaSuccess) _e = cudaGetLastError();                                 \
+    if (_e != cudaSuccess) return ctx_cuda((ctx), _e, name);                        \
+  } while (0)
+
+#ifdef __CUDACC__
+__device__ __forceinline__ void pdl_wait() { asm volatile("griddepcontrol.wait;" ::: "memory"); }
+#endif
+
 struct __align__(64) TmaDesc { unsigned long long opaque[16]; };
 int ctx_tma_encode(pano_ctx* ctx, TmaDesc* out, void* base, int rank, const unsigned long long* dims,
                    const unsigned long long* strides_bytes, const unsigned* box);
diff --git a/openpano_b200/csrc/match.cu b/openpano_b200/csrc/match.cu
--- a/openpano_b200/csrc/match.cu
+++ b/openpano_b200/csrc/match.cu
@@ -192,6 +192,7 @@
                          const unsigned* __restrict__ maxnorm_bits, const SideMeta* __restrict__ sides, int n_sides,
                          TcTop2* __restrict__ approx, long long res_total, float ratio_sqr, int lazy,
                          RowInfo* __restrict__ info) {
+  pdl_wait();
   const int r = blockIdx.x * blockDim.x + threadIdx.x;
   for (int side = blockIdx.y; side < n_sides; side += gridDim.y)
     refine_side_row(desc, norms, maxnorm_bits, sides, approx, res_total, ratio_sqr, lazy, info, side, r);
@@ -202,6 +203,7 @@
                                   const int2* __restrict__ g_meta, const TcTop2* __restrict__ g_approx,
                                   const int* __restrict__ n_blocks, float ratio_sqr, TcTop2* __restrict__ approx,
                                   RowInfo* __restrict__ info) {
+  pdl_wait();
   const int g = blockIdx.x * blockDim.x + threadIdx.x;
   if (g >= *n_blocks * 128) return;
   const int2 me = g_meta[g];
@@ -213,53 +215,48 @@
   info[sm.res_off + me.y] = refine_row(desc, sm, me.y, ap, tc_eps(norms[sm.q_base + me.y], nmax), ratio_sqr);
 }
 
-__global__ void __launch_bounds__(256)
-k_exact_rows(const float* __restrict__ desc, const SideMeta* __restrict__ sides, const int2* __restrict__ list,
-             const int* __restrict__ list_count, RowInfo* __restrict__ info) {
+__device__ __forceinline__ void exact_rescan_row(const float* __restrict__ desc, const SideMeta* __restrict__ sides,
+                                                 const int2 it, RowInfo* __restrict__ info) {
   __shared__ __align__(16) float sq[128];
   __shared__ float s_mn[8], s_sec[8];
   __shared__ int s_idx[8];
   const int tid = threadIdx.x, lane = tid & 31, wid = tid >> 5;
-  const int n = *list_count;
-  for (int e = blockIdx.x; e < n; e += gridDim.x) {
-    const int2 it = list[e];
-    const SideMeta sm = sides[it.x];
-    const float* q = desc + (size_t)(sm.q_base + it.y) * 128;
-    __syncthreads();
-    if (tid < 32) *(float4*)(&sq[tid * 4]) = __ldg((const float4*)q + tid);
-    __syncthreads();
-    float mn = FLT_MAX, sec = FLT_MAX;
-    int idx = 0x7fffffff;
-    for (int c = tid; c < sm.t_n; c += 256) {
-      const float4* pb = (const float4*)(desc + (size_t)(sm.t_base + c) * 128);
-      float4 yv[32];
-#pragma unroll
-      for (int k = 0; k < 32; ++k) yv[k] = __ldg(pb + k);
-      float l0 = 0.f, l1 = 0.f, l2 = 0.f, l3 = 0.f;
-#pragma unroll
-      for (int k = 0; k < 32; ++k) {
-        const float4 x = *(const float4*)(&sq[k * 4]), y = yv[k];
-        float d0 = x.x - y.x, d1 = x.y - y.y, d2 = x.z - y.z, d3 = x.w - y.w;
-        l0 += d0 * d0; l1 += d1 * d1; l2 += d2 * d2; l3 += d3 * d3;
-      }
-      float d = (l0 + l1) + (l2 + l3);
-      if (d < mn) { sec = mn; mn = d; idx = c; }
-      else if (d < sec) sec = d;
-    }
-#pragma unroll
-    for (int off = 16; off >= 1; off >>= 1) {
-      float m2 = __shfl_xor_sync(0xffffffffu, mn, off);
-      float s2 = __shfl_xor_sync(0xffffffffu, sec, off);
-      int i2 = __shfl_xor_sync(0xffffffffu, idx, off);
-      top2_merge(mn, idx, sec, m2, i2, s2);
-    }
-    if (lane == 0) { s_mn[wid] = mn; s_sec[wid] = sec; s_idx[wid] = idx; }
-    __syncthreads();
-    if (tid == 0) {
-      for (int wdx = 1; wdx < 8; ++wdx) top2_merge(mn, idx, sec, s_mn[wdx], s_idx[wdx], s_sec[wdx]);
-      RowInfo o; o.mn = mn; o.mn_hi = mn; o.idx = idx; o.sec_lo = sec; o.sec_hi = sec; o.state = 3; o.requested = 1; o.pad = 0;
-      info[sm.res_off + it.y] = o;
-    }
+  const SideMeta sm = sides[it.x];
+  const float* q = desc + (size_t)(sm.q_base + it.y) * 128;
+  __syncthreads();
+  if (tid < 32) *(float4*)(&sq[tid * 4]) = __ldg((const float4*)q + tid);
+  __syncthreads();
+  float mn = FLT_MAX, sec = FLT_MAX;
+  int idx = 0x7fffffff;
+  for (int c = tid; c < sm.t_n; c += 256) {
+    const float4* pb = (const float4*)(desc + (size_t)(sm.t_base + c) * 128);
+    float4 yv[32];
+#pragma unroll
+    for (int k = 0; k < 32; ++k) yv[k] = __ldg(pb + k);
+    float l0 = 0.f, l1 = 0.f, l2 = 0.f, l3 = 0.f;
+#pragma unroll
+    for (int k = 0; k < 32; ++k) {
+      const float4 x = *(const float4*)(&sq[k * 4]), y = yv[k];
+      float d0 = x.x - y.x, d1 = x.y - y.y, d2 = x.z - y.z, d3 = x.w - y.w;
+      l0 += d0 * d0; l1 += d1 * d1; l2 += d2 * d2; l3 += d3 * d3;
+    }
+    float d = (l0 + l1) + (l2 + l3);
+    if (d < mn) { sec = mn; mn = d; idx = c; }
+    else if (d < sec) sec = d;
+  }
+#pragma unroll
+  for (int off = 16; off >= 1; off >>= 1) {
+    float m2 = __shfl_xor_sync(0xffffffffu, mn, off);
+    float s2 = __shfl_xor_sync(0xffffffffu, sec, off);
+    int i2 = __shfl_xor_sync(0xffffffffu, idx, off);
+    top2_merge(mn, idx, sec, m2, i2, s2);
+  }
+  if (lane == 0) { s_mn[wid] = mn; s_sec[wid] = sec; s_idx[wid] = idx; }
+  __syncthreads();
+  if (tid == 0) {
+    for (int wdx = 1; wdx < 8; ++wdx) top2_merge(mn, idx, sec, s_mn[wdx], s_idx[wdx], s_sec[wdx]);
+    RowInfo o; o.mn = mn; o.mn_hi = mn; o.idx = idx; o.sec_lo = sec; o.sec_hi = sec; o.state = 3; o.requested = 1; o.pad = 0;
+    info[sm.res_off + it.y] = o;
   }
 }
 
@@ -341,125 +338,192 @@
   if (result >= 0) atomicAdd(total, 1);
 }
 
+#define FILTER_PART_TILES 4
+#define TC_FILTER_PARTS 8
+
+__device__ void plan_gather_list(const TcGatherSide* __restrict__ gsides, int n_sides, const int* side_cnt,
+                                 const int* list_rows, int block_cap, int fill, TcTask* __restrict__ tasks,
+                                 int* n_blocks, int* n_tasks, int2* __restrict__ fb_list, int* fb_cnt) {
+  __shared__ int s_blocks;
+  int parts = 1;
+  if (fill > 0) {
+    if (threadIdx.x == 0) s_blocks = 0;
+    __syncthreads();
+    for (int side = threadIdx.x; side < n_sides; side += blockDim.x) {
+      const int cnt = __ldcg(side_cnt + side);
+      if (cnt) atomicAdd(&s_blocks, (cnt + 127) / 128);
+    }
+    __syncthreads();
+    if (s_blocks > 0) parts = max(1, min(TC_FILTER_PARTS, fill / s_blocks));
+  }
+  for (int side = threadIdx.x; side < n_sides; side += blockDim.x) {
+    const int cnt = __ldcg(side_cnt + side);
+    if (cnt == 0) continue;
+    const TcGatherSide gs = gsides[side];
+    const int nb = (cnt + 127) / 128;
+    const int b0 = atomicAdd(n_blocks, nb);
+    if (b0 + nb > block_cap) {
+      atomicSub(n_blocks, nb);
+      const int f0 = atomicAdd(fb_cnt, cnt);
+      for (int i = 0; i < cnt; ++i) fb_list[f0 + i] = make_int2(side, __ldcg(list_rows + gs.list_off + i));
+      continue;
+    }
+    const int tiles = gs.t_blocks / 2;
+    const int np = max(1, min(parts, tiles / FILTER_PART_TILES));
+    const int t0 = n_tasks ? atomicAdd(n_tasks, nb * np) : b0;
+    for (int i = 0; i < nb; ++i)
+      for (int p = 0; p < np; ++p) {
+        const int c0 = tiles * p / np, c1 = tiles * (p + 1) / np;
+        TcTask t;
+        t.q_blk = b0 + i; t.q_row0 = (b0 + i) * 128; t.q_n = min(128, cnt - i * 128);
+        t.t_blk0 = gs.t_blk0 + 2 * c0; t.t_blocks = 2 * (c1 - c0); t.t_n = gs.t_n; t.t_pad = i * 128;
+        t.res_off = side; t.f_col0 = c0 * 256; t.f_pad = 0;
+        tasks[t0 + i * np + p] = t;
+      }
+  }
+}
+
+struct GatherPlan {
+  const TcGatherSide* gsides;
+  int* ticket;
+  int2* fb_list; int* fb_cnt;
+  int block_cap, fill;
+  TcTask* tasks; int* n_blocks; int* n_tasks;
+  int nom_cap; TcTask* nom_tasks; int* nom_blocks;
+};
+
 __global__ void k_match_decide(const PairMeta* __restrict__ pairs, int n_pairs, const SideMeta* __restrict__ sides,
                                RowInfo* __restrict__ info, float ratio_sqr, int first_round,
                                int* __restrict__ out, int* __restrict__ total,
                                int* list_rows, int* list_unknown, int* __restrict__ side_cnt,
-                               int n_sides) {
+                               int n_sides, const GatherPlan plan) {
+  __shared__ int s_last;
+  pdl_wait();
   const int row = blockIdx.x * blockDim.x + threadIdx.x;
   for (int pair = blockIdx.y; pair < n_pairs; pair += gridDim.y)
     match_decide_row(pairs, sides, info, ratio_sqr, first_round, out, total, list_rows, list_unknown, side_cnt, n_sides,
                      pair, row);
-}
-
-__global__ void k_gather_plan(const TcGatherSide* __restrict__ gsides, int n_sides, const int* __restrict__ side_cnt,
-                              const int* __restrict__ list_rows, int block_cap, TcTask* __restrict__ tasks,
-                              int* __restrict__ n_blocks, int2* __restrict__ fb_list, int* __restrict__ fb_cnt) {
-  const int side = blockIdx.x * blockDim.x + threadIdx.x;
-  if (side >= n_sides) return;
-  const int cnt = side_cnt[side];
-  if (cnt == 0) return;
-  const TcGatherSide gs = gsides[side];
-  const int nb = (cnt + 127) / 128;
-  const int b0 = atomicAdd(n_blocks, nb);
-  if (b0 + nb > block_cap) {
-    atomicSub(n_blocks, nb);
-    const int f0 = atomicAdd(fb_cnt, cnt);
-    for (int i = 0; i < cnt; ++i) fb_list[f0 + i] = make_int2(side, list_rows[gs.list_off + i]);
-    return;
-  }
-  for (int i = 0; i < nb; ++i) {
-    TcTask t;
-    t.q_blk = b0 + i; t.q_row0 = (b0 + i) * 128; t.q_n = min(128, cnt - i * 128);
-    t.t_blk0 = gs.t_blk0; t.t_blocks = gs.t_blocks; t.t_n = gs.t_n; t.t_pad = i * 128;
-    t.res_off = side;
-    tasks[b0 + i] = t;
-  }
+  if (!plan.ticket) return;
+  __threadfence();
+  __syncthreads();
+  if (threadIdx.x == 0) s_last = atomicAdd(plan.ticket, 1) == (int)(gridDim.x * gridDim.y) - 1;
+  __syncthreads();
+  if (!s_last) return;
+  __threadfence();
+  if (plan.nom_tasks)
+    plan_gather_list(plan.gsides, n_sides, side_cnt + n_sides, list_unknown, plan.nom_cap, 0, plan.nom_tasks,
+                     plan.nom_blocks, nullptr, plan.fb_list, plan.fb_cnt);
+  __syncthreads();
+  plan_gather_list(plan.gsides, n_sides, side_cnt, list_rows, plan.block_cap, plan.fill, plan.tasks, plan.n_blocks,
+                   plan.n_tasks, plan.fb_list, plan.fb_cnt);
+}
+
+__device__ __forceinline__ bool exact_cand_row(const float* __restrict__ desc, const SideMeta* __restrict__ sides,
+                                               const int2 me, int g, const int* __restrict__ cand_cnt,
+                                               const int* __restrict__ cand, RowInfo* __restrict__ info) {
+  const int lane = threadIdx.x & 31;
+  const SideMeta sm = sides[me.x];
+  const int cnt = cand_cnt[g];
+  if (cnt > TC_CAND_CAP || cnt < 1 || (cnt < 2 && sm.t_n >= 2)) return false;
+  float mn = FLT_MAX, sec = FLT_MAX;
+  int idx = 0x7fffffff;
+  if (lane < cnt) {
+    idx = cand[(size_t)g * TC_CAND_CAP + lane];
+    mn = exact_dist(desc + (size_t)(sm.q_base + me.y) * 128, desc + (size_t)(sm.t_base + idx) * 128);
+  }
+#pragma unroll
+  for (int off = 16; off >= 1; off >>= 1) {
+    float m2 = __shfl_xor_sync(0xffffffffu, mn, off);
+    float s2 = __shfl_xor_sync(0xffffffffu, sec, off);
+    int i2 = __shfl_xor_sync(0xffffffffu, idx, off);
+    top2_merge(mn, idx, sec, m2, i2, s2);
+  }
+  if (lane == 0) {
+    RowInfo o; o.mn = mn; o.mn_hi = mn; o.idx = idx; o.sec_lo = sec; o.sec_hi = sec; o.state = 3; o.requested = 1; o.pad = 0;
+    info[sm.res_off + me.y] = o;
+  }
+  return true;
 }
 
 __global__ void __launch_bounds__(256)
 k_exact_cands(const float* __restrict__ desc, const SideMeta* __restrict__ sides, const int* __restrict__ n_blocks,
               const int2* __restrict__ g_meta, const int* __restrict__ cand_cnt, const int* __restrict__ cand,
-              RowInfo* __restrict__ info, int2* __restrict__ fb_list, int* __restrict__ fb_cnt) {
-  const int lane = threadIdx.x & 31;
+              RowInfo* __restrict__ info, const int2* __restrict__ fb_list, const int* __restrict__ fb_cnt,
+              int* __restrict__ overflow_cnt) {
+  __shared__ int2 s_over[8];
+  __shared__ int s_n_over;
+  pdl_wait();
+  const int lane = threadIdx.x & 31, warp = threadIdx.x >> 5;
   const int nrow = *n_blocks * 128;
-  for (int g = blockIdx.x * 8 + (threadIdx.x >> 5); g < nrow; g += gridDim.x * 8) {
-    const int2 me = g_meta[g];
-    if (me.x < 0) continue;
-    const SideMeta sm = sides[me.x];
-    const int cnt = cand_cnt[g];
-    if (cnt > TC_CAND_CAP || cnt < 1 || (cnt < 2 && sm.t_n >= 2)) {
-      if (lane == 0) fb_list[atomicAdd(fb_cnt, 1)] = me;
-      continue;
-    }
-    float mn = FLT_MAX, sec = FLT_MAX;
-    int idx = 0x7fffffff;
-    if (lane < cnt) {
-      idx = cand[(size_t)g * TC_CAND_CAP + lane];
-      mn = exact_dist(desc + (size_t)(sm.q_base + me.y) * 128, desc + (size_t)(sm.t_base + idx) * 128);
-    }
-#pragma unroll
-    for (int off = 16; off >= 1; off >>= 1) {
-      float m2 = __shfl_xor_sync(0xffffffffu, mn, off);
-      float s2 = __shfl_xor_sync(0xffffffffu, sec, off);
-      int i2 = __shfl_xor_sync(0xffffffffu, idx, off);
-      top2_merge(mn, idx, sec, m2, i2, s2);
-    }
-    if (lane == 0) {
-      RowInfo o; o.mn = mn; o.mn_hi = mn; o.idx = idx; o.sec_lo = sec; o.sec_hi = sec; o.state = 3; o.requested = 1; o.pad = 0;
-      info[sm.res_off + me.y] = o;
-    }
-  }
+  for (int g0 = blockIdx.x * 8; g0 < nrow; g0 += gridDim.x * 8) {
+    if (threadIdx.x == 0) s_n_over = 0;
+    __syncthreads();
+    const int g = g0 + warp;
+    if (g < nrow) {
+      const int2 me = g_meta[g];
+      if (me.x >= 0 && !exact_cand_row(desc, sides, me, g, cand_cnt, cand, info) && lane == 0) {
+        s_over[atomicAdd(&s_n_over, 1)] = me;
+        atomicAdd(overflow_cnt, 1);
+      }
+    }
+    __syncthreads();
+    const int n_over = s_n_over;
+    for (int o = 0; o < n_over; ++o) exact_rescan_row(desc, sides, s_over[o], info);
+    __syncthreads();
+  }
+  const int n_fb = *fb_cnt;
+  for (int e = blockIdx.x; e < n_fb; e += gridDim.x) exact_rescan_row(desc, sides, fb_list[e], info);
 }
 
 __global__ void __launch_bounds__(256)
 k_match_count(const PairMeta* __restrict__ pairs, const int* __restrict__ out, int n_pairs, int* __restrict__ hdr) {
   __shared__ int s_c[8], s_p[8];
+  __shared__ int s_last, s_carry;
+  pdl_wait();
   const PairMeta pm = pairs[blockIdx.x];
+  const int tid = threadIdx.x, lane = tid & 31, wid = tid >> 5;
   int c = 0, pend = 0;
-  for (int r = pm.k0 + threadIdx.x; r < pm.k1; r += 256) {
+  for (int r = pm.k0 + tid; r < pm.k1; r += 256) {
     const int v = out[pm.out_off + r];
     c += v >= 0; pend += v == OUT_PENDING;
   }
   for (int off = 16; off; off >>= 1) { c += __shfl_xor_sync(0xffffffffu, c, off); pend += __shfl_xor_sync(0xffffffffu, pend, off); }
-  if ((threadIdx.x & 31) == 0) { s_c[threadIdx.x >> 5] = c; s_p[threadIdx.x >> 5] = pend; }
+  if (lane == 0) { s_c[wid] = c; s_p[wid] = pend; }
   __syncthreads();
-  if (threadIdx.x == 0) {
+  if (tid == 0) {
     for (int q = 1; q < 8; ++q) { c += s_c[q]; pend += s_p[q]; }
     hdr[2 + blockIdx.x] = c;
     if (pend) atomicAdd(&hdr[1], pend);
-  }
-}
-
-__global__ void __launch_bounds__(1024)
-k_match_offsets(int n_pairs, int* __restrict__ hdr) {
-  __shared__ int s_w[32];
-  __shared__ int s_carry;
+    __threadfence();
+    s_last = atomicAdd(&hdr[3 + 2 * n_pairs], 1) == n_pairs - 1;
+    s_carry = 0;
+  }
+  __syncthreads();
+  if (!s_last) return;
+  __threadfence();
   const int* cnt = hdr + 2;
-  int* off = hdr + 2 + n_pairs;
-  const int tid = threadIdx.x, lane = tid & 31, wid = tid >> 5;
-  if (tid == 0) s_carry = 0;
-  __syncthreads();
-  for (int base = 0; base < n_pairs; base += 1024) {
+  int* offs = hdr + 2 + n_pairs;
+  for (int base = 0; base < n_pairs; base += 256) {
     const int k = base + tid;
-    const int v = k < n_pairs ? cnt[k] : 0;
+    const int v = k < n_pairs ? __ldcg(cnt + k) : 0;
     int incl = v;
     for (int d = 1; d < 32; d <<= 1) { const int t = __shfl_up_sync(0xffffffffu, incl, d); if (lane >= d) incl += t; }
-    if (lane == 31) s_w[wid] = incl;
+    if (lane == 31) s_c[wid] = incl;
     __syncthreads();
     if (wid == 0) {
-      int w = s_w[lane], a = w;
-      for (int d = 1; d < 32; d <<= 1) { const int t = __shfl_up_sync(0xffffffffu, a, d); if (lane >= d) a += t; }
-      s_w[lane] = a - w;
+      const int w = lane < 8 ? s_c[lane] : 0;
+      int a = w;
+      for (int d = 1; d < 8; d <<= 1) { const int t = __shfl_up_sync(0xffffffffu, a, d); if (lane >= d) a += t; }
+      if (lane < 8) s_p[lane] = a - w;
     }
     __syncthreads();
     const int carry = s_carry;
-    if (k < n_pairs) off[k] = carry + s_w[wid] + incl - v;
-    __syncthreads();
-    if (tid == 1023) s_carry = carry + s_w[31] + incl;
-    __syncthreads();
-  }
-  if (tid == 0) { off[n_pairs] = s_carry; hdr[0] = s_carry; }
+    if (k < n_pairs) offs[k] = carry + s_p[wid] + incl - v;
+    __syncthreads();
+    if (tid == 255) s_carry = carry + s_p[7] + incl;
+    __syncthreads();
+  }
+  if (tid == 0) { offs[n_pairs] = s_carry; hdr[0] = s_carry; }
 }
 
 __global__ void __launch_bounds__(256)
@@ -467,6 +531,7 @@
               int* __restrict__ dense) {
   __shared__ int s_w[8];
   __shared__ int s_base;
+  pdl_wait();
   const PairMeta pm = pairs[blockIdx.x];
   int* dst = dense + 2 * (size_t)hdr[2 + n_pairs + blockIdx.x];
   const int tid = threadIdx.x, lane = tid & 31, wid = tid >> 5;
@@ -491,6 +556,7 @@
 }
 
 __global__ void k_match_download(int* __restrict__ h_dst, const int* __restrict__ dense, const int* __restrict__ hdr) {
+  pdl_wait();
   const size_t n = (size_t)hdr[0] * 2;
   for (size_t i = (size_t)blockIdx.x * blockDim.x + threadIdx.x; i < n; i += (size_t)gridDim.x * blockDim.x) h_dst[i] = dense[i];
 }
@@ -516,7 +582,10 @@
 #define MC_FB(r) (1 + (r))
 #define MC_BLK_FILTER(r) (5 + (r))
 #define MC_BLK_NOMINATE(r) (9 + (r))
-#define MC_HEAD 16
+#define MC_TICKET(r) (13 + (r))
+#define MC_OVERFLOW(r) (17 + (r))
+#define MC_TASK_FILTER(r) (21 + (r))
+#define MC_HEAD 25
 #define MC_ROUNDS 4
 
 static bool use_exact_path() {
@@ -654,7 +723,7 @@
     if (pl.max_small > 0) {
       if ((rc = b.list_rows.alloc(ctx, nres))) return rc;
       PANO_LAUNCH(ctx, "k_match_decide", k_match_decide, gd, 256, 0, b.pairs, n_pairs, b.sides, b.info, rs, 1, b.out,
-                  b.counters, b.list_rows, b.list_rows, b.counters + MC_HEAD, n_sides);
+                  b.counters, b.list_rows, b.list_rows, b.counters + MC_HEAD, n_sides, GatherPlan{});
     }
     return PANO_OK;
   }
@@ -662,15 +731,16 @@
   if (rc) return rc;
   if (pl.max_side_n > 0) {
     dim3 gr(ceil_div(pl.max_side_n, 128), grid_y(n_sides));
-    PANO_LAUNCH(ctx, "k_refine", k_refine, gr, 128, 0, fs->d_desc, ops->d_norms, ops->d_maxnorm, b.sides, n_sides, b.approx,
+    PANO_LAUNCH_PDL(ctx, "k_refine", k_refine, gr, 128, 0, fs->d_desc, ops->d_norms, ops->d_maxnorm, b.sides, n_sides, b.approx,
                 (long long)pl.res_total, rs, pl.lazy ? 1 : 0, b.info);
   }
   if (pl.max_small > 0) {
     int block_cap = (int)std::min<size_t>(std::max<size_t>(pl.tc_tasks.size(), 1), 4096);
     if (const char* e = getenv("PANO_MATCH_BLOCK_CAP")) block_cap = std::max(1, std::min(block_cap, atoi(e)));
     const size_t grow = (size_t)block_cap * 128;
+    const int task_cap = block_cap * TC_FILTER_PARTS;
     TcFilter f;
-    if ((rc = b.list_rows.alloc(ctx, nres)) || (rc = b.gtasks.alloc(ctx, block_cap)) ||
+    if ((rc = b.list_rows.alloc(ctx, nres)) || (rc = b.gtasks.alloc(ctx, task_cap)) ||
         (rc = b.gq.alloc(ctx, (size_t)block_cap * tc_block_bytes())) || (rc = b.g_meta.alloc(ctx, grow)) ||
         (rc = b.g_thr.alloc(ctx, grow)) || (rc = b.cand_cnt.alloc(ctx, grow)) ||
         (rc = b.cand.alloc(ctx, grow * TC_CAND_CAP)))
@@ -696,25 +766,25 @@
       int* side_cnt = b.counters + MC_HEAD + round * 2 * n_sides;
       int* fb_cnt = b.counters + MC_FB(round);
       int* n_blocks = b.counters + MC_BLK_FILTER(round);
-      PANO_LAUNCH(ctx, "k_match_decide", k_match_decide, gd, 256, 0, b.pairs, n_pairs, b.sides, b.info, rs, round == 0 ? 1 : 0,
-                  b.out, b.counters, b.list_rows, list_unknown, side_cnt, n_sides);
+      int* n_tasks = b.counters + MC_TASK_FILTER(round);
+      int* nom_blocks = b.counters + MC_BLK_NOMINATE(round);
+      GatherPlan gp{};
+      if (round < b.rounds)
+        gp = GatherPlan{b.gsides, b.counters + MC_TICKET(round), b.list, fb_cnt, block_cap, ctx->num_sms, b.gtasks,
+                        n_blocks, n_tasks, nom_cap, pl.lazy ? b.ntasks.get() : nullptr, nom_blocks};
+      PANO_LAUNCH_PDL(ctx, "k_match_decide", k_match_decide, gd, 256, 0, b.pairs, n_pairs, b.sides, b.info, rs,
+                      round == 0 ? 1 : 0, b.out, b.counters, b.list_rows, list_unknown, side_cnt, n_sides, gp);
       if (round == b.rounds) break;
       if (pl.lazy) {
-        int* nom_blocks = b.counters + MC_BLK_NOMINATE(round);
-        PANO_LAUNCH(ctx, "k_gather_plan", k_gather_plan, ceil_div(n_sides, 128), 128, 0, b.gsides, n_sides,
-                    side_cnt + n_sides, b.list_unknown, nom_cap, b.ntasks, nom_blocks, b.list, fb_cnt);
         nf.n_tasks = nom_blocks;
         if ((rc = tc_run_nominate(ctx, ops, &nf, nom_cap, b.n_approx))) return rc;
-        PANO_LAUNCH(ctx, "k_refine_gathered", k_refine_gathered, nom_cap, 128, 0, fs->d_desc, ops->d_norms, ops->d_maxnorm,
-                    b.sides, b.n_meta, b.n_approx, nom_blocks, rs, b.approx, b.info);
+        PANO_LAUNCH_PDL(ctx, "k_refine_gathered", k_refine_gathered, nom_cap, 128, 0, fs->d_desc, ops->d_norms,
+                        ops->d_maxnorm, b.sides, b.n_meta, b.n_approx, nom_blocks, rs, b.approx, b.info);
       }
-      PANO_LAUNCH(ctx, "k_gather_plan", k_gather_plan, ceil_div(n_sides, 128), 128, 0, b.gsides, n_sides, side_cnt,
-                  b.list_rows, block_cap, b.gtasks, n_blocks, b.list, fb_cnt);
-      f.n_tasks = n_blocks;
-      if ((rc = tc_run_filter(ctx, ops, &f, block_cap))) return rc;
-      PANO_LAUNCH(ctx, "k_exact_cands", k_exact_cands, eg, 256, 0, fs->d_desc, b.sides, n_blocks, b.g_meta, b.cand_cnt,
-                  b.cand, b.info, b.list, fb_cnt);
-      PANO_LAUNCH(ctx, "k_exact_rows", k_exact_rows, eg, 256, 0, fs->d_desc, b.sides, b.list, fb_cnt, b.info);
+      f.n_tasks = n_tasks;
+      if ((rc = tc_run_filter(ctx, ops, &f, task_cap))) return rc;
+      PANO_LAUNCH_PDL(ctx, "k_exact_cands", k_exact_cands, eg, 256, 0, fs->d_desc, b.sides, n_blocks, b.g_meta,
+                      b.cand_cnt, b.cand, b.info, b.list, fb_cnt, b.counters + MC_OVERFLOW(round));
     }
   }
   return PANO_OK;
@@ -770,16 +840,15 @@
   const size_t n_hdr = 3 + 2 * (size_t)n_pairs;
   const size_t cap = (size_t)std::max<long long>(pl.out_total, 1) * 2;
   DevBuf<int> d_hdr, d_dense;
-  if ((rc = d_hdr.alloc(ctx, n_hdr)) || (rc = d_dense.alloc(ctx, cap))) return rc;
+  if ((rc = d_hdr.alloc(ctx, n_hdr + 1)) || (rc = d_dense.alloc(ctx, cap))) return rc;
   int* h_stage = (int*)ctx_ring(ctx, (n_hdr + cap) * sizeof(int));
   if (!h_stage) return ctx_fail(ctx, PANO_ERR_CUDA, "pinned ring allocation failed");
-  if ((rc = ctx_zero(ctx, d_hdr, 2 * sizeof(int)))) return rc;
+  if ((rc = ctx_zero(ctx, d_hdr, (n_hdr + 1) * sizeof(int)))) return rc;
   if (n_pairs > 0) {
-    PANO_LAUNCH(ctx, "k_match_count", k_match_count, n_pairs, 256, 0, b.pairs, b.out, n_pairs, d_hdr);
-    PANO_LAUNCH(ctx, "k_match_offsets", k_match_offsets, 1, 1024, 0, n_pairs, d_hdr);
-    PANO_LAUNCH(ctx, "k_match_write", k_match_write, n_pairs, 256, 0, b.pairs, b.out, n_pairs, d_hdr, d_dense);
-    PANO_LAUNCH(ctx, "k_match_download", k_match_download, std::max(1, std::min(ctx->num_sms, (int)(cap / 4096) + 1)), 256, 0,
-                h_stage + n_hdr, d_dense, d_hdr);
+    PANO_LAUNCH_PDL(ctx, "k_match_count", k_match_count, n_pairs, 256, 0, b.pairs, b.out, n_pairs, d_hdr);
+    PANO_LAUNCH_PDL(ctx, "k_match_write", k_match_write, n_pairs, 256, 0, b.pairs, b.out, n_pairs, d_hdr, d_dense);
+    PANO_LAUNCH_PDL(ctx, "k_match_download", k_match_download, std::max(1, std::min(ctx->num_sms, (int)(cap / 4096) + 1)), 256,
+                    0, h_stage + n_hdr, d_dense, d_hdr);
   }
   rc = ctx_store(ctx, h_stage, d_hdr, n_hdr * sizeof(int));
   cudaError_t e = ctx_spin_stream(ctx);
@@ -834,7 +903,7 @@
       else if (q < n_sides) requested += v;
       else nominated += v;
     }
-  for (int round = 0; round < rounds; ++round) rescans += h[MC_FB(round)];
+  for (int round = 0; round < rounds; ++round) rescans += h[MC_FB(round)] + h[MC_OVERFLOW(round)];
   ctx->last_match_nominated_rows = (int)nominated;
   ctx->last_match_exact_rows = (int)requested;
   ctx->last_match_full_rescans = (int)rescans;
diff --git a/openpano_b200/csrc/match_tc.cu b/openpano_b200/csrc/match_tc.cu
--- a/openpano_b200/csrc/match_tc.cu
+++ b/openpano_b200/csrc/match_tc.cu
@@ -17,6 +17,7 @@
 
 __global__ void k_tc_maxnorm(const float* __restrict__ desc, const TcImage* __restrict__ imgs, int n_img,
                              float* __restrict__ norms, unsigned* __restrict__ maxnorm_bits) {
+  pdl_wait();
   const int img = blockIdx.y;
   const TcImage im = imgs[img];
   const int r = blockIdx.x * blockDim.x + threadIdx.x;
@@ -42,6 +43,7 @@
 __global__ void k_tc_prep(const float* __restrict__ desc, const float* __restrict__ norms,
                           const unsigned* __restrict__ maxnorm_bits, const TcImage* __restrict__ imgs,
                           unsigned char* __restrict__ qbuf, unsigned char* __restrict__ tbuf) {
+  pdl_wait();
   const TcImage im = imgs[blockIdx.y];
   const int r = blockIdx.x * blockDim.x + threadIdx.x;
   if (r >= im.n_pad) return;
@@ -199,6 +201,7 @@
           const unsigned* __restrict__ maxnorm_bits, TcTop2* __restrict__ res,
           const int* __restrict__ g_thr, int* __restrict__ cand_cnt, int* __restrict__ cand) {
   extern __shared__ __align__(1024) unsigned char tc_smem[];
+  pdl_wait();
   const int task_end = n_tasks_dev ? *n_tasks_dev : n_tasks_host;
   if ((int)blockIdx.x >= task_end) return;
   unsigned char* sA = tc_smem;
@@ -271,7 +274,7 @@
                            make_smem_desc(b0 + 16 * TC_SBO + k * 2 * TC_TLBO, TC_TLBO), k);
         wgmma_commit();
         int k1[2] = {0x7fffffff, 0x7fffffff}, k2[2] = {0x7fffffff, 0x7fffffff};
-        const int col_base = t * 256 + 2 * quad;
+        const int col_base = (FILTER ? tk.f_col0 : 0) + t * 256 + 2 * quad;
         wgmma_wait<1>();
         acc_fence(acc0);
         tc_reduce_half<FILTER, 0>(acc0, keymask, prefilter, g2, k1, k2, thr, col_base, tk.t_n, grow, cand_cnt, cand);
@@ -338,8 +341,8 @@
   if ((rc = ctx_zero(ctx, ops->d_maxnorm, sizeof(unsigned)))) return rc;
   if (max_pad == 0) return PANO_OK;
   dim3 g1(ceil_div(max_pad, 128), n);
-  PANO_LAUNCH(ctx, "k_tc_maxnorm", k_tc_maxnorm, g1, 128, 0, d_desc, ops->d_imgs, n, ops->d_norms, ops->d_maxnorm);
-  PANO_LAUNCH(ctx, "k_tc_prep", k_tc_prep, g1, 128, 0, d_desc, ops->d_norms, ops->d_maxnorm, ops->d_imgs, ops->qbuf, ops->tbuf);
+  PANO_LAUNCH_PDL(ctx, "k_tc_maxnorm", k_tc_maxnorm, g1, 128, 0, d_desc, ops->d_imgs, n, ops->d_norms, ops->d_maxnorm);
+  PANO_LAUNCH_PDL(ctx, "k_tc_prep", k_tc_prep, g1, 128, 0, d_desc, ops->d_norms, ops->d_maxnorm, ops->d_imgs, ops->qbuf, ops->tbuf);
   return PANO_OK;
 }
 
@@ -356,7 +359,7 @@
   if (n_tasks == 0) return PANO_OK;
   const size_t smem = tc_smem_bytes();
   if (int rc = tc_set_attrs(ctx)) return rc;
-  PANO_LAUNCH(ctx, "k_tc_top2", k_tc_pass<false>, std::min(n_tasks, ctx->num_sms), TC_THREADS, smem, ops->qbuf, ops->tbuf, d_tasks,
+  PANO_LAUNCH_PDL(ctx, "k_tc_top2", k_tc_pass<false>, std::min(n_tasks, ctx->num_sms), TC_THREADS, smem, ops->qbuf, ops->tbuf, d_tasks,
               (const int*)nullptr, n_tasks, ops->d_maxnorm, d_res, (const int*)nullptr, (int*)nullptr, (int*)nullptr);
   return PANO_OK;
 }
@@ -369,8 +372,10 @@
                  const TcTop2* __restrict__ approx, const float* __restrict__ norms,
                  const unsigned* __restrict__ maxnorm_bits, int2* __restrict__ g_meta, int* __restrict__ g_thr,
                  int* __restrict__ cand_cnt) {
+  pdl_wait();
   if ((int)blockIdx.x >= *n_tasks_dev) return;
   const TcTask tk = tasks[blockIdx.x];
+  if (tk.f_col0 != 0) return;
   const int side = (int)tk.res_off;
   const TcGatherSide gs = gsides[side];
   const int r = threadIdx.x, g = tk.q_row0 + r;
@@ -403,9 +408,9 @@
   if (max_blocks <= 0) return PANO_OK;
   const size_t smem = tc_smem_bytes();
   if (int rc = tc_set_attrs(ctx)) return rc;
-  PANO_LAUNCH(ctx, "k_tc_gather_rows", k_tc_gather_rows, max_blocks, 128, 0, ops->qbuf, f->gq, f->tasks, f->n_tasks,
+  PANO_LAUNCH_PDL(ctx, "k_tc_gather_rows", k_tc_gather_rows, max_blocks, 128, 0, ops->qbuf, f->gq, f->tasks, f->n_tasks,
               f->gsides, f->list_rows, f->approx, ops->d_norms, ops->d_maxnorm, f->g_meta, f->g_thr, f->cand_cnt);
-  PANO_LAUNCH(ctx, "k_tc_filter", k_tc_pass<true>, std::min(max_blocks, ctx->num_sms), TC_THREADS, smem, f->gq, ops->tbuf, f->tasks, f->n_tasks,
+  PANO_LAUNCH_PDL(ctx, "k_tc_filter", k_tc_pass<true>, std::min(max_blocks, ctx->num_sms), TC_THREADS, smem, f->gq, ops->tbuf, f->tasks, f->n_tasks,
               0, ops->d_maxnorm, (TcTop2*)nullptr, f->g_thr, f->cand_cnt, f->cand);
   return PANO_OK;
 }
@@ -414,10 +419,10 @@
   if (max_blocks <= 0) return PANO_OK;
   const size_t smem = tc_smem_bytes();
   if (int rc = tc_set_attrs(ctx)) return rc;
-  PANO_LAUNCH(ctx, "k_tc_gather_rows", k_tc_gather_rows, max_blocks, 128, 0, ops->qbuf, f->gq, f->tasks, f->n_tasks,
+  PANO_LAUNCH_PDL(ctx, "k_tc_gather_rows", k_tc_gather_rows, max_blocks, 128, 0, ops->qbuf, f->gq, f->tasks, f->n_tasks,
               f->gsides, f->list_rows, (const TcTop2*)nullptr, ops->d_norms, ops->d_maxnorm, f->g_meta, (int*)nullptr,
               (int*)nullptr);
-  PANO_LAUNCH(ctx, "k_tc_nominate", k_tc_pass<false>, std::min(max_blocks, ctx->num_sms), TC_THREADS, smem, f->gq, ops->tbuf, f->tasks,
+  PANO_LAUNCH_PDL(ctx, "k_tc_nominate", k_tc_pass<false>, std::min(max_blocks, ctx->num_sms), TC_THREADS, smem, f->gq, ops->tbuf, f->tasks,
               f->n_tasks, 0, ops->d_maxnorm, d_res, (const int*)nullptr, (int*)nullptr, (int*)nullptr);
   return PANO_OK;
 }
diff --git a/openpano_b200/csrc/match_tc.cuh b/openpano_b200/csrc/match_tc.cuh
--- a/openpano_b200/csrc/match_tc.cuh
+++ b/openpano_b200/csrc/match_tc.cuh
@@ -19,6 +19,8 @@
   int t_blk0, t_blocks;
   int t_n, t_pad;
   long long res_off;
+  int f_col0;
+  int f_pad;
 };
 
 struct TcGatherSide {
diff --git a/openpano_b200/csrc/sift.cu b/openpano_b200/csrc/sift.cu
--- a/openpano_b200/csrc/sift.cu
+++ b/openpano_b200/csrc/sift.cu
@@ -329,6 +329,7 @@
 
 __global__ void __launch_bounds__(256)
 k_extrema_seams(const OctMeta* __restrict__ octs, int n_oct, const float* __restrict__ arena, const ExtremaParams ep) {
+  pdl_wait();
   const int img = blockIdx.y;
   const int n = min(ep.seam_count[img], ep.seam_cap);
   for (int i = blockIdx.x * blockDim.x + threadIdx.x; i < n; i += gridDim.x * blockDim.x) {
@@ -367,6 +368,7 @@
 k_rank_sort(const int* __restrict__ cand_count, const uint32_t* __restrict__ keys,
             uint32_t* __restrict__ sorted, int cap) {
   __shared__ uint32_t sk[1024];
+  pdl_wait();
   const int img = blockIdx.y;
   const int n = min(cand_count[img], cap);
   const uint32_t* k = keys + (size_t)img * cap;
@@ -483,6 +485,7 @@
 __global__ void k_refine(const OctMeta* __restrict__ octs, const float* __restrict__ arena, int n_oct,
                          const int* __restrict__ cand_count, const uint32_t* __restrict__ sorted,
                          RefineParams rp, int cap, pano_sspoint* __restrict__ out, unsigned char* __restrict__ valid) {
+  pdl_wait();
   const int img = blockIdx.y;
   const int n = min(cand_count[img], cap);
   for (int i = blockIdx.x * blockDim.x + threadIdx.x; i < n; i += gridDim.x * blockDim.x) {
@@ -578,6 +581,7 @@
   __shared__ uint64_t s_exptab[32];
   __shared__ int s_pref[SIFT_MAX_IMG + 1];
   load_exp2f_tab(s_exptab, threadIdx.x);
+  pdl_wait();
   if (threadIdx.x == 0) {
     int acc = 0;
     for (int i = 0; i < n_img; ++i) { s_pref[i] = acc; acc += min(cand_count[i], cap); }
@@ -703,6 +707,7 @@
               int* __restrict__ desc_cand, float* __restrict__ desc_dir) {
   __shared__ int s_warp[32];
   __shared__ int s_warp2[32];
+  pdl_wait();
   const int img = blockIdx.x;
   const int n = min(cand_count[img], cap);
   const int per = (n + SCAN_THREADS - 1) / SCAN_THREADS;
@@ -780,6 +785,7 @@
   __shared__ uint64_t s_exptab[32];
   __shared__ int s_pref[SIFT_MAX_IMG + 1];
   load_exp2f_tab(s_exptab, threadIdx.x);
+  pdl_wait();
   if (threadIdx.x == 0) {
     int acc = 0;
     for (int i = 0; i < n_img; ++i) { s_pref[i] = acc; acc += min(n_desc[i], cap); }
@@ -1219,7 +1225,7 @@
       const int grid = std::min(wk->n_tiles, ctx->num_sms * 3);
       PANO_LAUNCH(ctx, "k_blur_extrema", k_blur_extrema, grid, BT_THREADS, smf, wk->d_oct, wk->d_tilespan, n_om, wk->n_tiles,
                   wk->d_maps, wk->arena, gt, ep);
-      PANO_LAUNCH(ctx, "k_extrema_seams", k_extrema_seams, dim3(8, n), 256, 0, wk->d_oct, n_oct, wk->arena, ep);
+      PANO_LAUNCH_PDL(ctx, "k_extrema_seams", k_extrema_seams, dim3(8, n), 256, 0, wk->d_oct, n_oct, wk->arena, ep);
     } else {
       if (smem > 48 * 1024)
         PANO_CUDA(ctx, sift_smem_limit(ctx, (const void*)k_blur_dog, smem));
@@ -1230,22 +1236,22 @@
   }
   {
     dim3 g(8, n);
-    PANO_LAUNCH(ctx, "k_rank_sort", k_rank_sort, g, 256, 0, wk->cand_count, wk->cand_keys, wk->sorted_keys, cap);
+    PANO_LAUNCH_PDL(ctx, "k_rank_sort", k_rank_sort, g, 256, 0, wk->cand_count, wk->cand_keys, wk->sorted_keys, cap);
     RefineParams rp{n_scale, p->calc_offset_depth, p->offset_thres, p->contrast_thres, p->edge_ratio,
                     p->gauss_sigma, p->scale_factor};
     dim3 g4(16, n);
-    PANO_LAUNCH(ctx, "k_refine", k_refine, g4, 128, 0, wk->d_oct, wk->arena, n_oct, wk->cand_count, wk->sorted_keys, rp, cap,
+    PANO_LAUNCH_PDL(ctx, "k_refine", k_refine, g4, 128, 0, wk->d_oct, wk->arena, n_oct, wk->cand_count, wk->sorted_keys, rp, cap,
                 wk->refined, wk->kp_valid);
-    PANO_LAUNCH(ctx, "k_orientation", k_orientation, ctx->num_sms * 8, ORI_WARPS * 32, 0, wk->d_oct, wk->arena, n_oct, n, cap,
+    PANO_LAUNCH_PDL(ctx, "k_orientation", k_orientation, ctx->num_sms * 8, ORI_WARPS * 32, 0, wk->d_oct, wk->arena, n_oct, n, cap,
                 wk->cand_count, wk->refined, wk->kp_valid, p->ori_radius, p->ori_hist_smooth_count, wk->npeaks, wk->dirs,
                 wk->cand_count + n + 1);
-    PANO_LAUNCH(ctx, "k_expand_scan", k_expand_scan, n, SCAN_THREADS, 0, wk->cand_count, wk->kp_valid, wk->npeaks,
+    PANO_LAUNCH_PDL(ctx, "k_expand_scan", k_expand_scan, n, SCAN_THREADS, 0, wk->cand_count, wk->kp_valid, wk->npeaks,
                 wk->dirs, cap, fs->d_count, wk->n_refined, wk->desc_cand, wk->desc_dir);
     DescParams dp{p->desc_hist_scale_factor, p->desc_int_factor};
     const size_t dsm = sizeof(DescQuadSmem) * DESC_WARPS;
     PANO_CUDA(ctx, sift_smem_limit(ctx, (const void*)k_descriptor, dsm));
     const int grid = ctx->num_sms * DESC_MIN_CTAS;
-    PANO_LAUNCH(ctx, "k_descriptor", k_descriptor, grid, DESC_THREADS, dsm, wk->d_oct, wk->d_img, wk->arena, n_oct, n, cap,
+    PANO_LAUNCH_PDL(ctx, "k_descriptor", k_descriptor, grid, DESC_THREADS, dsm, wk->d_oct, wk->d_img, wk->arena, n_oct, n, cap,
                 wk->refined, fs->d_count, wk->desc_cand, wk->desc_dir, dp, fs->d_desc, fs->d_coor, wk->cand_count + n);
   }
   wk->n_desc = fs->d_count;
```
